# pw1316/MonteCarloPathTracer

Hardware: AMD Instinct MI355X
Metric: Mray/s + achieved HBM GB/s, Cornell Box 1024spp at 1/2/4/8 MI355X (higher is better)
Workload: dtype f32; 1 GPU; cornell_1024x1024_1024spp; scene=scene01, width=1024, height=1024, spp=1024, max_depth=7, spp_chunk=32, parallelism=pixel-tiles x1, pipeline=wavefront, wf_sort=False, kd_build=reference, kd_nodes=4395, kernel_variant=4

## Files before the change

include/mcpt.h:

```cpp
#ifndef MCPT_H
#define MCPT_H

#include <stddef.h>
#include <stdint.h>

#ifdef __cplusplus
extern "C" {
#endif

#define MCPT_ABI_VERSION 9

enum {
    MCPT_OK = 0,
    MCPT_E_INVALID = -1,
    MCPT_E_IO = -2,
    MCPT_E_PARSE = -3,
    MCPT_E_DEVICE = -4,
    MCPT_E_NOMEM = -5,
    MCPT_E_UNSUPPORTED = -6
};

typedef struct mcpt_model mcpt_model;
typedef struct mcpt_scene mcpt_scene;

// ... 84 lines not shown

typedef struct {
    int32_t pipeline;
    int32_t variant;
    int32_t wf_streams;
    uint32_t wf_batch;
    int32_t wf_refill;
    int32_t wf_group_shift;
    int32_t ready_thresh;
    int32_t tail_units;
    uint64_t work_paths;
    uint64_t workspace_bytes;
    uint64_t wf_queue_bytes;
    uint64_t device_free_bytes;
    int32_t devices;
    int32_t peer_access;
    uint32_t wf_batch_default;
} mcpt_plan_info;

typedef struct {
    const char* kd_cache_dir;
    int32_t host_only;
    int32_t layout;
    int32_t kd_build;
} mcpt_scene_options;

enum {
    MCPT_LAYOUT_AUTO = 0,
    MCPT_LAYOUT_GLOBAL = 1
};
enum {
    MCPT_KD_BUILD_REFERENCE = 0,
    MCPT_KD_BUILD_SAH = 1
};

int mcpt_abi_version(void);
const char* mcpt_last_error(void);
int mcpt_init(const int32_t* devices, int32_t n_devices);
int mcpt_device_count(int32_t* out);
void mcpt_render_params_default(mcpt_render_params* p);
void mcpt_render_params_quinengine(mcpt_render_params* p);

typedef struct {
    const float* vertices;        int64_t n_vertices;
    const float* normals;         int64_t n_normals;
    const int32_t* triangles;     int64_t n_triangles;
    const double* materials;      int64_t n_materials;
    const char* const* group_names;
    const int64_t* group_offsets;
    const int32_t* group_tris;    int64_t n_groups;
} mcpt_model_desc;
int mcpt_model_create(const mcpt_model_desc* d, mcpt_model** out);
int mcpt_model_read_obj(const char* path, mcpt_model** out);
int mcpt_model_read_obj_ex(const char* path, int32_t flavor, mcpt_model** out);
enum {
    MCPT_OBJ_CVMCTRACER = 0,
    MCPT_OBJ_TINYOBJ = 1
};
void mcpt_model_free(mcpt_model* m);
int mcpt_model_get_info(const mcpt_model* m, mcpt_model_info* out);
int mcpt_model_copy_vertices(const mcpt_model* m, float* out);
int mcpt_model_copy_normals(const mcpt_model* m, float* out);
int mcpt_model_copy_triangles(const mcpt_model* m, int32_t* out);
int mcpt_model_copy_materials(const mcpt_model* m, double* out);
int mcpt_model_group(const mcpt_model* m, int64_t g, char* name_buf, int64_t name_cap,
                     int64_t* n, int32_t* tris);

int mcpt_scene_create(const mcpt_model* m, mcpt_scene** out);
int mcpt_scene_create_host(const mcpt_model* m, mcpt_scene** out);
int mcpt_scene_create_cached(const mcpt_model* m, const char* kd_cache_dir, int32_t host_only,
                             mcpt_scene** out, int32_t* cache_hit);
int mcpt_scene_create_ex(const mcpt_model* m, const mcpt_scene_options* options, mcpt_scene** out,
                         int32_t* cache_hit);
void mcpt_scene_destroy(mcpt_scene* s);
int mcpt_scene_get_info(const mcpt_scene* s, mcpt_scene_info* out);
int mcpt_scene_terminal_cull_boxes(const mcpt_scene* s);
int mcpt_scene_miss_cull_boxes(const mcpt_scene* s, float* boxes);
int mcpt_scene_direct_lists(const mcpt_scene* s, int32_t* tri_box, uint32_t* box_tris, uint32_t* lists,
                            int32_t* list_kd);
uint64_t mcpt_scene_direct_rays(const mcpt_scene* s);
uint64_t mcpt_scene_extend_rays(const mcpt_scene* s);
uint64_t mcpt_scene_clipped_rays(const mcpt_scene* s);
uint64_t mcpt_scene_primary_shaded(const mcpt_scene* s);
uint64_t mcpt_scene_primary_shade_lds(const mcpt_scene* s);
int mcpt_scene_primary_tile_classes(mcpt_scene* s, uint32_t out[4]);
int mcpt_scene_copy_kd(const mcpt_scene* s, uint32_t* nodes, uint32_t* leaf_ids,
                       int32_t* kd_tris, float* geoms);

int mcpt_render(mcpt_scene* s, const mcpt_render_params* p, float* fb_rgb, mcpt_render_stats* stats);
int mcpt_render_device(mcpt_scene* s, const mcpt_render_params* p, float* d_fb_rgba, void* hip_stream);
int mcpt_render_stats_read(mcpt_scene* s, mcpt_render_stats* out);
int mcpt_render_unit_counters(mcpt_scene* s, const mcpt_render_params* p, float* fb_rgb,
                              uint32_t* unit_counters);
int64_t mcpt_shard_pixel_count(const mcpt_render_params* p);
int mcpt_shard_pixels(const mcpt_render_params* p, int32_t* xy);
int mcpt_intersect(mcpt_scene* s, int64_t n, const float* o, const float* d, float t_max,
                   int32_t* tri_out, float* hit_out, mcpt_render_stats* stats);
int mcpt_scene_reserve(mcpt_scene* s, const mcpt_render_params* p);
int mcpt_plan_query(mcpt_scene* s, const mcpt_render_params* p, mcpt_plan_info* out);

int mcpt_render_aov(mcpt_scene* s, const mcpt_render_params* p, float* albedo_cov, float* normal_depth);
int mcpt_render_aov_device(mcpt_scene* s, const mcpt_render_params* p, float* d_albedo_cov, float* d_normal_depth,
                           void* hip_stream);

typedef struct {
    int32_t width, height;
    int32_t iterations;
    int32_t normal_power_log2;
    float sigma_z;
    float albedo_floor;
    int32_t gamma_space;
} mcpt_denoise_params;
void mcpt_denoise_params_default(mcpt_denoise_params* p);
int mcpt_denoise(const mcpt_denoise_params* p, const float* color_rgb, const float* albedo_cov,
                 const float* normal_depth, float* out_rgb);
int mcpt_denoise_device(const mcpt_denoise_params* p, const float* d_color_rgba, const float* d_albedo_cov,
                        const float* d_normal_depth, float* d_out_rgba, float* d_scratch_rgba, void* hip_stream);

int mcpt_render_var(mcpt_scene* s, const mcpt_render_params* p, float* fb_rgb, float* var_rgba,
                    mcpt_render_stats* stats);
int mcpt_render_var_device(mcpt_scene* s, const mcpt_render_params* p, float* d_fb_rgba, float* d_var_rgba,
                           void* hip_stream);

typedef struct {
    mcpt_denoise_params base;
    float sigma_l;
} mcpt_denoise_var_params;
void mcpt_denoise_var_params_default(mcpt_denoise_var_params* p);
int mcpt_denoise_var(const mcpt_denoise_var_params* p, const float* color_rgb, const float* var_rgba,
                     const float* albedo_cov, const float* normal_depth, float* out_rgb);
int mcpt_denoise_var_device(const mcpt_denoise_var_params* p, const float* d_color_rgba, const float* d_var_rgba,
                            const float* d_albedo_cov, const float* d_normal_depth, float* d_out_rgba,
                            float* d_scratch_rgba, void* hip_stream);

typedef struct {
    int32_t max_passes;
    int32_t min_passes;
    float   threshold;
    float   lum_floor;
    int32_t dilate;
    int32_t force_list;
} mcpt_adaptive_params;
void mcpt_adaptive_params_default(mcpt_adaptive_params*);
int mcpt_render_adaptive(mcpt_scene*, const mcpt_render_params*, const mcpt_adaptive_params*,
                         float* fb_rgb, float* var_rgba, uint32_t* pass_count, mcpt_render_stats* stats);
int mcpt_render_adaptive_device(mcpt_scene*, const mcpt_render_params*, const mcpt_adaptive_params*,
                                float* d_fb_rgba, float* d_var_rgba, uint32_t* d_pass_count, void* hip_stream);
int mcpt_render_adaptive_ex(mcpt_scene*, const mcpt_render_params*, const mcpt_adaptive_params*,
                            float* fb_rgb, float* var_rgba, uint32_t* pass_count, mcpt_render_stats* stats);
int mcpt_render_adaptive_ex_device(mcpt_scene*, const mcpt_render_params*, const mcpt_adaptive_params*,
                                   float* d_fb_rgba, float* d_var_rgba, uint32_t* d_pass_count, void* hip_stream);

enum { MCPT_TRACE_CLOSEST = 0, MCPT_TRACE_ANY = 1 };
typedef struct {
    int32_t kind;
    float   t_max;
    int32_t lean;
    int32_t workgroups;
    int32_t refill;
} mcpt_trace_params;
void mcpt_trace_params_default(mcpt_trace_params*);

int mcpt_trace_device(mcpt_scene*, const mcpt_trace_params* p, int64_t n, const float* d_o, const float* d_d,
                      const float* d_t_max, int32_t* d_tri, float* d_hit, void* hip_stream);
int mcpt_occluded_device(mcpt_scene*, const mcpt_trace_params* p, int64_t n, const float* d_o, const float* d_d,
                         const float* d_t_max, uint8_t* d_occluded, void* hip_stream);
// ... 31 lines not shown
```

montecarlopathtracer_amd/_build.py:

```python
from __future__ import annotations

import os
import subprocess
import sys
from concurrent.futures import ThreadPoolExecutor

HERE = os.path.dirname(os.path.abspath(__file__))
ROOT = os.path.dirname(HERE)
CSRC = os.path.join(HERE, "csrc")
LIBDIR = os.path.join(HERE, "lib")
LIB = os.path.join(LIBDIR, os.environ.get("MCPT_LIB_NAME", "libmcpt.so"))
SOURCES = ["host_model.cpp", "kd_cache.cpp", "capi.cpp", "scene_image.cpp", "plan.cpp", "render_host.cpp", "queries.cpp",
           "render.hip", "wavefront.hip", "wavefront_primary.hip", "wavefront_primary_shade.hip",
           "aov.hip", "denoise.hip", "variance.hip", "denoise_var.hip", "adaptive.hip", "rayquery.hip"]
_WF_FLAGS = ["-mllvm", "-amdgpu-set-wave-priority=1", "-mllvm", "-two-entry-phi-node-folding-threshold=8",
             "-mllvm", "-unroll-threshold=2000"]
SOURCE_FLAGS = {"wavefront_primary.hip": ["-mllvm", "-structurizecfg-skip-uniform-regions=1"] + _WF_FLAGS,
                "wavefront_primary_shade.hip": _WF_FLAGS,
                "wavefront.hip": _WF_FLAGS,
                "rayquery.hip": _WF_FLAGS,
                "render.hip": ["-mllvm", "-enable-gvn-hoist", "-mllvm", "-unroll-threshold=2000"]}
SOURCE_SCHED = {"wavefront_primary_shade.hip": "iterative-minreg"}
HEADERS = ["capi_internal.hpp", "staging.hpp", "host_model.hpp", "mcpt_device.hpp", "render_launch.hpp", "wf_route.hpp", "trace_device.hpp", "half_box.hpp",
           "aov_device.hpp", "aov_launch.hpp", "variance_launch.hpp", "adaptive_launch.hpp", "partial_sum.hpp", "rayquery_launch.hpp",
           "wf_device.hpp", "wf_primary_body.hpp", "wf_primary_walk.hpp", "wf_primary_pairs.hpp", "wf_primary_shade_body.hpp", "wf_shade_item.hpp"]
ARCH = os.environ.get("MCPT_OFFLOAD_ARCH", "gfx950")

COMMON = ["-O3", "-std=c++17", "-fPIC", "-ffp-contract=off", "-fno-fast-math", "-fno-slp-vectorize", "-Wall",
          "-I" + os.path.join(ROOT, "include")] + os.environ.get("MCPT_EXTRA_FLAGS", "").split()


def _hipcc() -> str:
    for c in (os.environ.get("HIPCC"), "/opt/rocm/bin/hipcc", "hipcc"):
        if c and (os.path.sep not in c or os.path.exists(c)):
            return c
    raise RuntimeError("hipcc not found")


def _stale() -> bool:
    if not os.path.exists(LIB):
        return True
    t = os.path.getmtime(LIB)
    deps = [os.path.join(CSRC, f) for f in SOURCES + HEADERS] + [os.path.join(ROOT, "include", "mcpt.h"),
                                                                 os.path.abspath(__file__)]
    return any(os.path.getmtime(d) > t for d in deps)


def build(force: bool = False, verbose: bool = False) -> str:
    if not force and not _stale():
        return LIB
    os.makedirs(os.path.join(LIBDIR, "obj"), exist_ok=True)
    hipcc = _hipcc()

    def compile_one(src):
        obj = os.path.join(LIBDIR, "obj", os.path.basename(LIB) + "." + src + ".o")
        sched = SOURCE_SCHED.get(src) or os.environ.get("MCPT_SCHED", "max-ilp")
        lang = (["-x", "hip", f"--offload-arch={ARCH}", "-mllvm", f"-amdgpu-sched-strategy={sched}"]
                if src.endswith(".hip")
                else ["-x", "c++", "-D__HIP_PLATFORM_AMD__", "-I/opt/rocm/include"])
        cmd = [hipcc] + lang + COMMON + SOURCE_FLAGS.get(src, []) + ["-c", os.path.join(CSRC, src), "-o", obj]
        if verbose:
            print(" ".join(cmd), file=sys.stderr)
        r = subprocess.run(cmd, capture_output=True, text=True)
        if r.returncode != 0:
            raise RuntimeError(f"compile failed: {src}\n{r.stdout}\n{r.stderr}")
        return obj

    with ThreadPoolExecutor(max_workers=len(SOURCES)) as ex:
        objs = list(ex.map(compile_one, SOURCES))
    tmp = LIB + f".{os.getpid()}.tmp"
    cmd = [hipcc, f"--offload-arch={ARCH}", "-shared", "-fPIC", "-o", tmp] + objs
    r = subprocess.run(cmd, capture_output=True, text=True)
    if r.returncode != 0:
        raise RuntimeError(f"link failed\n{r.stdout}\n{r.stderr}")
    os.replace(tmp, LIB)
    return LIB


if __name__ == "__main__":
    print(build(force="--force" in sys.argv, verbose=True))
```

montecarlopathtracer_amd/_capi.py:

```python
from __future__ import annotations

import ctypes as C
import os

try:
    import torch
except Exception:
    torch = None

_HERE = os.path.dirname(os.path.abspath(__file__))
LIB_PATH = os.environ.get("MCPT_LIB_PATH") or os.path.join(_HERE, "lib", "libmcpt.so")

MCPT_OK = 0
ABI_VERSION = 9
MODE_CVMCTRACER = 0
MODE_QUINENGINE = 1
PIPELINE_MEGAKERNEL = 0
PIPELINE_WAVEFRONT = 1
GATHER_PEER = 0
GATHER_RCCL = 1
ERRORS = {-1: "INVALID", -2: "IO", -3: "PARSE", -4: "DEVICE", -5: "NOMEM", -6: "UNSUPPORTED"}


class McptError(RuntimeError):
# ... 57 lines not shown


class DenoiseParamsC(C.Structure):
    _fields_ = [("width", C.c_int32), ("height", C.c_int32), ("iterations", C.c_int32),
                ("normal_power_log2", C.c_int32), ("sigma_z", C.c_float), ("albedo_floor", C.c_float),
                ("gamma_space", C.c_int32)]


class DenoiseVarParamsC(C.Structure):
    _fields_ = [("base", DenoiseParamsC), ("sigma_l", C.c_float)]


class AdaptiveParamsC(C.Structure):
    _fields_ = [("max_passes", C.c_int32), ("min_passes", C.c_int32), ("threshold", C.c_float),
                ("lum_floor", C.c_float), ("dilate", C.c_int32), ("force_list", C.c_int32)]


class TraceParamsC(C.Structure):
    _fields_ = [("kind", C.c_int32), ("t_max", C.c_float), ("lean", C.c_int32), ("workgroups", C.c_int32),
                ("refill", C.c_int32)]


class RadianceParamsC(C.Structure):
    _fields_ = [("spp", C.c_uint32), ("spp_offset", C.c_uint32), ("spp_chunk", C.c_uint32),
                ("max_depth", C.c_int32), ("illum", C.c_float), ("fresnel_kd", C.c_int32), ("seed", C.c_uint64),
                ("prev_count", C.c_uint32), ("lean", C.c_int32), ("workgroups", C.c_int32),
                ("ready_thresh", C.c_int32)]


TRACE_CLOSEST = 0
TRACE_ANY = 1
OBJ_CVMCTRACER = 0
OBJ_TINYOBJ = 1
LAYOUT_AUTO = 0
LAYOUT_GLOBAL = 1
KD_BUILD_REFERENCE = 0
KD_BUILD_SAH = 1


class ModelDesc(C.Structure):
    _fields_ = [
        ("vertices", C.POINTER(C.c_float)), ("n_vertices", C.c_int64),
        ("normals", C.POINTER(C.c_float)), ("n_normals", C.c_int64),
        ("triangles", C.POINTER(C.c_int32)), ("n_triangles", C.c_int64),
        ("materials", C.POINTER(C.c_double)), ("n_materials", C.c_int64),
        ("group_names", C.POINTER(C.c_char_p)), ("group_offsets", C.POINTER(C.c_int64)),
        ("group_tris", C.POINTER(C.c_int32)), ("n_groups", C.c_int64),
    ]


_vp = C.c_void_p
_SIGS = {
    "mcpt_abi_version": (C.c_int, []),
    "mcpt_last_error": (C.c_char_p, []),
    "mcpt_init": (C.c_int, [C.POINTER(C.c_int32), C.c_int32]),
    "mcpt_device_count": (C.c_int, [C.POINTER(C.c_int32)]),
    "mcpt_render_params_default": (None, [C.POINTER(RenderParamsC)]),
    "mcpt_render_params_quinengine": (None, [C.POINTER(RenderParamsC)]),
    "mcpt_model_create": (C.c_int, [C.POINTER(ModelDesc), C.POINTER(_vp)]),
    "mcpt_model_read_obj": (C.c_int, [C.c_char_p, C.POINTER(_vp)]),
    "mcpt_model_read_obj_ex": (C.c_int, [C.c_char_p, C.c_int32, C.POINTER(_vp)]),
    "mcpt_model_free": (None, [_vp]),
    "mcpt_model_get_info": (C.c_int, [_vp, C.POINTER(ModelInfo)]),
    "mcpt_model_copy_vertices": (C.c_int, [_vp, C.POINTER(C.c_float)]),
    "mcpt_model_copy_normals": (C.c_int, [_vp, C.POINTER(C.c_float)]),
    "mcpt_model_copy_triangles": (C.c_int, [_vp, C.POINTER(C.c_int32)]),
    "mcpt_model_copy_materials": (C.c_int, [_vp, C.POINTER(C.c_double)]),
    "mcpt_model_group": (C.c_int, [_vp, C.c_int64, C.c_char_p, C.c_int64, C.POINTER(C.c_int64), C.POINTER(C.c_int32)]),
    "mcpt_scene_create": (C.c_int, [_vp, C.POINTER(_vp)]),
    "mcpt_scene_create_host": (C.c_int, [_vp, C.POINTER(_vp)]),
    "mcpt_scene_create_cached": (C.c_int, [_vp, C.c_char_p, C.c_int32, C.POINTER(_vp), C.POINTER(C.c_int32)]),
    "mcpt_scene_create_ex": (C.c_int, [_vp, C.POINTER(SceneOptions), C.POINTER(_vp), C.POINTER(C.c_int32)]),
    "mcpt_scene_destroy": (None, [_vp]),
    "mcpt_scene_get_info": (C.c_int, [_vp, C.POINTER(SceneInfo)]),
    "mcpt_scene_terminal_cull_boxes": (C.c_int, [_vp]),
    "mcpt_scene_miss_cull_boxes": (C.c_int, [_vp, C.POINTER(C.c_float)]),
    "mcpt_scene_primary_tile_classes": (C.c_int, [_vp, C.POINTER(C.c_uint32)]),
    "mcpt_scene_direct_lists": (C.c_int, [_vp, C.POINTER(C.c_int32), C.POINTER(C.c_uint32), C.POINTER(C.c_uint32),
                                           C.POINTER(C.c_int32)]),
    "mcpt_scene_direct_rays": (C.c_uint64, [_vp]),
    "mcpt_scene_extend_rays": (C.c_uint64, [_vp]),
    "mcpt_scene_clipped_rays": (C.c_uint64, [_vp]),
    "mcpt_scene_primary_shaded": (C.c_uint64, [_vp]),
    "mcpt_scene_primary_shade_lds": (C.c_uint64, [_vp]),
    "mcpt_scene_copy_kd": (C.c_int, [_vp, C.POINTER(C.c_uint32), C.POINTER(C.c_uint32), C.POINTER(C.c_int32),
                                     C.POINTER(C.c_float)]),
    "mcpt_render": (C.c_int, [_vp, C.POINTER(RenderParamsC), C.POINTER(C.c_float), C.POINTER(RenderStats)]),
    "mcpt_render_device": (C.c_int, [_vp, C.POINTER(RenderParamsC), _vp, _vp]),
    "mcpt_render_unit_counters": (C.c_int, [_vp, C.POINTER(RenderParamsC), C.POINTER(C.c_float),
                                            C.POINTER(C.c_uint32)]),
    "mcpt_render_stats_read": (C.c_int, [_vp, C.POINTER(RenderStats)]),
    "mcpt_intersect": (C.c_int, [_vp, C.c_int64, C.POINTER(C.c_float), C.POINTER(C.c_float), C.c_float,
                                 C.POINTER(C.c_int32), C.POINTER(C.c_float), C.POINTER(RenderStats)]),
    "mcpt_shard_pixel_count": (C.c_int64, [C.POINTER(RenderParamsC)]),
    "mcpt_shard_pixels": (C.c_int, [C.POINTER(RenderParamsC), C.POINTER(C.c_int32)]),
    "mcpt_scene_reserve": (C.c_int, [_vp, C.POINTER(RenderParamsC)]),
    "mcpt_plan_query": (C.c_int, [_vp, C.POINTER(RenderParamsC), C.POINTER(PlanInfo)]),
    "mcpt_render_aov": (C.c_int, [_vp, C.POINTER(RenderParamsC), C.POINTER(C.c_float), C.POINTER(C.c_float)]),
    "mcpt_render_aov_device": (C.c_int, [_vp, C.POINTER(RenderParamsC), _vp, _vp, _vp]),
    "mcpt_denoise_params_default": (None, [C.POINTER(DenoiseParamsC)]),
    "mcpt_denoise": (C.c_int, [C.POINTER(DenoiseParamsC), C.POINTER(C.c_float), C.POINTER(C.c_float),
                               C.POINTER(C.c_float), C.POINTER(C.c_float)]),
    "mcpt_denoise_device": (C.c_int, [C.POINTER(DenoiseParamsC), _vp, _vp, _vp, _vp, _vp, _vp]),
    "mcpt_render_var": (C.c_int, [_vp, C.POINTER(RenderParamsC), C.POINTER(C.c_float), C.POINTER(C.c_float),
                                  C.POINTER(RenderStats)]),
    "mcpt_render_var_device": (C.c_int, [_vp, C.POINTER(RenderParamsC), _vp, _vp, _vp]),
    "mcpt_denoise_var_params_default": (None, [C.POINTER(DenoiseVarParamsC)]),
    "mcpt_denoise_var": (C.c_int, [C.POINTER(DenoiseVarParamsC), C.POINTER(C.c_float), C.POINTER(C.c_float),
                                   C.POINTER(C.c_float), C.POINTER(C.c_float), C.POINTER(C.c_float)]),
    "mcpt_denoise_var_device": (C.c_int, [C.POINTER(DenoiseVarParamsC), _vp, _vp, _vp, _vp, _vp, _vp, _vp]),
    "mcpt_adaptive_params_default": (None, [C.POINTER(AdaptiveParamsC)]),
    "mcpt_render_adaptive": (C.c_int, [_vp, C.POINTER(RenderParamsC), C.POINTER(AdaptiveParamsC),
                                       C.POINTER(C.c_float), C.POINTER(C.c_float), C.POINTER(C.c_uint32),
                                       C.POINTER(RenderStats)]),
    "mcpt_render_adaptive_device": (C.c_int, [_vp, C.POINTER(RenderParamsC), C.POINTER(AdaptiveParamsC), _vp, _vp,
                                              _vp, _vp]),
    "mcpt_render_adaptive_ex": (C.c_int, [_vp, C.POINTER(RenderParamsC), C.POINTER(AdaptiveParamsC),
                                          C.POINTER(C.c_float), C.POINTER(C.c_float), C.POINTER(C.c_uint32),
                                          C.POINTER(RenderStats)]),
    "mcpt_render_adaptive_ex_device": (C.c_int, [_vp, C.POINTER(RenderParamsC), C.POINTER(AdaptiveParamsC), _vp,
                                                 _vp, _vp, _vp]),
    "mcpt_trace_params_default": (None, [C.POINTER(TraceParamsC)]),
    "mcpt_trace_device": (C.c_int, [_vp, C.POINTER(TraceParamsC), C.c_int64, _vp, _vp, _vp, _vp, _vp, _vp]),
    "mcpt_occluded_device": (C.c_int, [_vp, C.POINTER(TraceParamsC), C.c_int64, _vp, _vp, _vp, _vp, _vp]),
    "mcpt_occluded": (C.c_int, [_vp, C.POINTER(TraceParamsC), C.c_int64, C.POINTER(C.c_float), C.POINTER(C.c_float),
                                C.POINTER(C.c_float), C.POINTER(C.c_uint8), C.POINTER(RenderStats)]),
    "mcpt_trace_stats_read": (C.c_int, [_vp, C.POINTER(RenderStats)]),
    "mcpt_scene_reserve_rays": (C.c_int, [_vp]),
    "mcpt_radiance_params_default": (None, [C.POINTER(RadianceParamsC)]),
    "mcpt_radiance_device": (C.c_int, [_vp, C.POINTER(RadianceParamsC), C.c_int64, _vp, _vp, _vp, _vp, _vp]),
    "mcpt_radiance": (C.c_int, [_vp, C.POINTER(RadianceParamsC), C.c_int64, C.POINTER(C.c_float),
                                C.POINTER(C.c_float), C.POINTER(C.c_uint32), C.POINTER(C.c_float),
                                C.POINTER(RenderStats)]),
    "mcpt_scene_reserve_radiance": (C.c_int, [_vp, C.POINTER(RadianceParamsC), C.c_int64]),
}

_lib = None


def lib():
    global _lib
    if _lib is None:
        if not os.path.exists(LIB_PATH):
            raise ImportError(f"{LIB_PATH} not found: build it with `python -c 'import __graft_entry__ as g; "
                              f"g.build()'` or `python -m montecarlopathtracer_amd._build`")
        L = C.CDLL(LIB_PATH)
        for name, (res, args) in _SIGS.items():
            f = getattr(L, name)
            f.restype = res
            f.argtypes = args
        if L.mcpt_abi_version() != ABI_VERSION:
            raise ImportError("libmcpt.so ABI version mismatch")
        _lib = L
    return _lib


def check(rc: int) -> int:
    if rc < 0:
        raise McptError(rc, lib().mcpt_last_error().decode(errors="replace"))
    return rc


def declared_symbols():
    return list(_SIGS)
```

montecarlopathtracer_amd/csrc/capi_internal.hpp:

```cpp
#pragma once
#include <hip/hip_runtime.h>
#include <rccl/rccl.h>

#include <cstdint>
#include <cstring>
#include <memory>
#include <string>
#include <vector>

#include "../../include/mcpt.h"
#include "host_model.hpp"
#include "render_launch.hpp"
#include "staging.hpp"
#include "wf_route.hpp"

struct mcpt_model {
    mcpt::ObjModel m;
};

namespace mcpt::host {

int fail(int code, const std::string& msg);
extern thread_local std::vector<int> g_devices;
extern thread_local bool g_peer_ok;
// ... 5 lines not shown
            throw mcpt::Error{e_ == hipErrorOutOfMemory ? MCPT_E_NOMEM : MCPT_E_DEVICE,   \
                              std::string(#expr) + ": " + hipGetErrorString(e_)};       \
    } while (0)

template <typename F>
int guarded(F&& f) {
    try {
        return f();
    } catch (const mcpt::Error& e) {
        return fail(e.code, e.msg);
    } catch (const std::bad_alloc&) {
        return fail(MCPT_E_NOMEM, "out of host memory");
    } catch (const std::exception& e) {
        return fail(MCPT_E_INVALID, e.what());
    }
}

struct DevBuf {
    void* p = nullptr;
    size_t bytes = 0;
};

struct TempDev {
    void* p = nullptr;
    TempDev() = default;
    explicit TempDev(size_t bytes) { alloc(bytes); }
    TempDev(const TempDev&) = delete;
    TempDev& operator=(const TempDev&) = delete;
    ~TempDev() {
        if (p) (void)hipFree(p);
    }
    void alloc(size_t bytes) { HIP_TRY(hipMalloc(&p, bytes ? bytes : 16)); }
    void* release() {
        void* q = p;
        p = nullptr;
        return q;
    }
};

struct Workspace {
    DevBuf partial;
    DevBuf small;
    DevBuf spill;
    DevBuf fb;
    DevBuf wf;
    DevBuf tail;
};

struct Timing {
    hipEvent_t e[3];
};

struct DeviceGuard {
    int prev = -1;
    DeviceGuard() { (void)hipGetDevice(&prev); }
    ~DeviceGuard() {
        if (prev >= 0) (void)hipSetDevice(prev);
    }
};

}

struct mcpt_scene {
    mcpt::HostScene hs;
    bool on_device = false;
    int device = -1;
    int cus = 0;
    std::vector<unsigned char> image;
    std::vector<uint32_t> tri_order;
    mcpt::GpuScene gpu{};
    uint32_t n_cull_boxes = 0;
    uint32_t cull_box[mcpt::kMaxCullBoxes][3] = {};
    float cull_gain = 0.0f;
    uint32_t n_miss_boxes = 0;
    float miss_box[mcpt::kMaxMissBoxes][6] = {};
    std::vector<int32_t> tri_box;
    uint32_t box_tris[mcpt::kMaxMissBoxes] = {};
    uint32_t direct_counts = 0;
    uint32_t direct_list[mcpt::kMaxMissBoxes * 16] = {};
    uint64_t direct_rays = 0;
    uint64_t extend_rays = 0;
    uint64_t clipped_rays = 0;
    uint64_t primary_shaded = 0;
    mcpt::host::DevBuf d_image, d_normals;
    mcpt::host::Workspace ws;
    std::vector<mcpt::host::Timing> pending, free_timing;
    mcpt::host::Timing capture_timing{};
    bool has_capture_timing = false;
    int last_variant = 0;
    uint64_t renders = 0;
    size_t wf_reserved = 0;
    bool reserved = false;
    std::vector<void*> retired;
    std::vector<std::unique_ptr<mcpt_scene>> replicas;
    hipStream_t stream = nullptr;
    hipEvent_t done = nullptr;
    hipEvent_t start = nullptr;
    mcpt::host::DevBuf gather;
    hipStream_t wf_stream[mcpt::kMaxWfStreams] = {};
    hipEvent_t wf_fork = nullptr, wf_join[mcpt::kMaxWfStreams] = {};
    bool peer_access = true;
    std::vector<ncclComm_t> comms;
    mcpt::host::DevBuf gather_send;
    mcpt::host::DevBuf ad_list, ad_flags, ad_blocks;
    uint32_t* ad_host_n = nullptr;
    mcpt::host::DevBuf rq_order, rq_stats;
    mcpt::host::DevBuf rad_partial, rad_tail, rad_small;

    std::vector<mcpt::host::DevBuf*> buffers() {
        return {&d_image, &d_normals, &ws.partial, &ws.small, &ws.spill, &ws.fb, &ws.wf, &ws.tail, &gather, &gather_send,
                &ad_list, &ad_flags, &ad_blocks, &rq_order, &rq_stats, &rad_partial, &rad_tail, &rad_small};
    }
    ~mcpt_scene();
};

namespace mcpt::host {

struct Plan {
    mcpt::KernelParams kp;
    size_t out_pixels;
    bool capturing = false;
    int pipeline;
    int wf_streams;
    uint32_t wf_capacity;
    bool wf_batch_explicit;
    int32_t wf_sort;
    int32_t wf_refill;
    mcpt::WfRoute route;
    int64_t tail_per_lane;
    int64_t tail_exact;
    uint64_t wf_mem_limit;
    uint64_t work;
    int sets() const { return pipeline == MCPT_PIPELINE_WAVEFRONT ? wf_streams : 1; }
};

struct Prepared {
    Plan pl;
    mcpt::WfParams wf[mcpt::kMaxWfStreams];
};

inline bool ranges_overlap(const void* a, size_t na, const void* b, size_t nb) {
    const uintptr_t x = reinterpret_cast<uintptr_t>(a), y = reinterpret_cast<uintptr_t>(b);
    return x < y + nb && y < x + na;
}

void ensure_buf(DevBuf& b, size_t need);
void grow_ws(mcpt_scene& s, DevBuf& b, size_t need, bool capturing);
void set_device(const mcpt_scene& s);
bool stream_capturing(hipStream_t st);
uint32_t tea16(uint32_t v0, uint32_t v1);
int ready_thresh_for(const mcpt_scene& s, int32_t asked);
size_t launched_lanes(const mcpt_scene& s);
mcpt::WfFacts scene_facts(const mcpt_scene& s);
constexpr size_t kSpillEntries = 32;
constexpr int64_t kTailPerLane = 4;
size_t spill_bytes(const mcpt_scene& s, int sets);
void grow_spill(mcpt_scene& s, int sets, bool capturing);
uint64_t tail_split(uint64_t lanes, int64_t per_lane, int64_t exact, uint32_t total_units, uint32_t chunk);
uint64_t tail_units_for(const mcpt_scene& s, const Plan& pl);
Plan make_plan(const mcpt_scene& s, const mcpt_render_params* p);
uint32_t wf_batch_capacity(const mcpt_scene& s, const mcpt_render_params* p, uint64_t work, uint32_t chunk, int nstr);
void prepare_wavefront_list(mcpt_scene& s, Plan& pl, const Plan& pass0, uint32_t n, const mcpt_render_params* p,
                            mcpt::WfParams* out);
void fit_wavefront(const mcpt_scene& s, Plan& pl);
void prepare_workspace(mcpt_scene& s, Plan& pl, bool tail_split = false, int spill_sets = 1);
uint32_t* tile_classes(const mcpt_scene& s);
// ... 8 lines not shown
```

montecarlopathtracer_amd/csrc/host_model.cpp:

```cpp
#include "host_model.hpp"

#include <algorithm>
#include <array>
#include <cmath>
#include <cctype>
#include <cfloat>
#include <cstdio>
#include <cstdlib>
#include <cstring>
#include <deque>
#include <fstream>
#include <map>
#include <numeric>
#include <sstream>

#include "../../include/mcpt.h"

namespace mcpt {
namespace {

struct Cursor {
    const char* p;
    const char* end;
    bool fail = false;
// ... 501 lines not shown
    if (!nt || max_boxes < 1) return 0;
    for (float v : hs.kd_verts)
        if (!std::isfinite(v)) return 0;
    std::vector<CBox> tb(nt);
    CBox all{{INFINITY, INFINITY, INFINITY}, {-INFINITY, -INFINITY, -INFINITY}};
    for (size_t k = 0; k < nt; ++k) {
        const float* v = &hs.kd_verts[9 * k];
        CBox b{{v[0], v[1], v[2]}, {v[0], v[1], v[2]}};
        for (int j = 1; j < 3; ++j) b.add(CBox{{v[3 * j], v[3 * j + 1], v[3 * j + 2]}, {v[3 * j], v[3 * j + 1], v[3 * j + 2]}});
        tb[k] = b;
        all.add(b);
    }
    std::vector<CBox> bx;
    if (nt <= kMissCullExact) {
        bx = tb;
    } else {
        for (int with_planes = 1; with_planes >= 0; --with_planes) {
            std::map<std::pair<int, uint32_t>, CBox> buckets;
            for (const CBox& b : tb) {
                std::pair<int, uint32_t> key{3, 0u};
                for (int a = 0; a < 3 && with_planes; ++a)
                    if (b.lo[a] == b.hi[a] && key.first == 3) {
                        const float c = b.lo[a] + 0.0f;
                        uint32_t bits;
                        std::memcpy(&bits, &c, 4);
                        key = {a, bits};
                    }
                if (key.first == 3) {
                    for (int a = 0; a < 3; ++a) {
                        const double ext = double(all.hi[a]) - all.lo[a];
                        const double c = (double(b.lo[a]) + b.hi[a]) * 0.5 - all.lo[a];
                        const int cell = ext > 0.0 ? std::min(7, std::max(0, int(c / ext * 8.0))) : 0;
                        key.second = key.second * 8u + uint32_t(cell);
                    }
                }
                auto it = buckets.find(key);
                if (it == buckets.end()) buckets.emplace(key, b);
                else it->second.add(b);
            }
            bx.clear();
            for (const auto& kv : buckets) bx.push_back(kv.second);
            if (bx.size() <= kMissCullExact) break;
        }
    }
    cluster_boxes(bx, bx.size());
    bool face[3][2] = {};
    for (const CBox& b : bx) {
        for (int a = 0; a < 3; ++a) {
            if (b.lo[a] != b.hi[a]) continue;
            bool covers = true;
            for (int c = 0; c < 3; ++c)
                if (c != a) covers = covers && b.lo[c] <= all.lo[c] && b.hi[c] >= all.hi[c];
            if (covers && b.lo[a] == all.lo[a]) face[a][0] = true;
            if (covers && b.lo[a] == all.hi[a]) face[a][1] = true;
        }
    }
    if (face[0][0] && face[0][1] && face[1][0] && face[1][1] && face[2][0] && face[2][1]) return 0;
    cluster_boxes(bx, static_cast<size_t>(max_boxes));
    for (const CBox& b : bx) {
        bool spans = true;
        for (int a = 0; a < 3; ++a) spans = spans && b.lo[a] <= all.lo[a] && b.hi[a] >= all.hi[a];
        if (spans) return 0;
    }
    for (size_t k = 0; k < bx.size(); ++k)
        for (int a = 0; a < 3; ++a) {
            boxes[k][a] = bx[k].lo[a];
            boxes[k][3 + a] = bx[k].hi[a];
        }
    return static_cast<int>(bx.size());
}

void direct_list_assign(const HostScene& hs, const float (*boxes)[6], int n_boxes, std::vector<int32_t>& tri_box) {
    const size_t nt = hs.kd_verts.size() / 9;
    tri_box.assign(nt, -1);
    for (size_t k = 0; k < nt; ++k) {
        const float* v = &hs.kd_verts[9 * k];
        for (int b = 0; b < n_boxes && tri_box[k] < 0; ++b) {
            bool in = true;
            for (int j = 0; j < 3; ++j)
                for (int a = 0; a < 3; ++a) in = in && v[3 * j + a] >= boxes[b][a] && v[3 * j + a] <= boxes[b][3 + a];
            if (in) tri_box[k] = b;
        }
    }
}

namespace {

inline float smin(float a, float b) { return (b < a) ? b : a; }
inline float smax(float a, float b) { return (a < b) ? b : a; }

struct Box {
    float mn[3], mx[3];
    static Box empty() {
        Box b;
        for (int i = 0; i < 3; ++i) { b.mn[i] = FLT_MAX; b.mx[i] = -FLT_MAX; }
        return b;
    }
    void add_pt(const float* p) {
        for (int i = 0; i < 3; ++i) { mn[i] = smin(mn[i], p[i]); mx[i] = smax(mx[i], p[i]); }
    }
    void add(const Box& r) { add_pt(r.mn); add_pt(r.mx); }
    void clip(const Box& r) {
        for (int i = 0; i < 3; ++i) { mn[i] = smax(mn[i], r.mn[i]); mx[i] = smin(mx[i], r.mx[i]); }
    }
    float half_area() const {
        float s0 = mx[0] - mn[0], s1 = mx[1] - mn[1], s2 = mx[2] - mn[2];
        return s0 * s1 + s1 * s2 + s2 * s0;
    }
};

struct BNode {
    Box box;
    Box region;
    std::vector<uint32_t> ids;
    uint32_t axis = 0;
    float split = 0.0f;
    int32_t left = -1, right = -1;
    int depth = 0;
};

template <typename FL, typename FR>
inline void classify(const Box& tb, int a, float v, FL&& to_left, FR&& to_right) {
    if (tb.mn[a] == tb.mx[a] && tb.mn[a] == v) {
        to_left();
    } else {
        if (tb.mn[a] < v) to_left();
        if (tb.mx[a] > v) to_right();
    }
}

#ifndef MCPT_SAH_CT
#define MCPT_SAH_CT 1.0f
#define MCPT_SAH_CI 1.5f
#endif
constexpr float kSahCt = MCPT_SAH_CT, kSahCi = MCPT_SAH_CI;
struct SahScratch {
    std::vector<float> mins, maxs, plan, cand;
};
bool sah_split(const std::vector<Box>& tbox, const std::vector<uint32_t>& ids, const Box& R, SahScratch& w,
               int& ax, float& val) {
    const float sz[3] = {R.mx[0] - R.mn[0], R.mx[1] - R.mn[1], R.mx[2] - R.mn[2]};
    const float A0 = sz[0] * sz[1] + sz[1] * sz[2] + sz[2] * sz[0];
    if (!(A0 > 0.0f)) return false;
    const size_t n = ids.size();
    float best = kSahCi * static_cast<float>(n);
    bool found = false;
    for (int a = 0; a < 3; ++a) {
        w.mins.clear(); w.maxs.clear(); w.plan.clear(); w.cand.clear();
        for (uint32_t id : ids) {
            const float lo = tbox[id].mn[a], hi = tbox[id].mx[a];
            w.mins.push_back(lo);
            w.maxs.push_back(hi);
            if (lo == hi) w.plan.push_back(lo);
            if (R.mn[a] < lo && lo < R.mx[a]) w.cand.push_back(lo + 0.0f);
            if (R.mn[a] < hi && hi < R.mx[a]) w.cand.push_back(hi + 0.0f);
        }
        std::sort(w.mins.begin(), w.mins.end());
        std::sort(w.maxs.begin(), w.maxs.end());
        std::sort(w.plan.begin(), w.plan.end());
        std::sort(w.cand.begin(), w.cand.end());
        size_t im = 0, ix = 0, ip = 0;
        for (size_t q = 0; q < w.cand.size(); ++q) {
            if (q > 0 && !(w.cand[q - 1] < w.cand[q])) continue;
            const float v = w.cand[q];
            while (im < n && w.mins[im] < v) ++im;
            while (ix < n && !(v < w.maxs[ix])) ++ix;
// ... 161 lines not shown
```

montecarlopathtracer_amd/csrc/host_model.hpp:

```cpp
#pragma once

#include <cstdint>
#include <map>
#include <string>
#include <vector>

namespace mcpt {

struct Vec3 {
    float x = 0, y = 0, z = 0;
};

struct ObjTriangle {
    int32_t v[3] = {0, 0, 0};
    int32_t t[3] = {0, 0, 0};
    int32_t n[3] = {0, 0, 0};
    int32_t material = 0;
};

struct ObjMaterial {
    std::string name;
    Vec3 Ka, Kd, Ks;
    double Ns = 1.0, Tr = 0.0, Ni = 1.0;
};

struct ObjModel {
    std::string path;
    std::vector<Vec3> vertices;
    int64_t n_texcoords = 0;
    std::vector<Vec3> normals;
    std::vector<ObjTriangle> triangles;
    std::vector<ObjMaterial> materials;
    std::map<std::string, std::vector<int32_t>> groups;
};

void read_obj(const std::string& path, ObjModel& out, int flavor = 0);
void read_obj_cv(const std::string& path, ObjModel& out);

struct Geometry {
    Vec3 Ka, Kd, Ks;
    float Ns, Tr, Ni;
    uint32_t start, count;
};

struct KdNode {
    uint32_t left = 0xFFFFFFFFu, right = 0xFFFFFFFFu;
    float bmin[3], bmax[3];
    uint32_t axis = 0;
    float split = 0.0f;
    uint32_t leaf_begin = 0, leaf_count = 0;
};

struct HostScene {
    std::vector<Geometry> geoms;
    std::vector<int32_t> kd_tris;
    std::vector<uint32_t> kd_geom;
    std::vector<uint32_t> kd_prio;
    std::vector<float> kd_verts;
    std::vector<float> kd_normals;
    std::vector<KdNode> nodes;
    std::vector<uint32_t> leaf_ids;
    int kd_depth = 0;
    int kd_build = 0;
};

void build_host_scene(const ObjModel& m, HostScene& out, const char* kd_cache_dir = nullptr,
                      int* cache_hit = nullptr, int kd_build = 0);
int terminal_cull_boxes(const HostScene& hs, float (*boxes)[6], int max_boxes);
int miss_cull_boxes(const HostScene& hs, float (*boxes)[6], int max_boxes);
void direct_list_assign(const HostScene& hs, const float (*boxes)[6], int n_boxes, std::vector<int32_t>& tri_box);
bool kd_cache_load(const std::string& dir, const std::vector<float>& tri_verts, std::vector<KdNode>& nodes,
                   std::vector<uint32_t>& leaf_ids, int& depth, int kd_build = 0);
bool kd_cache_store(const std::string& dir, const std::vector<float>& tri_verts, const std::vector<KdNode>& nodes,
                    const std::vector<uint32_t>& leaf_ids, int depth, int kd_build = 0);
void build_kdtree(const std::vector<float>& tri_verts, std::vector<KdNode>& nodes,
                  std::vector<uint32_t>& leaf_ids, int& depth, int kd_build = 0);

struct Error {
    int code;
    std::string msg;
};

}
```

montecarlopathtracer_amd/csrc/plan.cpp:

```cpp
#include <algorithm>
#include <cfloat>
#include <cmath>
#include <cstdio>

#include "capi_internal.hpp"

using namespace mcpt::host;

namespace {

struct Vf {
    float x, y, z;
};
Vf normal_of(Vf v) {
    float len = std::sqrt(v.x * v.x + v.y * v.y + v.z * v.z);
    float d = std::fmax(len, FLT_MIN);
    return Vf{v.x / d, v.y / d, v.z / d};
}
Vf cross_of(Vf a, Vf b) { return Vf{a.y * b.z - a.z * b.y, a.z * b.x - a.x * b.z, a.x * b.y - a.y * b.x}; }

int clamp_i(int v, int lo, int hi) { return v < lo ? lo : (v > hi ? hi : v); }

int wavefront_streams(const mcpt::WfRoute& r, uint64_t work, const mcpt_render_params* p) {
    const int n = p->wf_streams > 0 ? p->wf_streams
// ... 51 lines not shown
        w.radiance = reinterpret_cast<float4*>(b); b += l.f4;
        w.tile_cand = l.tiles ? reinterpret_cast<uint32_t*>(b) : nullptr; b += l.tiles;
        w.tile_classes = tile_classes(s);
        w.cnt = reinterpret_cast<mcpt::WfCounters*>(b);
        w.capacity = pl.wf_capacity;
        w.slot_stride = static_cast<uint32_t>(l.cap_slots);
        w.refill_thresh = clamp_i(pl.wf_refill, 1, 64);
        w.sort = pl.wf_sort;
        w.nseg = r.nseg;
        w.group_shift = r.group_shift;
        w.xcd_deal = r.xcd_deal;
        w.shade_cull = r.shade_cull ? 1u : 0u;
        w.n_cull_boxes = r.n_cull_boxes;
        std::memcpy(w.cull_box, s.cull_box, sizeof w.cull_box);
        w.n_miss_boxes = r.n_miss_boxes;
        std::memcpy(w.miss_box, s.miss_box, sizeof w.miss_box);
        w.direct_counts = r.direct_counts;
        std::memcpy(w.direct_list, s.direct_list, sizeof w.direct_list);
    }
}

void ensure_wf_streams(mcpt_scene& s, int n) {
    if (n > 1 && !s.wf_fork) HIP_TRY(hipEventCreateWithFlags(&s.wf_fork, hipEventDisableTiming));
    for (int i = 1; i < n; i++) {
        if (!s.wf_stream[i]) HIP_TRY(hipStreamCreateWithFlags(&s.wf_stream[i], hipStreamNonBlocking));
        if (!s.wf_join[i]) HIP_TRY(hipEventCreateWithFlags(&s.wf_join[i], hipEventDisableTiming));
    }
}

}

namespace mcpt::host {

void ensure_buf(DevBuf& b, size_t need) {
    if (b.bytes >= need && b.p) return;
    if (b.p) HIP_TRY(hipFree(b.p));
    b.p = nullptr;
    b.bytes = 0;
    HIP_TRY(hipMalloc(&b.p, need ? need : 16));
    b.bytes = need;
}

void grow_ws(mcpt_scene& s, DevBuf& b, size_t need, bool capturing) {
    if (b.bytes >= need && b.p) return;
    if (capturing)
        throw mcpt::Error{MCPT_E_NOMEM, "render needs more workspace than the scene holds while its stream is "
                                        "capturing a graph: call mcpt_scene_reserve with these params first"};
    if (b.p && s.reserved) {
        s.retired.push_back(b.p);
        b.p = nullptr;
        b.bytes = 0;
    }
    ensure_buf(b, need);
}

void set_device(const mcpt_scene& s) {
    int cur = -1;
    HIP_TRY(hipGetDevice(&cur));
    if (cur != s.device) HIP_TRY(hipSetDevice(s.device));
}

bool stream_capturing(hipStream_t st) {
    if (!st) return false;
    hipStreamCaptureStatus cs = hipStreamCaptureStatusNone;
    HIP_TRY(hipStreamIsCapturing(st, &cs));
    return cs != hipStreamCaptureStatusNone;
}

uint32_t tea16(uint32_t v0, uint32_t v1) {
    uint32_t sum = 0;
    for (int n = 0; n < 16; n++) {
        sum += 0x9e3779b9u;
        v0 += ((v1 << 4) + 0xa341316cu) ^ (v1 + sum) ^ ((v1 >> 5) + 0xc8013ea4u);
        v1 += ((v0 << 4) + 0xad90777du) ^ (v0 + sum) ^ ((v0 >> 5) + 0x7e95761eu);
    }
    return v0;
}

int ready_thresh_for(const mcpt_scene& s, int32_t asked) { return asked > 0 ? asked : (mcpt::scene_in_lds(s.gpu) ? 32 : 40); }

size_t launched_lanes(const mcpt_scene& s) { return static_cast<size_t>(mcpt::total_lanes_for(s.gpu, s.cus)); }

mcpt::WfFacts scene_facts(const mcpt_scene& s) {
    return mcpt::WfFacts{&s.gpu, s.n_miss_boxes, s.direct_counts, s.n_cull_boxes, s.cus};
}

size_t spill_bytes(const mcpt_scene& s, int sets) { return size_t(sets) * kSpillEntries * launched_lanes(s) * 16; }
void grow_spill(mcpt_scene& s, int sets, bool capturing) { grow_ws(s, s.ws.spill, spill_bytes(s, sets), capturing); }

Plan make_plan(const mcpt_scene& s, const mcpt_render_params* p) {
    if (!p) throw mcpt::Error{MCPT_E_INVALID, "params is NULL"};
    if (p->width <= 0 || p->height <= 0) throw mcpt::Error{MCPT_E_INVALID, "width/height must be positive"};
    if (p->spp == 0) throw mcpt::Error{MCPT_E_INVALID, "spp must be > 0"};
    if (p->max_depth < 0 || p->max_depth > mcpt::kMaxDepthParam) throw mcpt::Error{MCPT_E_INVALID, "max_depth out of range"};
    if (p->wf_streams < 0 || p->wf_streams > mcpt::kMaxWfStreams)
        throw mcpt::Error{MCPT_E_INVALID, "wf_streams must be 0 (automatic) or 1..4"};
    if (p->wf_refill < 0 || p->wf_refill > 64 || p->ready_thresh < 0 || p->ready_thresh > 64)
        throw mcpt::Error{MCPT_E_INVALID, "wf_refill / ready_thresh must be 0 (automatic) or 1..64"};
    if (p->wf_group_shift != 0 && (p->wf_group_shift < 6 || p->wf_group_shift > 14))
        throw mcpt::Error{MCPT_E_INVALID, "wf_group_shift must be 0 (automatic) or 6..14"};
    if (p->tail_units < 0) throw mcpt::Error{MCPT_E_INVALID, "tail_units must be >= 0"};
    if (p->gather != MCPT_GATHER_PEER && p->gather != MCPT_GATHER_RCCL)
        throw mcpt::Error{MCPT_E_INVALID, "unknown gather"};
    const int T = p->tile > 0 ? p->tile : 8;
    if (T > 256) throw mcpt::Error{MCPT_E_INVALID, "tile too large"};
    const int sc = p->shard_count > 1 ? p->shard_count : 1;
    const int si = sc > 1 ? p->shard_index : 0;
    if (si < 0 || si >= sc) throw mcpt::Error{MCPT_E_INVALID, "shard_index out of range"};
    const uint64_t tiles_x = (uint64_t(p->width) + T - 1) / T, tiles_y = (uint64_t(p->height) + T - 1) / T;
    const uint64_t ntiles = tiles_x * tiles_y;
    const uint64_t owned = uint64_t(si) < ntiles ? (ntiles - uint64_t(si) + uint64_t(sc) - 1) / uint64_t(sc) : 0;
    const uint64_t npix = owned * uint64_t(T) * uint64_t(T);
    const uint32_t chunk = p->spp_chunk ? (p->spp_chunk < p->spp ? p->spp_chunk : p->spp) : p->spp;
    const uint64_t nchunks = (uint64_t(p->spp) + chunk - 1) / chunk;
    if (npix * nchunks >= 0xFFFFFFFFull) throw mcpt::Error{MCPT_E_UNSUPPORTED, "too many work units for one call"};

    Plan pl;
    mcpt::KernelParams& k = pl.kp;
    std::memset(&k, 0, sizeof k);
    k.scene = s.gpu;
    k.width = p->width; k.height = p->height;
    k.tile = T; k.tiles_x = static_cast<int32_t>(tiles_x);
    k.shard_count = sc; k.shard_index = si;
    k.packed = (p->packed || sc > 1) ? 1 : 0;
    k.npix_local = static_cast<uint32_t>(npix);
    k.spp = p->spp; k.spp_offset = p->spp_offset; k.chunk = chunk;
    k.nchunks = static_cast<uint32_t>(nchunks);
    k.total_units = static_cast<uint32_t>(npix * nchunks);
    k.div_npix = mcpt::FastDiv::make(std::max<uint32_t>(k.npix_local, 1));
    k.div_tt = mcpt::FastDiv::make(static_cast<uint32_t>(T * T));
    k.div_tiles_x = mcpt::FastDiv::make(static_cast<uint32_t>(tiles_x));
    k.div_tile = mcpt::FastDiv::make(static_cast<uint32_t>(T));
    k.div_chunk = mcpt::FastDiv::make(chunk);
    k.tail_units = k.total_units;
    k.total_items = k.total_units;
    k.max_depth = p->max_depth;
    k.lean = p->lean ? 1 : 0;
    k.illum = p->illum;
    const float a = p->fov_deg * 3.14159265359f / 360;
    k.tan_half_fov = static_cast<float>(std::tan(static_cast<double>(a)));
    k.h_over_w = 1.0 * static_cast<double>(static_cast<uint32_t>(p->height)) / static_cast<double>(static_cast<uint32_t>(p->width));
    k.inv_w_pow2 = (p->width > 0 && (p->width & (p->width - 1)) == 0) ? 1.0 / static_cast<double>(p->width) : 0.0;
    k.fresnel_kd = p->fresnel_kd ? 1 : 0;
    k.prev_count = p->prev_count;
    Vf d = normal_of(Vf{p->dir[0], p->dir[1], p->dir[2]});
    Vf r = normal_of(cross_of(d, Vf{p->up[0], p->up[1], p->up[2]}));
    Vf u = normal_of(cross_of(r, d));
    for (int i = 0; i < 3; ++i) k.eye[i] = p->eye[i];
    k.fwd[0] = d.x; k.fwd[1] = d.y; k.fwd[2] = d.z;
    k.up[0] = u.x; k.up[1] = u.y; k.up[2] = u.z;
    k.right[0] = r.x; k.right[1] = r.y; k.right[2] = r.z;
    if (p->mode != MCPT_MODE_CVMCTRACER && p->mode != MCPT_MODE_QUINENGINE)
        throw mcpt::Error{MCPT_E_INVALID, "unknown mode"};
    k.mode = p->mode;
    k.best_init = FLT_MAX;
    if (p->mode == MCPT_MODE_QUINENGINE) {
        k.key = static_cast<uint32_t>(p->seed);
        k.best_init = 10000.0f;
        const float a = p->fov_deg * 3.14159265359f / 360;
        const float ys = static_cast<float>(1.0 / std::tan(static_cast<double>(a)));
        k.proj22 = ys;
        k.proj11 = ys / (static_cast<float>(p->width) / static_cast<float>(p->height));
    } else {
        k.key = tea16(static_cast<uint32_t>(p->seed), static_cast<uint32_t>(p->seed >> 32));
    }
    k.ready_thresh = ready_thresh_for(s, p->ready_thresh);
    pl.out_pixels = k.packed ? size_t(npix) : size_t(p->width) * size_t(p->height);
// ... 227 lines not shown
```

montecarlopathtracer_amd/csrc/render_host.cpp:

```cpp
#include <dlfcn.h>

#include <algorithm>
#include <cmath>

#include "adaptive_launch.hpp"
#include "aov_launch.hpp"
#include "capi_internal.hpp"
#include "variance_launch.hpp"

using namespace mcpt::host;

namespace {

struct Rccl {
    decltype(&ncclCommInitAll) comm_init_all = nullptr;
    decltype(&ncclCommDestroy) comm_destroy = nullptr;
    decltype(&ncclGather) gather = nullptr;
    decltype(&ncclGroupStart) group_start = nullptr;
    decltype(&ncclGroupEnd) group_end = nullptr;
    decltype(&ncclGetErrorString) error_string = nullptr;
    std::string load_error;
};
const Rccl& rccl() {
    static const Rccl r = [] {
        Rccl x;
        void* h = dlopen("librccl.so.1", RTLD_NOW | RTLD_LOCAL);
        if (!h) h = dlopen("/opt/rocm/lib/librccl.so.1", RTLD_NOW | RTLD_LOCAL);
        if (!h) {
            const char* e = dlerror();
            x.load_error = std::string("cannot load librccl: ") + (e ? e : "?");
            return x;
        }
        x.comm_init_all = reinterpret_cast<decltype(&ncclCommInitAll)>(dlsym(h, "ncclCommInitAll"));
        x.comm_destroy = reinterpret_cast<decltype(&ncclCommDestroy)>(dlsym(h, "ncclCommDestroy"));
        x.gather = reinterpret_cast<decltype(&ncclGather)>(dlsym(h, "ncclGather"));
        x.group_start = reinterpret_cast<decltype(&ncclGroupStart)>(dlsym(h, "ncclGroupStart"));
        x.group_end = reinterpret_cast<decltype(&ncclGroupEnd)>(dlsym(h, "ncclGroupEnd"));
        x.error_string = reinterpret_cast<decltype(&ncclGetErrorString)>(dlsym(h, "ncclGetErrorString"));
        if (!x.comm_init_all || !x.comm_destroy || !x.gather || !x.group_start || !x.group_end || !x.error_string)
            x.load_error = "librccl lacks ncclCommInitAll / ncclGather / ncclGroupStart / ncclGroupEnd";
        return x;
    }();
    return r;
}

#define NCCL_TRY(expr)                                                                                  \
    do {                                                                                                \
        ncclResult_t r_ = (expr);                                                                       \
        if (r_ != ncclSuccess)                                                                          \
            throw mcpt::Error{MCPT_E_DEVICE, std::string(#expr) + ": " + rccl().error_string(r_)};   \
    } while (0)

void render_multi(mcpt_scene& s, const mcpt_render_params* p, float* d_fb, hipStream_t st);

void ensure_capture_timing(mcpt_scene& s) {
    if (s.has_capture_timing) return;
    for (auto& ev : s.capture_timing.e) HIP_TRY(hipEventCreate(&ev));
    s.has_capture_timing = true;
}

Timing acquire_timing(mcpt_scene& s, bool capturing) {
    Timing t;
    if (capturing) {
        ensure_capture_timing(s);
        t = s.capture_timing;
    } else if (!s.free_timing.empty()) {
        t = s.free_timing.back();
        s.free_timing.pop_back();
    } else {
        for (auto& ev : t.e) HIP_TRY(hipEventCreate(&ev));
    }
    return t;
}

mcpt::WfStreams wf_streams_on(const mcpt_scene& s, int n, hipStream_t st) {
    mcpt::WfStreams wst{};
    wst.n = n;
    wst.st[0] = st;
    wst.fork = s.wf_fork;
    for (int i = 1; i < wst.n; i++) {
        wst.st[i] = s.wf_stream[i];
        wst.join[i] = s.wf_join[i];
    }
    return wst;
}

void render_async(mcpt_scene& s, const mcpt_render_params* p, float* d_fb, hipStream_t st,
                  uint32_t* d_unit_counters = nullptr, bool raw_mean = false, float* d_var = nullptr,
                  Plan* fitted = nullptr) {
    if (!s.on_device) throw mcpt::Error{MCPT_E_INVALID, "scene was created host-only"};
    if (!d_fb) throw mcpt::Error{MCPT_E_INVALID, "framebuffer is NULL"};
    if (multi_device(s, p, d_unit_counters)) {
        render_multi(s, p, d_fb, st);
        return;
    }
    set_device(s);
    Prepared R;
    prepare_render(s, p, stream_capturing(st), d_unit_counters != nullptr, R);
    Plan& pl = R.pl;
    pl.kp.raw_mean = raw_mean ? 1 : 0;
    pl.kp.unit_counters = d_unit_counters;
    if (fitted) *fitted = pl;
    HIP_TRY(hipMemsetAsync(tile_classes(s), 0, 16, st));
    const Timing t = acquire_timing(s, pl.capturing);
    if (pl.pipeline == MCPT_PIPELINE_WAVEFRONT) {
        HIP_TRY(mcpt::launch_wavefront(pl.kp, pl.route, R.wf, wf_streams_on(s, pl.sets(), st), t.e[0], t.e[1], t.e[2],
                                       reinterpret_cast<float4*>(d_fb), &s.last_variant));
    } else {
        HIP_TRY(mcpt::launch_render(pl.kp, s.cus, st, t.e[0], t.e[1], t.e[2], reinterpret_cast<float4*>(d_fb),
                                    &s.last_variant));
    }
    if (d_var) HIP_TRY(mcpt::launch_variance(pl.kp, reinterpret_cast<float4*>(d_var), st));
    if (pl.capturing) return;
    s.pending.push_back(t);
    s.renders++;
}

void read_stats(mcpt_scene& s, mcpt_render_stats* out) {
    set_device(s);
    mcpt_render_stats r;
    std::memset(&r, 0, sizeof r);
    double kms = 0, rms = 0;
    for (auto& t : s.pending) {
        HIP_TRY(hipEventSynchronize(t.e[2]));
        float a = 0, b = 0;
        HIP_TRY(hipEventElapsedTime(&a, t.e[0], t.e[1]));
        HIP_TRY(hipEventElapsedTime(&b, t.e[1], t.e[2]));
        kms += a;
        rms += b;
        s.free_timing.push_back(t);
    }
    s.pending.clear();
    s.direct_rays = 0;
    s.extend_rays = 0;
    s.clipped_rays = 0;
    s.primary_shaded = 0;
    if (s.ws.small.p) {
        unsigned long long st[mcpt::kStatSlots];
        char* const block = static_cast<char*>(s.ws.small.p) + 64;
        HIP_TRY(hipMemcpy(st, block, sizeof st, hipMemcpyDeviceToHost));
        HIP_TRY(hipMemset(block, 0, sizeof st));
        HIP_TRY(hipStreamSynchronize(nullptr));
        if (st[8] | st[9] | st[10] | st[11])
            std::fprintf(stderr, "mcpt phase cycles (sum over waves): units %llu trav %llu shade %llu burst_iters %llu "
                         "scatter %llu\n", st[8], st[9], st[10], st[11], st[12]);
#ifdef MCPT_PHASE_TIMING
        {
            unsigned long long lu[6], lw[6];
            mcpt::read_lane_use(lu);
            mcpt::read_lane_use_wf(lw);
            for (int i = 0; i < 6; i++) lu[i] += lw[i];
            std::fprintf(stderr, "mcpt lane use: descent %.3f (%llu wave-iters) triangle %.3f (%llu) burst %.3f (%llu)\n",
                         lu[0] ? double(lu[1]) / (64.0 * lu[0]) : 0.0, lu[0], lu[2] ? double(lu[3]) / (64.0 * lu[2]) : 0.0,
                         lu[2], lu[4] ? double(lu[5]) / (64.0 * lu[4]) : 0.0, lu[4]);
        }
#endif
        r.rays = st[0]; r.paths = st[1]; r.inner_visits = st[2]; r.leaf_visits = st[3];
        r.leaf_refs = st[4]; r.tri_tests = st[5]; r.shades = st[6]; r.stack_spills = st[7];
        s.direct_rays = st[mcpt::kStatDirect];
        s.extend_rays = st[mcpt::kStatExtend];
        s.clipped_rays = st[mcpt::kStatClipped];
        s.primary_shaded = st[mcpt::kStatPrimaryShaded];
    }
    r.renders = s.renders;
    r.devices = 1;
    s.renders = 0;
    r.kernel_ms = kms;
    r.reduce_ms = rms;
    r.variant = s.last_variant;
    if (out) *out = r;
}

void ensure_comms(mcpt_scene& s) {
    if (!s.comms.empty()) return;
    const Rccl& R = rccl();
    if (!R.load_error.empty()) throw mcpt::Error{MCPT_E_UNSUPPORTED, R.load_error};
    std::vector<int> devs{s.device};
    for (auto& rep : s.replicas) devs.push_back(rep->device);
    std::vector<ncclComm_t> comms(devs.size(), nullptr);
    NCCL_TRY(R.comm_init_all(comms.data(), static_cast<int>(devs.size()), devs.data()));
    s.comms = comms;
}

uint64_t multi_slot(const Plan& full, const mcpt_render_params* p, int n) {
    const int T = full.kp.tile;
    const uint64_t ntiles = uint64_t(full.kp.tiles_x) * ((uint64_t(p->height) + T - 1) / T);
    return (ntiles + n - 1) / n * uint64_t(T) * uint64_t(T);
}

void render_multi(mcpt_scene& s, const mcpt_render_params* p, float* d_fb, hipStream_t st) {
    DeviceGuard guard;
    set_device(s);
    const Plan full = make_plan(s, p);
    const bool use_rccl = p->gather == MCPT_GATHER_RCCL;
    const int n = 1 + static_cast<int>(s.replicas.size());
    const int T = full.kp.tile;
    const uint64_t slot = multi_slot(full, p, n);
    if (slot * n >= (uint64_t(1) << 32)) throw mcpt::Error{MCPT_E_UNSUPPORTED, "image too large"};
    const bool cap = stream_capturing(st);
    grow_ws(s, s.gather, size_t(n) * slot * 16, cap);
    if (use_rccl) {
        ensure_comms(s);
        grow_ws(s, s.gather_send, size_t(slot) * 16, cap);
    }
    if (!s.start) HIP_TRY(hipEventCreateWithFlags(&s.start, hipEventDisableTiming));
    HIP_TRY(hipEventRecord(s.start, st));
    for (int r = 1; r < n; ++r) {
        mcpt_scene& R = *s.replicas[size_t(r - 1)];
        set_device(R);
        const mcpt_render_params pr = shard_params(*p, n, r);
        const size_t bytes = size_t(mcpt_shard_pixel_count(&pr)) * 16;
        grow_ws(R, R.ws.fb, use_rccl ? size_t(slot) * 16 : bytes, cap);
        HIP_TRY(hipStreamWaitEvent(R.stream, s.start, 0));
        render_async(R, &pr, static_cast<float*>(R.ws.fb.p), R.stream, nullptr, true);
        if (use_rccl) continue;
        char* dst = static_cast<char*>(s.gather.p) + size_t(r) * slot * 16;
        if (!bytes) {
        } else if (R.device == s.device && !p->force_peer_copy)
            HIP_TRY(hipMemcpyAsync(dst, R.ws.fb.p, bytes, hipMemcpyDeviceToDevice, R.stream));
        else
            HIP_TRY(hipMemcpyPeerAsync(dst, s.device, R.ws.fb.p, R.device, bytes, R.stream));
        HIP_TRY(hipEventRecord(R.done, R.stream));
    }
    set_device(s);
    const mcpt_render_params p0 = shard_params(*p, n, 0);
    render_async(s, &p0, static_cast<float*>(use_rccl ? s.gather_send.p : s.gather.p), st, nullptr, true);
    if (use_rccl) {
        const Rccl& R = rccl();
        const size_t count = size_t(slot) * 4;
        NCCL_TRY(R.group_start());
        try {
            for (int r = 0; r < n; ++r) {
                const void* send = r ? s.replicas[size_t(r - 1)]->ws.fb.p : s.gather_send.p;
                hipStream_t rs = r ? s.replicas[size_t(r - 1)]->stream : st;
                NCCL_TRY(R.gather(send, r ? nullptr : s.gather.p, count, ncclFloat32, 0, s.comms[size_t(r)], rs));
            }
        } catch (...) {
            (void)R.group_end();
            throw;
        }
        NCCL_TRY(R.group_end());
        for (auto& rep : s.replicas) {
            set_device(*rep);
            HIP_TRY(hipEventRecord(rep->done, rep->stream));
        }
        set_device(s);
    }
    for (auto& R : s.replicas) HIP_TRY(hipStreamWaitEvent(st, R->done, 0));
    mcpt::GatherParams g{};
    g.src = static_cast<const float4*>(s.gather.p);
    g.fb = reinterpret_cast<float4*>(d_fb);
    g.slot = static_cast<uint32_t>(slot);
    g.width = p->width; g.height = p->height; g.tile = T; g.tiles_x = full.kp.tiles_x; g.nshards = n;
    g.prev_count = p->prev_count;
    g.mode = p->mode;
    HIP_TRY(mcpt::launch_gather(g, st));
}

void read_stats_all(mcpt_scene& s, mcpt_render_stats* out) {
    mcpt_render_stats r;
    read_stats(s, &r);
    for (auto& R : s.replicas) {
        mcpt_render_stats q;
        read_stats(*R, &q);
        r.rays += q.rays; r.paths += q.paths; r.inner_visits += q.inner_visits; r.leaf_visits += q.leaf_visits;
        r.leaf_refs += q.leaf_refs; r.tri_tests += q.tri_tests; r.shades += q.shades;
        r.stack_spills += q.stack_spills;
        s.direct_rays += R->direct_rays;
        s.extend_rays += R->extend_rays;
        s.clipped_rays += R->clipped_rays;
        s.primary_shaded += R->primary_shaded;
        r.kernel_ms = std::max(r.kernel_ms, q.kernel_ms);
        r.reduce_ms = std::max(r.reduce_ms, q.reduce_ms);
    }
    r.devices = 1 + static_cast<int32_t>(s.replicas.size());
    set_device(s);
    if (out) *out = r;
}

void check_aov(const mcpt_scene& s, const mcpt_render_params* p, const float* ac, const float* nd) {
    if (ac == nd) throw mcpt::Error{MCPT_E_INVALID, "albedo_cov and normal_depth are the same buffer"};
    if (p->width <= 0 || p->height <= 0) throw mcpt::Error{MCPT_E_INVALID, "width/height must be positive"};
    if (p->spp == 0) throw mcpt::Error{MCPT_E_INVALID, "spp must be > 0"};
    if (!s.on_device) throw mcpt::Error{MCPT_E_INVALID, "scene was created host-only"};
    if (p->shard_count > 1 || p->packed)
        throw mcpt::Error{MCPT_E_UNSUPPORTED, "feature buffers are not sharded: shard_count <= 1, packed = 0"};
}

void aov_async(mcpt_scene& s, const mcpt_render_params* p, float* d_ac, float* d_nd, hipStream_t st) {
    if (!p) throw mcpt::Error{MCPT_E_INVALID, "params is NULL"};
    if (!d_ac || !d_nd) throw mcpt::Error{MCPT_E_INVALID, "NULL feature buffer"};
    check_aov(s, p, d_ac, d_nd);
    set_device(s);
    mcpt_render_params q = *p;
    q.spp_chunk = 0;
    q.tile = 8;
    q.shard_count = 1; q.shard_index = 0;
    q.pipeline = MCPT_PIPELINE_MEGAKERNEL;
    q.max_depth = 0;
    Plan pl = make_plan(s, &q);
    pl.capturing = stream_capturing(st);
    grow_spill(s, 1, pl.capturing);
    pl.kp.spill = static_cast<uint4*>(s.ws.spill.p);
    pl.kp.total_lanes = static_cast<uint32_t>(launched_lanes(s));
    HIP_TRY(mcpt::launch_aov(pl.kp, reinterpret_cast<float4*>(d_ac), reinterpret_cast<float4*>(d_nd), st));
}

void check_var_params(const mcpt_scene& s, const mcpt_render_params* p) {
    if (!p) throw mcpt::Error{MCPT_E_INVALID, "params is NULL"};
    if (p->width <= 0 || p->height <= 0) throw mcpt::Error{MCPT_E_INVALID, "width/height must be positive"};
    if (p->spp == 0) throw mcpt::Error{MCPT_E_INVALID, "spp must be > 0"};
    if (p->spp_chunk == 0 || p->spp_chunk >= p->spp)
        throw mcpt::Error{MCPT_E_INVALID, "the variance needs at least two chunks: set spp_chunk to 1 .. spp - 1 "
                                          "(spp_chunk = 0 is one chunk)"};
    if (p->shard_count > 1 || p->packed)
        throw mcpt::Error{MCPT_E_UNSUPPORTED, "the variance is not sharded: shard_count <= 1, packed = 0"};
    if (!s.replicas.empty() || p->gather == MCPT_GATHER_RCCL)
        throw mcpt::Error{MCPT_E_UNSUPPORTED, "the variance needs a one-device scene and the peer gather"};
}
void check_var_render(const mcpt_scene& s, const mcpt_render_params* p) {
    check_var_params(s, p);
    if (!s.on_device) throw mcpt::Error{MCPT_E_INVALID, "scene was created host-only"};
}

struct Adaptive {
    int32_t max_passes, min_passes, radius;
    float threshold, lum_floor;
    bool force_list;
};
Adaptive adaptive_resolve(const mcpt_adaptive_params* p) {
    mcpt_adaptive_params z;
    std::memset(&z, 0, sizeof z);
    if (!p) p = &z;
    if (p->max_passes < 0 || p->max_passes > 4096)
        throw mcpt::Error{MCPT_E_INVALID, "max_passes must be 0 (default 8) or 1..4096"};
    Adaptive a;
    a.max_passes = p->max_passes ? p->max_passes : 8;
    if (p->min_passes < 0 || p->min_passes > a.max_passes)
        throw mcpt::Error{MCPT_E_INVALID, "min_passes must be 0 (default 1) or 1..max_passes"};
    a.min_passes = p->min_passes ? p->min_passes : 1;
    if (!(p->threshold >= 0.0f) || !std::isfinite(p->threshold))
        throw mcpt::Error{MCPT_E_INVALID, "threshold must be finite and >= 0 (0 = default 0.2)"};
    a.threshold = p->threshold != 0.0f ? p->threshold : 0.2f;
    if (!(p->lum_floor >= 0.0f) || !std::isfinite(p->lum_floor))
        throw mcpt::Error{MCPT_E_INVALID, "lum_floor must be finite and >= 0 (0 = default 0.01)"};
    a.lum_floor = p->lum_floor != 0.0f ? p->lum_floor : 0.01f;
    if (p->dilate > 4) throw mcpt::Error{MCPT_E_INVALID, "dilate must be at most 4 (0 = default 1, < 0 = none)"};
    a.radius = p->dilate == 0 ? 1 : (p->dilate < 0 ? 0 : p->dilate);
    if (p->force_list != 0 && p->force_list != 1) throw mcpt::Error{MCPT_E_INVALID, "force_list must be 0 or 1"};
    a.force_list = p->force_list == 1;
    return a;
}

void check_adaptive_render(const mcpt_scene& s, const mcpt_render_params* p, const Adaptive& a, hipStream_t st,
                           bool any_pipeline) {
    check_var_params(s, p);
    (void)make_plan(s, p);
    if (p->prev_count != 0)
        throw mcpt::Error{MCPT_E_INVALID, "prev_count must be 0: an adaptive render starts its own running mean"};
    if (uint64_t(p->spp_offset) + uint64_t(a.max_passes) * uint64_t(p->spp) > (uint64_t(1) << 32))
        throw mcpt::Error{MCPT_E_INVALID, "spp_offset + max_passes * spp passes 2^32 sample indices"};
    if (!any_pipeline && p->pipeline != MCPT_PIPELINE_MEGAKERNEL)
        throw mcpt::Error{MCPT_E_UNSUPPORTED, "pipeline: adaptive sampling runs on the megakernel only"};
    if (p->mode != MCPT_MODE_CVMCTRACER)
        throw mcpt::Error{MCPT_E_UNSUPPORTED, "mode: adaptive sampling selects in linear radiance, CVMCTracer mode only"};
    if (!s.on_device) throw mcpt::Error{MCPT_E_INVALID, "scene was created host-only"};
    if (stream_capturing(st))
        throw mcpt::Error{MCPT_E_UNSUPPORTED, "hip_stream is capturing a graph: the host reads the pixel list's "
                                              "length each pass"};
}

void adaptive_async(mcpt_scene& s, const mcpt_render_params* p, const Adaptive& a, float* d_fb, float* d_var,
                    uint32_t* d_count, hipStream_t st) {
    set_device(s);
    const Plan full = make_plan(s, p);
    const size_t npx = size_t(p->width) * size_t(p->height);
    const uint32_t npix = full.kp.npix_local, nb = mcpt::adaptive_blocks(npix);
    mcpt::AdaptiveWs aw{};
    if (a.max_passes > 1) {
        const size_t counts = (size_t(nb) + 1 + 1) / 2 * 8;
        grow_ws(s, s.ad_list, size_t(npix) * 4, false);
        grow_ws(s, s.ad_flags, npx * 4, false);
        grow_ws(s, s.ad_blocks, counts + size_t(nb) * (mcpt::kAdaptiveBlock / 64) * 8, false);
        if (!s.ad_host_n) HIP_TRY(hipHostMalloc(reinterpret_cast<void**>(&s.ad_host_n), 64, hipHostMallocDefault));
        aw.list = static_cast<uint32_t*>(s.ad_list.p);
        aw.flags = static_cast<uint32_t*>(s.ad_flags.p);
        aw.blocks = static_cast<uint32_t*>(s.ad_blocks.p);
        aw.masks = reinterpret_cast<unsigned long long*>(static_cast<char*>(s.ad_blocks.p) + counts);
    }
    float4* fb = reinterpret_cast<float4*>(d_fb);
    float4* var = reinterpret_cast<float4*>(d_var);
    const bool wavefront = p->pipeline == MCPT_PIPELINE_WAVEFRONT;
    Plan pass0;
    render_async(s, p, d_fb, st, nullptr, false, d_var, &pass0);
    HIP_TRY(mcpt::launch_adaptive_fill(d_count, npx, 1u, st));
    for (int32_t j = 1; j < a.max_passes; ++j) {
        mcpt_render_params pj = *p;
        pj.spp_offset = p->spp_offset + uint32_t(j) * p->spp;
        pj.prev_count = uint32_t(j);
        const bool all = j < a.min_passes;
        if (all && !a.force_list) {
            render_async(s, &pj, d_fb, st, nullptr, false, d_var);
            HIP_TRY(mcpt::launch_adaptive_fill(d_count, npx, uint32_t(j) + 1u, st));
            continue;
        }
        mcpt::AdaptiveSelect sel;
        sel.threshold = a.threshold;
        sel.lum_floor = a.lum_floor;
        sel.radius = a.radius;
        sel.pass = uint32_t(j);
        sel.all = all ? 1 : 0;
        HIP_TRY(mcpt::launch_adaptive_select(full.kp, sel, aw, fb, var, d_count, st));
        HIP_TRY(hipMemcpyAsync(s.ad_host_n, aw.blocks + nb, 4, hipMemcpyDeviceToHost, st));
        HIP_TRY(hipStreamSynchronize(st));
        const uint32_t n = *s.ad_host_n;
        if (!n) break;
        if (n > npix) throw mcpt::Error{MCPT_E_DEVICE, "adaptive pixel list longer than the frame"};
        Prepared R;
        R.pl = make_plan(s, &pj);
        mcpt::KernelParams& k = R.pl.kp;
        Timing t;
        if (wavefront) {
            prepare_wavefront_list(s, R.pl, pass0, n, &pj, R.wf);
            k.pixel_list = aw.list;
            HIP_TRY(hipMemsetAsync(tile_classes(s), 0, 16, st));
            t = acquire_timing(s, false);
            HIP_TRY(mcpt::launch_wavefront(k, R.pl.route, R.wf, wf_streams_on(s, R.pl.sets(), st), t.e[0], t.e[1],
                                           nullptr, nullptr, &s.last_variant));
        } else {
            k.npix_local = n;
            k.total_units = n * k.nchunks;
            k.div_npix = mcpt::FastDiv::make(n);
            prepare_workspace(s, R.pl, true);
            k.pixel_list = aw.list;
            t = acquire_timing(s, false);
            HIP_TRY(mcpt::launch_render_list(k, s.cus, st, t.e[0], t.e[1], &s.last_variant));
        }
        HIP_TRY(mcpt::launch_adaptive_merge(k, fb, var, d_count, st));
        HIP_TRY(hipEventRecord(t.e[2], st));
        s.pending.push_back(t);
        s.renders++;
    }
}

int render_sync(mcpt_scene* s, const mcpt_render_params* p, float* fb_rgb, mcpt_render_stats* stats,
                uint32_t* unit_counters, float* var_rgba = nullptr) {
    return guarded([&]() -> int {
        if (!s || !fb_rgb) return fail(MCPT_E_INVALID, "NULL argument");
        if (var_rgba) check_var_render(*s, p);
        if (!s->on_device) return fail(MCPT_E_INVALID, "scene was created host-only");
        set_device(*s);
        Plan pl = make_plan(*s, p);
        const size_t npx = pl.out_pixels;
        const auto c = carve({npx * 16, var_rgba ? npx * 16 : size_t(0)});
        ensure_buf(s->ws.fb, c.total);
        float* d_fb = c.at<float>(s->ws.fb.p, 0);
        float* d_var = var_rgba ? c.at<float>(s->ws.fb.p, 1) : nullptr;
        if (var_rgba && p->prev_count > 0) HIP_TRY(hipMemcpy(d_var, var_rgba, npx * 16, hipMemcpyHostToDevice));
        std::vector<float> rgba(npx * 4, 0.0f);
        if (p->prev_count > 0) {
            rgb_to_rgba(fb_rgb, npx, rgba.data());
            HIP_TRY(hipMemcpy(d_fb, rgba.data(), npx * 16, hipMemcpyHostToDevice));
        } else {
            HIP_TRY(hipMemset(d_fb, 0, npx * 16));
        }
        read_stats_all(*s, nullptr);
        TempDev uc;
        const size_t uc_bytes = size_t(pl.kp.total_units) * 16;
        if (unit_counters) {
            uc.alloc(uc_bytes);
            HIP_TRY(hipMemset(uc.p, 0, uc_bytes ? uc_bytes : 16));
        }
        render_async(*s, p, d_fb, nullptr, static_cast<uint32_t*>(uc.p), false, d_var);
        HIP_TRY(hipStreamSynchronize(nullptr));
        if (var_rgba) HIP_TRY(hipMemcpy(var_rgba, d_var, npx * 16, hipMemcpyDeviceToHost));
        if (unit_counters) HIP_TRY(hipMemcpy(unit_counters, uc.p, uc_bytes, hipMemcpyDeviceToHost));
        HIP_TRY(hipMemcpy(rgba.data(), d_fb, npx * 16, hipMemcpyDeviceToHost));
        rgba_to_rgb(rgba.data(), npx, fb_rgb);
        read_stats_all(*s, stats);
        return MCPT_OK;
    });
}

}

namespace mcpt::host {

void destroy_comms(mcpt_scene& s) {
    if (s.comms.empty()) return;
    for (auto& R : s.replicas) {
        (void)hipSetDevice(R->device);
        (void)hipDeviceSynchronize();
    }
    for (ncclComm_t c : s.comms) (void)rccl().comm_destroy(c);
    (void)hipSetDevice(s.device);
}

}

extern "C" {

int mcpt_render_device(mcpt_scene* s, const mcpt_render_params* p, float* d_fb_rgba, void* hip_stream) {
    return guarded([&]() -> int {
        if (!s) return fail(MCPT_E_INVALID, "NULL scene");
        render_async(*s, p, d_fb_rgba, static_cast<hipStream_t>(hip_stream));
        return MCPT_OK;
    });
}

// ... 181 lines not shown
```

montecarlopathtracer_amd/csrc/render_launch.hpp:

```cpp
#pragma once

#include <hip/hip_runtime.h>
#include <stdint.h>

namespace mcpt {

constexpr int kLdsBlock = 1024;
constexpr int kGlobalBlock = 256;
constexpr int kGlobalBlocksPerCu = 4;
#ifndef MCPT_WF_GLOBAL_SEGS
#define MCPT_WF_GLOBAL_SEGS 4
#endif
constexpr int kWfGlobalSegsPerCu = MCPT_WF_GLOBAL_SEGS;
constexpr size_t kMaxLds = 160 * 1024;
constexpr int kMaxCullBoxes = 8;
#ifndef MCPT_PRIMARY_LIST_K
#define MCPT_PRIMARY_LIST_K 4
#endif
constexpr uint32_t kListK = MCPT_PRIMARY_LIST_K;
constexpr uint32_t kListRecWords = (kListK + 2u + 3u) & ~3u;
constexpr uint32_t kListMaxTris = 4096;
constexpr int kMaxMissBoxes = 8;
#ifndef MCPT_DIRECT_K
#define MCPT_DIRECT_K 2
#endif
constexpr uint32_t kDirectK = MCPT_DIRECT_K;
static_assert(kDirectK >= 1 && kDirectK <= 15, "a box's count is carried in 4 bits");
constexpr uint32_t kDirectTableWords = kMaxMissBoxes * kDirectK;
constexpr size_t kDirectLdsBytes = (size_t(kDirectTableWords) * 4 + 16 + 15) & ~size_t(15);
constexpr int kStatDirect = 13;
constexpr size_t kDirectShadeLds = size_t(kDirectTableWords) * (48 + 4);
static_assert(kDirectTableWords * 3 <= 256, "the shade's smallest workgroup copies one record part per thread");
constexpr int kStatExtend = 14;
constexpr uint32_t kDirectShift = 24, kDepthMask = (1u << kDirectShift) - 1u;
constexpr int kMaxDepthParam = 1000;
static_assert(3u * kMaxDepthParam + 1u < kDepthMask, "a ray's depth must fit under its selector");
static_assert(kMaxMissBoxes <= 8, "the clip walk's selector is one byte of box bits");
constexpr int kStatClipped = 15;
constexpr int kStatPrimaryShaded = 16;
constexpr int kStatSlots = 17;

struct GpuGeom {
    float Ka[3], Kd[3], Ks[3];
    float Ns, Tr, Ni;
    uint32_t Ns_u;
    uint32_t pad[3];
};
static_assert(sizeof(GpuGeom) == 64, "GpuGeom layout");

struct GpuScene {
    const unsigned char* image;
    const float4* normals;
    uint32_t image_bytes;
    uint32_t off_tris, off_nodes, off_leafs, off_geoms;
    uint32_t node_boxes;
    uint32_t n_tris, n_nodes, n_leafs, n_geoms;
    float root_min[3], root_max[3];
    uint32_t root_w[2];
};

struct FastDiv {
    uint32_t m, s1, s2, d;
    static FastDiv make(uint32_t d) {
        uint32_t l = 0;
        while (l < 32 && (uint64_t(1) << l) < d) l++;
        FastDiv f;
        f.m = static_cast<uint32_t>(((uint64_t(1) << 32) * ((uint64_t(1) << l) - d)) / d + 1);
        f.s1 = l < 1 ? l : 1;
        f.s2 = l > 0 ? l - 1 : 0;
        f.d = d;
        return f;
    }
    __host__ __device__ __forceinline__ uint32_t div(uint32_t n) const {
        const uint32_t t = static_cast<uint32_t>((uint64_t(m) * n) >> 32);
        return (t + ((n - t) >> s1)) >> s2;
    }
};

struct KernelParams {
    GpuScene scene;
    int32_t width, height;
    int32_t tile, tiles_x, shard_count, shard_index, packed;
    uint32_t npix_local;
    uint32_t spp, spp_offset, chunk, nchunks, total_units;
    int32_t max_depth;
    float illum, tan_half_fov;
    int32_t fresnel_kd;
    uint32_t prev_count;
    int32_t mode;
    float proj11, proj22;
    float best_init;
    float eye[3], fwd[3], up[3], right[3];
    uint32_t key;
    float4* partial;
    uint32_t* counter;
    unsigned long long* stats;
    uint4* spill;
    uint32_t total_lanes;
    uint32_t* unit_counters;
    int32_t ready_thresh;
    int32_t lean;
    FastDiv div_npix, div_tt, div_tiles_x, div_tile;
    uint32_t tail_units, total_items;
    FastDiv div_chunk;
    float4* tail_buf;
    double h_over_w, inv_w_pow2;
    int32_t raw_mean;
    const uint32_t* pixel_list;
};

struct RayInputs {
    const float* o;
    const float* d;
    const uint32_t* stream;
};
constexpr uint32_t kRadMinUnits = 64;

struct GatherParams {
    const float4* src;
    float4* fb;
    uint32_t slot;
    int32_t width, height, tile, tiles_x, nshards;
    uint32_t prev_count;
    int32_t mode;
};

constexpr int kQueryBlock = 256;
struct QueryParams {
    GpuScene scene;
    const float* o;
    const float* d;
    int32_t* slot;
    float* hit;
    uint4* spill;
    unsigned long long* stats;
    uint32_t n;
    float best_init;
};

struct WfCounters {
    uint32_t queued;
    uint32_t hits;
    uint32_t resolved;
    uint32_t pad[5];
};
struct WfParams {
    float4* q[2];
    float4* radiance;
    WfCounters* cnt;
    uint32_t capacity;
    uint32_t slot_stride;
    uint32_t v0, nb, s_begin, ns, chunk_index;
    uint32_t nsc;
    uint32_t nseg, seg;
    uint32_t group_shift;
    int32_t bounce;
    int32_t refill_thresh;
    int32_t sort;
    uint32_t xcd_deal;
    uint32_t n_cull_boxes;
    uint32_t cull_box[kMaxCullBoxes][3];
    uint32_t* tile_cand;
    uint32_t* tile_classes;
    uint32_t n_miss_boxes;
    float miss_box[kMaxMissBoxes][6];
    uint32_t direct_counts;
    uint32_t direct_list[kDirectTableWords];
    uint32_t shade_cull;
};

inline size_t lds_bytes_in_lds(uint32_t image_bytes, int S) { return (size_t)image_bytes + (size_t)S * kLdsBlock * 16; }
constexpr size_t kLdsCounterBytes = 32;
inline size_t lds_bytes_counted_in_lds(uint32_t image_bytes, int S) {
    return lds_bytes_in_lds(image_bytes, S) + kLdsCounterBytes;
}
constexpr size_t lds_bytes_global(int S, bool counted) {
    return (size_t)S * kGlobalBlock * 16 + (counted ? kLdsCounterBytes : 0);
}
inline bool scene_in_lds(const GpuScene& sc) { return !sc.node_boxes; }
struct MegakernelVariant {
    int variant;
    bool in_lds;
    int S;
};
MegakernelVariant megakernel_variant(const GpuScene& sc);
int total_lanes_for(const GpuScene& sc, int cus);
#ifdef __HIP__
template <typename K>
hipError_t set_dyn_lds(K kernel, size_t lds_bytes) {
    return hipFuncSetAttribute(reinterpret_cast<const void*>(kernel), hipFuncAttributeMaxDynamicSharedMemorySize,
                               (int)lds_bytes);
}
template <typename K, typename... Args>
hipError_t launch_dyn_lds(K kernel, dim3 grid, dim3 block, size_t lds_bytes, hipStream_t st, const Args&... args) {
    const hipError_t e = set_dyn_lds(kernel, lds_bytes);
    if (e != hipSuccess) return e;
    hipLaunchKernelGGL(kernel, grid, block, lds_bytes, st, args...);
    return hipGetLastError();
}
#endif
hipError_t launch_render(const KernelParams& kp, int cus, hipStream_t st, hipEvent_t ev0, hipEvent_t ev1,
                         hipEvent_t ev2, float4* fb, int* variant_out);
hipError_t launch_render_list(const KernelParams& kp, int cus, hipStream_t st, hipEvent_t ev0, hipEvent_t ev1,
                              int* variant_out);
hipError_t launch_reduce(const KernelParams& kp, float4* fb, hipStream_t st);
hipError_t prepare_radiance(const GpuScene& sc);
uint32_t radiance_grid(const GpuScene& sc, uint64_t items, int cus, int max_workgroups);
hipError_t launch_radiance(const KernelParams& kp, const RayInputs& ri, int cus, int max_workgroups, float4* out,
                           hipStream_t st);
hipError_t launch_gather(const GatherParams& g, hipStream_t st);
hipError_t launch_query(const QueryParams& q, hipStream_t st);
#ifdef MCPT_PHASE_TIMING
void read_lane_use(unsigned long long out[6]);
void read_lane_use_wf(unsigned long long out[6]);
#endif
constexpr int kMaxWfStreams = 4;
struct WfStreams {
    int n;
    hipStream_t st[kMaxWfStreams];
    hipEvent_t fork, join[kMaxWfStreams];
};
struct WfRoute;
hipError_t launch_wavefront(const KernelParams& kp, const WfRoute& route, const WfParams* wf, const WfStreams& ws,
                            hipEvent_t ev0, hipEvent_t ev1, hipEvent_t ev2, float4* fb, int* variant_out);

}
```

montecarlopathtracer_amd/csrc/scene_image.cpp:

```cpp
#include <algorithm>
#include <cmath>
#include <cstdio>

#include "capi_internal.hpp"
#include "half_box.hpp"

using namespace mcpt::host;

mcpt_scene::~mcpt_scene() {
    if (!on_device) return;
    int prev = -1;
    (void)hipGetDevice(&prev);
    (void)hipSetDevice(device);
    (void)hipDeviceSynchronize();
    destroy_comms(*this);
    for (DevBuf* b : buffers())
        if (b->p) (void)hipFree(b->p);
    if (ad_host_n) (void)hipHostFree(ad_host_n);
    for (void* p : retired) (void)hipFree(p);
    for (auto& t : pending) for (auto ev : t.e) (void)hipEventDestroy(ev);
    for (auto& t : free_timing) for (auto ev : t.e) (void)hipEventDestroy(ev);
    if (has_capture_timing) for (auto ev : capture_timing.e) (void)hipEventDestroy(ev);
    for (hipEvent_t ev : {done, start, wf_fork})
        if (ev) (void)hipEventDestroy(ev);
// ... 128 lines not shown
        for (uint32_t i : ord.leaf_order) {
            leaf_begin_new[i] = at;
            for (uint32_t r = 0; r < hs.nodes[i].leaf_count; ++r)
                refs[at++] = 3u * ord.tri_new[hs.leaf_ids[hs.nodes[i].leaf_begin + r]];
        }
    }
    for (uint32_t i = 0; i < nn; ++i) {
        const mcpt::KdNode& n = hs.nodes[i];
        uint32_t w[2];
        if (n.axis) {
            const uint32_t dl = ord.node_new[n.left];
            w[0] = ((n.axis - 1u) << 30) | (boxes ? 3u * ((dl - 1u) / 2u) : dl);
            std::memcpy(&w[1], &n.split, 4);
        } else {
            w[0] = (3u << 30) | leaf_begin_new[i];
            w[1] = n.leaf_count;
        }
        const uint32_t dv = ord.node_new[i];
        if (i == 0) {
            s.gpu.root_w[0] = w[0];
            s.gpu.root_w[1] = w[1];
            if (boxes) continue;
        }
        if (!boxes) {
            std::memcpy(img + off_nodes + size_t(dv + 1) * 8, w, 8);
            continue;
        }
        const size_t m = (dv - 1) / 2, side = (dv - 1) % 2;
        unsigned char* rec = img + off_nodes + m * 48;
        std::memcpy(rec + side * 8, w, 8);
        uint16_t hb[6];
        for (int a = 0; a < 3; ++a) {
            hb[a] = mcpt::f32_to_f16_dir(n.bmin[a], -1);
            hb[3 + a] = mcpt::f32_to_f16_dir(n.bmax[a], +1);
        }
        std::memcpy(rec + 16 + side * 12, hb, 12);
    }
    for (uint32_t g = 0; g < ng; ++g) {
        const mcpt::Geometry& ge = hs.geoms[g];
        mcpt::GpuGeom gg{};
        gg.Ka[0] = ge.Ka.x; gg.Ka[1] = ge.Ka.y; gg.Ka[2] = ge.Ka.z;
        gg.Kd[0] = ge.Kd.x; gg.Kd[1] = ge.Kd.y; gg.Kd[2] = ge.Kd.z;
        gg.Ks[0] = ge.Ks.x; gg.Ks[1] = ge.Ks.y; gg.Ks[2] = ge.Ks.z;
        gg.Ns = ge.Ns; gg.Tr = ge.Tr; gg.Ni = ge.Ni;
        gg.Ns_u = ge.Ns > 0.0f ? (ge.Ns < 4294967040.0f ? static_cast<uint32_t>(ge.Ns) : 0xFFFFFF00u) : 0u;
        std::memcpy(img + off_geoms + size_t(g) * 64, &gg, 64);
    }
    mcpt::GpuScene& gs = s.gpu;
    gs.image_bytes = static_cast<uint32_t>(total);
    gs.off_tris = static_cast<uint32_t>(off_tris);
    gs.off_nodes = static_cast<uint32_t>(off_nodes);
    gs.off_leafs = static_cast<uint32_t>(off_leafs);
    gs.off_geoms = static_cast<uint32_t>(off_geoms);
    gs.node_boxes = boxes ? 1u : 0u;
    gs.n_tris = nt; gs.n_nodes = nn; gs.n_leafs = nl; gs.n_geoms = ng;
    if (nn) {
        for (int a = 0; a < 3; ++a) { gs.root_min[a] = hs.nodes[0].bmin[a]; gs.root_max[a] = hs.nodes[0].bmax[a]; }
    }
    float eb[mcpt::kMaxCullBoxes][6];
    s.n_cull_boxes = static_cast<uint32_t>(mcpt::terminal_cull_boxes(hs, eb, mcpt::kMaxCullBoxes));
    for (uint32_t b = 0; b < s.n_cull_boxes; ++b) {
        uint16_t hb[6];
        for (int a = 0; a < 3; ++a) {
            hb[a] = mcpt::f32_to_f16_dir(eb[b][a], -1);
            hb[3 + a] = mcpt::f32_to_f16_dir(eb[b][3 + a], +1);
        }
        std::memcpy(s.cull_box[b], hb, 12);
    }
    s.n_miss_boxes = static_cast<uint32_t>(mcpt::miss_cull_boxes(hs, s.miss_box, mcpt::kMaxMissBoxes));
    mcpt::direct_list_assign(hs, s.miss_box, static_cast<int>(s.n_miss_boxes), s.tri_box);
    s.direct_counts = 0;
    std::memset(s.direct_list, 0, sizeof s.direct_list);
    std::memset(s.box_tris, 0, sizeof s.box_tris);
    for (uint32_t slot = 0; slot < nt && s.n_miss_boxes; ++slot) {
        const int32_t b = s.tri_box[s.tri_order[slot]];
        if (b < 0) throw mcpt::Error{MCPT_E_INVALID, "a triangle outside every occluder box"};
        if (s.box_tris[b] < mcpt::kDirectK) s.direct_list[size_t(b) * mcpt::kDirectK + s.box_tris[b]] = 3u * slot;
        s.box_tris[b]++;
    }
    for (uint32_t b = 0; b < s.n_miss_boxes; ++b) {
        if (s.box_tris[b] >= 1 && s.box_tris[b] <= mcpt::kDirectK) s.direct_counts |= s.box_tris[b] << (4u * b);
        else std::memset(&s.direct_list[size_t(b) * mcpt::kDirectK], 0, 4 * mcpt::kDirectK);
    }
    s.cull_gain = 0.0f;
    for (const mcpt::Geometry& ge : hs.geoms)
        for (float k : {ge.Kd.x, ge.Kd.y, ge.Kd.z, ge.Ks.x, ge.Ks.y, ge.Ks.z})
            if (std::fabs(k) > s.cull_gain) s.cull_gain = std::fabs(k);
}

void upload(mcpt_scene& s, int device, const std::vector<unsigned char>& image, const std::vector<float>& nrm) {
    HIP_TRY(hipSetDevice(device));
    s.device = device;
    HIP_TRY(hipDeviceGetAttribute(&s.cus, hipDeviceAttributeMultiprocessorCount, s.device));
    s.on_device = true;
    HIP_TRY(hipMalloc(&s.d_image.p, image.size()));
    HIP_TRY(hipMemcpy(s.d_image.p, image.data(), image.size(), hipMemcpyHostToDevice));
    HIP_TRY(hipMalloc(&s.d_normals.p, nrm.size() * 4));
    HIP_TRY(hipMemcpy(s.d_normals.p, nrm.data(), nrm.size() * 4, hipMemcpyHostToDevice));
    s.gpu.image = static_cast<const unsigned char*>(s.d_image.p);
    s.gpu.normals = static_cast<const float4*>(s.d_normals.p);
}

int scene_create_impl(const mcpt_model* m, mcpt_scene** out, bool device, const char* kd_cache_dir = nullptr,
                      int32_t* cache_hit = nullptr, int32_t layout = MCPT_LAYOUT_AUTO,
                      int32_t kd_build = MCPT_KD_BUILD_REFERENCE) {
    return guarded([&]() -> int {
        if (!m || !out) return fail(MCPT_E_INVALID, "NULL argument");
        if (kd_build != MCPT_KD_BUILD_REFERENCE && kd_build != MCPT_KD_BUILD_SAH)
            return fail(MCPT_E_INVALID, "unknown kd_build");
        auto s = std::make_unique<mcpt_scene>();
        int hit = 0;
        mcpt::build_host_scene(m->m, s->hs, kd_cache_dir, &hit, kd_build);
        if (cache_hit) *cache_hit = hit;
        if (s->hs.kd_tris.empty()) return fail(MCPT_E_INVALID, "scene has no triangles");
        if (layout != MCPT_LAYOUT_AUTO && layout != MCPT_LAYOUT_GLOBAL) return fail(MCPT_E_INVALID, "unknown layout");
        build_image(*s, layout == MCPT_LAYOUT_GLOBAL);
        if (device) {
            const size_t nt = s->hs.kd_tris.size();
            std::vector<float> nrm(nt * 12, 0.0f);
            for (size_t k = 0; k < nt; ++k)
                for (int j = 0; j < 3; ++j)
                    for (int c = 0; c < 3; ++c)
                        nrm[12 * k + 4 * j + c] = s->hs.kd_normals[9 * size_t(s->tri_order[k]) + 3 * j + c];
            int cur = 0;
            HIP_TRY(hipGetDevice(&cur));
            const std::vector<int> devs = g_devices.empty() ? std::vector<int>{cur} : g_devices;
            upload(*s, devs[0], s->image, nrm);
            for (size_t i = 1; i < devs.size(); ++i) {
                auto R = std::make_unique<mcpt_scene>();
                R->gpu = s->gpu;
                R->n_cull_boxes = s->n_cull_boxes;
                std::memcpy(R->cull_box, s->cull_box, sizeof s->cull_box);
                R->cull_gain = s->cull_gain;
                R->n_miss_boxes = s->n_miss_boxes;
                std::memcpy(R->miss_box, s->miss_box, sizeof s->miss_box);
                R->direct_counts = s->direct_counts;
                std::memcpy(R->direct_list, s->direct_list, sizeof s->direct_list);
                upload(*R, devs[i], s->image, nrm);
                HIP_TRY(hipStreamCreateWithFlags(&R->stream, hipStreamNonBlocking));
                HIP_TRY(hipEventCreateWithFlags(&R->done, hipEventDisableTiming));
                s->replicas.push_back(std::move(R));
            }
            HIP_TRY(hipSetDevice(devs[0]));
            s->peer_access = g_peer_ok;
        }
        *out = s.release();
        return MCPT_OK;
    });
}

}

extern "C" {

int mcpt_model_create(const mcpt_model_desc* d, mcpt_model** out) {
    return guarded([&]() -> int {
        if (!d || !out) return fail(MCPT_E_INVALID, "NULL argument");
        if (d->n_vertices < 1 || d->n_normals < 1 || d->n_triangles < 1 || d->n_materials < 1 || d->n_groups < 0)
            return fail(MCPT_E_INVALID, "arrays must include the dummy element 0");
        if (!d->vertices || !d->normals || !d->triangles || !d->materials ||
            (d->n_groups > 0 && (!d->group_names || !d->group_offsets || !d->group_tris)))
            return fail(MCPT_E_INVALID, "NULL array");
        auto m = std::make_unique<mcpt_model>();
        mcpt::ObjModel& o = m->m;
        o.path = "<memory>";
        o.vertices.resize(size_t(d->n_vertices));
        for (int64_t i = 0; i < d->n_vertices; ++i)
            o.vertices[size_t(i)] = mcpt::Vec3{d->vertices[3 * i], d->vertices[3 * i + 1], d->vertices[3 * i + 2]};
        o.normals.resize(size_t(d->n_normals));
        for (int64_t i = 0; i < d->n_normals; ++i)
            o.normals[size_t(i)] = mcpt::Vec3{d->normals[3 * i], d->normals[3 * i + 1], d->normals[3 * i + 2]};
        o.n_texcoords = 1;
        o.triangles.resize(size_t(d->n_triangles));
        for (int64_t i = 0; i < d->n_triangles; ++i) {
            const int32_t* t = d->triangles + 10 * i;
            auto& dst = o.triangles[size_t(i)];
            for (int j = 0; j < 3; ++j) { dst.v[j] = t[j]; dst.t[j] = t[3 + j]; dst.n[j] = t[6 + j]; }
            dst.material = t[9];
            if (i > 0 && (t[9] < 0 || t[9] >= d->n_materials)) return fail(MCPT_E_INVALID, "material index out of range");
        }
        o.materials.resize(size_t(d->n_materials));
        for (int64_t i = 0; i < d->n_materials; ++i) {
            const double* q = d->materials + 12 * i;
            auto& mt = o.materials[size_t(i)];
            mt.Ka = mcpt::Vec3{float(q[0]), float(q[1]), float(q[2])};
            mt.Kd = mcpt::Vec3{float(q[3]), float(q[4]), float(q[5])};
            mt.Ks = mcpt::Vec3{float(q[6]), float(q[7]), float(q[8])};
            mt.Ns = q[9]; mt.Tr = q[10]; mt.Ni = q[11];
        }
        for (int64_t g = 0; g < d->n_groups; ++g) {
            const int64_t b = d->group_offsets[g], e = d->group_offsets[g + 1];
            if (b < 0 || e < b) return fail(MCPT_E_INVALID, "bad group offsets");
            auto& dst = o.groups[d->group_names[g] ? d->group_names[g] : ""];
            for (int64_t k = b; k < e; ++k) {
                if (d->group_tris[k] < 1 || d->group_tris[k] >= d->n_triangles)
                    return fail(MCPT_E_INVALID, "group triangle index out of range");
                dst.push_back(d->group_tris[k]);
            }
        }
        *out = m.release();
        return MCPT_OK;
    });
}

int mcpt_model_read_obj(const char* path, mcpt_model** out) {
    return guarded([&]() -> int {
        if (!path || !out) return fail(MCPT_E_INVALID, "path/out is NULL");
        auto m = std::make_unique<mcpt_model>();
        mcpt::read_obj(path, m->m);
        *out = m.release();
        return MCPT_OK;
    });
}

int mcpt_model_read_obj_ex(const char* path, int32_t flavor, mcpt_model** out) {
    return guarded([&]() -> int {
        if (!path || !out) return fail(MCPT_E_INVALID, "path/out is NULL");
        if (flavor != MCPT_OBJ_CVMCTRACER && flavor != MCPT_OBJ_TINYOBJ) return fail(MCPT_E_INVALID, "unknown flavor");
        auto m = std::make_unique<mcpt_model>();
        mcpt::read_obj(path, m->m, flavor);
// ... 55 lines not shown
int mcpt_model_group(const mcpt_model* m, int64_t g, char* name_buf, int64_t name_cap, int64_t* n, int32_t* tris) {
    if (!m || g < 0 || g >= static_cast<int64_t>(m->m.groups.size())) return fail(MCPT_E_INVALID, "bad group index");
    auto it = m->m.groups.begin();
    std::advance(it, g);
    if (name_buf && name_cap > 0) std::snprintf(name_buf, static_cast<size_t>(name_cap), "%s", it->first.c_str());
    if (n) *n = static_cast<int64_t>(it->second.size());
    if (tris && !it->second.empty()) std::memcpy(tris, it->second.data(), it->second.size() * sizeof(int32_t));
    return MCPT_OK;
}

int mcpt_scene_create(const mcpt_model* m, mcpt_scene** out) { return scene_create_impl(m, out, true); }
int mcpt_scene_create_host(const mcpt_model* m, mcpt_scene** out) { return scene_create_impl(m, out, false); }
int mcpt_scene_create_cached(const mcpt_model* m, const char* kd_cache_dir, int32_t host_only, mcpt_scene** out,
                             int32_t* cache_hit) {
    return scene_create_impl(m, out, host_only == 0, kd_cache_dir, cache_hit);
}
int mcpt_scene_create_ex(const mcpt_model* m, const mcpt_scene_options* o, mcpt_scene** out, int32_t* cache_hit) {
    const mcpt_scene_options d{nullptr, 0, MCPT_LAYOUT_AUTO, MCPT_KD_BUILD_REFERENCE};
    if (!o) o = &d;
    const char* dir = o->kd_cache_dir && o->kd_cache_dir[0] ? o->kd_cache_dir : nullptr;
    return scene_create_impl(m, out, o->host_only == 0, dir, cache_hit, o->layout, o->kd_build);
}

void mcpt_scene_destroy(mcpt_scene* s) { delete s; }

int mcpt_scene_get_info(const mcpt_scene* s, mcpt_scene_info* out) {
    if (!s || !out) return fail(MCPT_E_INVALID, "NULL argument");
    out->n_geometries = static_cast<int64_t>(s->hs.geoms.size());
    out->n_triangles = static_cast<int64_t>(s->hs.kd_tris.size());
    out->n_nodes = static_cast<int64_t>(s->hs.nodes.size());
    out->n_leaf_refs = static_cast<int64_t>(s->hs.leaf_ids.size());
    out->kd_depth = s->hs.kd_depth;
    out->lds_bytes = s->gpu.node_boxes ? 0 : s->gpu.image_bytes;
    out->node_boxes = s->gpu.node_boxes;
    out->device = s->device;
    out->n_devices = s->on_device ? 1 + static_cast<int64_t>(s->replicas.size()) : 0;
    out->kd_build = s->hs.kd_build;
    return MCPT_OK;
}

int mcpt_scene_primary_tile_classes(mcpt_scene* s, uint32_t out[4]) {
    if (!s || !out) return MCPT_E_INVALID;
    return guarded([&] {
        out[0] = out[1] = out[2] = 0;
        out[3] = mcpt::kListK;
        if (!s->on_device || !s->ws.small.p) return MCPT_OK;
        set_device(*s);
        HIP_TRY(hipDeviceSynchronize());
        HIP_TRY(hipMemcpy(out, tile_classes(*s), 12, hipMemcpyDeviceToHost));
        return MCPT_OK;
    });
}

int mcpt_scene_terminal_cull_boxes(const mcpt_scene* s) {
    return s ? static_cast<int>(s->n_cull_boxes) : 0;
}

int mcpt_scene_miss_cull_boxes(const mcpt_scene* s, float* boxes) {
    if (!s) return 0;
    if (boxes) std::memcpy(boxes, s->miss_box, sizeof(float) * 6 * s->n_miss_boxes);
    return static_cast<int>(s->n_miss_boxes);
}

int mcpt_scene_direct_lists(const mcpt_scene* s, int32_t* tri_box, uint32_t* box_tris, uint32_t* lists,
                            int32_t* list_kd) {
    if (!s) return 0;
    if (list_kd)
        for (uint32_t b = 0; b < mcpt::kMaxMissBoxes; ++b)
            for (uint32_t j = 0; j < mcpt::kDirectK; ++j) {
                const bool have = j < ((s->direct_counts >> (4u * b)) & 15u);
                list_kd[b * mcpt::kDirectK + j] =
                    have ? static_cast<int32_t>(s->tri_order[s->direct_list[b * mcpt::kDirectK + j] / 3u]) : -1;
            }
    if (tri_box && !s->tri_box.empty()) std::memcpy(tri_box, s->tri_box.data(), 4 * s->tri_box.size());
    if (box_tris) std::memcpy(box_tris, s->box_tris, 4 * mcpt::kMaxMissBoxes);
    if (lists) std::memcpy(lists, s->direct_list, 4 * mcpt::kDirectTableWords);
    return static_cast<int>(mcpt::kDirectK);
}

uint64_t mcpt_scene_direct_rays(const mcpt_scene* s) { return s ? s->direct_rays : 0; }
uint64_t mcpt_scene_extend_rays(const mcpt_scene* s) { return s ? s->extend_rays : 0; }
uint64_t mcpt_scene_clipped_rays(const mcpt_scene* s) { return s ? s->clipped_rays : 0; }
uint64_t mcpt_scene_primary_shaded(const mcpt_scene* s) { return s ? s->primary_shaded : 0; }
uint64_t mcpt_scene_primary_shade_lds(const mcpt_scene* s) {
    if (!s) return 0;
    mcpt::WfFacts f = scene_facts(*s);
    f.lean = true;
    return mcpt::wf_route(f).primary_shade_lds;
}

int mcpt_scene_copy_kd(const mcpt_scene* s, uint32_t* nodes, uint32_t* leaf_ids, int32_t* kd_tris, float* geoms) {
    if (!s) return fail(MCPT_E_INVALID, "NULL scene");
    const auto& hs = s->hs;
    if (nodes)
        for (size_t i = 0; i < hs.nodes.size(); ++i) {
            const auto& n = hs.nodes[i];
            uint32_t* o = nodes + 12 * i;
            o[0] = n.left; o[1] = n.right; o[2] = n.axis;
            std::memcpy(&o[3], &n.split, 4);
            std::memcpy(&o[4], n.bmin, 12);
            std::memcpy(&o[7], n.bmax, 12);
            o[10] = n.leaf_begin; o[11] = n.leaf_count;
        }
    if (leaf_ids && !hs.leaf_ids.empty()) std::memcpy(leaf_ids, hs.leaf_ids.data(), hs.leaf_ids.size() * 4);
    if (kd_tris) std::memcpy(kd_tris, hs.kd_tris.data(), hs.kd_tris.size() * 4);
    if (geoms)
        for (size_t g = 0; g < hs.geoms.size(); ++g) {
            const auto& e = hs.geoms[g];
            float* o = geoms + 14 * g;
            o[0] = e.Ka.x; o[1] = e.Ka.y; o[2] = e.Ka.z; o[3] = e.Kd.x; o[4] = e.Kd.y; o[5] = e.Kd.z;
            o[6] = e.Ks.x; o[7] = e.Ks.y; o[8] = e.Ks.z; o[9] = e.Ns; o[10] = e.Tr; o[11] = e.Ni;
            o[12] = static_cast<float>(e.start); o[13] = static_cast<float>(e.count);
        }
    return MCPT_OK;
}

}
```

montecarlopathtracer_amd/csrc/trace_device.hpp:

```cpp
#pragma once

#include <hip/hip_runtime.h>
#include <stdint.h>

#include "mcpt_device.hpp"
#include "render_launch.hpp"

namespace mcpt {
namespace trace {

using namespace dev;

struct Counters {
    uint32_t rays, paths, inner, leaf, refs, tests, shades, spills;
};

#ifdef MCPT_PHASE_TIMING
struct LaneUse {
    unsigned long long desc_w, desc_l, tri_w, tri_l, burst_w, burst_l;
};
static __device__ LaneUse g_lane_use;
__device__ __forceinline__ void lane_use(unsigned long long& w, unsigned long long& l) {
    const uint64_t ex = __builtin_amdgcn_read_exec();
    if ((threadIdx.x & 63u) == (uint32_t)(__ffsll((unsigned long long)ex) - 1)) {
// ... 152 lines not shown
template <bool EARLY_PRIO = false>
__device__ __forceinline__ void test_tri_pair(RayState& r, const float4 A0, const float4 A1, const float4 A2,
                                              uint32_t ka, const float4 B0, const float4 B1, const float4 B2,
                                              uint32_t kb, bool two) {
    TriDets qa, qb;
    const bool oka = tri_prefilter(r, A0, A1, A2, qa);
    const bool okb = tri_prefilter(r, B0, B1, B2, qb) & two;
    uint32_t prio = 0;
    if constexpr (EARLY_PRIO) prio = oka ? __float_as_uint(A0.w) : __float_as_uint(B0.w);
    if (oka | okb) {
        TriDets q;
        q.detA = oka ? qa.detA : qb.detA;
        q.qb = oka ? qa.qb : qb.qb;
        q.qg = oka ? qa.qg : qb.qg;
        q.qt = oka ? qa.qt : qb.qt;
        if constexpr (!EARLY_PRIO) prio = oka ? __float_as_uint(A0.w) : __float_as_uint(B0.w);
        tri_accept(r, q, prio, oka ? ka : kb);
    }
    if (oka & okb) tri_accept(r, qb, __float_as_uint(B0.w), kb);
}
__device__ __forceinline__ void test_tri(RayState& r, const float4* __restrict__ tris, uint32_t k) {
    test_tri_v(r, tris[k], tris[k + 1], tris[k + 2], k);
}

typedef float f32x4 __attribute__((ext_vector_type(4)));
typedef __attribute__((address_space(3))) f32x4 lds_f32x4;
template <bool IN_LDS>
__device__ __forceinline__ float4 ld_tri(const float4* __restrict__ p) {
    if constexpr (IN_LDS) {
        const f32x4 v = *(const volatile lds_f32x4*)p;
        return make_float4(v.x, v.y, v.z, v.w);
    } else {
        return *p;
    }
}

#ifdef MCPT_PHASE_MARKERS
#define MCPT_MARK(n) asm volatile("s_nop 15\n\ts_nop " #n ::: "memory")
#else
#define MCPT_MARK(n) do {} while (0)
#endif
#ifdef MCPT_PHASE_TIMING
#define MCPT_LU_PARAM , LaneUse& lu
#define MCPT_LU_ARG , lu
#else
#define MCPT_LU_PARAM
#define MCPT_LU_ARG
#endif
#ifndef MCPT_DESCENT_CAP
#define MCPT_DESCENT_CAP 4
#endif
#ifndef MCPT_DESCENT_CAP_GLOBAL
#define MCPT_DESCENT_CAP_GLOBAL 5
#endif
__device__ __forceinline__ float h2f(uint32_t bits16) {
    return (float)__builtin_bit_cast(_Float16, (unsigned short)bits16);
}
__device__ __forceinline__ bool slab_hit(const RayState& r, float lx, float ly, float lz, float hx, float hy,
                                         float hz) {
    const bool nx = __float_as_uint(r.d.x) >> 31, ny = __float_as_uint(r.d.y) >> 31, nz = __float_as_uint(r.d.z) >> 31;
    const float tx0 = ((nx ? hx : lx) - r.o.x) * r.ix, tx1 = ((nx ? lx : hx) - r.o.x) * r.ix;
    const float ty0 = ((ny ? hy : ly) - r.o.y) * r.iy, ty1 = ((ny ? ly : hy) - r.o.y) * r.iy;
    const float tz0 = ((nz ? hz : lz) - r.o.z) * r.iz, tz1 = ((nz ? lz : hz) - r.o.z) * r.iz;
    const float lo = max_qnan(max3_qnan(0.0f, tx0, ty0), tz0);
    const float hi = min_qnan(min3_qnan(r.best, tx1, ty1), tz1);
    return !(lo * kEpsLo > hi * kEpsHi);
}
__device__ __forceinline__ bool box_hit(const RayState& r, uint32_t b0, uint32_t b1, uint32_t b2) {
    const float lx = h2f(b0 & 0xFFFFu), hx = h2f(b1 >> 16);
    const float ly = h2f(b0 >> 16), hy = h2f(b2 & 0xFFFFu);
    const float lz = h2f(b1 & 0xFFFFu), hz = h2f(b2 >> 16);
    return slab_hit(r, lx, ly, lz, hx, hy, hz);
}

__device__ __forceinline__ void box_interval(V3 o, V3 d, V3 inv, float best_init, const float (&b)[6], float& lo,
                                             float& hi) {
    const bool nx = __float_as_uint(d.x) >> 31, ny = __float_as_uint(d.y) >> 31, nz = __float_as_uint(d.z) >> 31;
    const float ax = (b[0] - o.x) * inv.x, bx = (b[3] - o.x) * inv.x;
    const float ay = (b[1] - o.y) * inv.y, by = (b[4] - o.y) * inv.y;
    const float az = (b[2] - o.z) * inv.z, bz = (b[5] - o.z) * inv.z;
    lo = max_qnan(max3_qnan(0.0f, nx ? bx : ax, ny ? by : ay), nz ? bz : az);
    hi = min_qnan(min3_qnan(best_init, nx ? ax : bx, ny ? ay : by), nz ? az : bz);
}
__device__ __forceinline__ uint32_t scene_box_hits(V3 o, V3 d, V3 inv, float best_init,
                                                   const float (&boxes)[kMaxMissBoxes][6], uint32_t n) {
    uint32_t acc = 0;
#pragma unroll 1
    for (uint32_t i = 0; i < n; i++) {
        float lo, hi;
        box_interval(o, d, inv, best_init, boxes[i], lo, hi);
        acc |= !(lo * kEpsLo > hi * kEpsHi) ? 1u << i : 0u;
    }
    return acc;
}

__device__ __forceinline__ bool emitter_reachable(V3 o, V3 d, V3 inv, float best_init,
                                                  const uint32_t (&boxes)[kMaxCullBoxes][3], uint32_t n) {
    RayState r;
    r.o = o;
    r.d = d;
    r.ix = inv.x;
    r.iy = inv.y;
    r.iz = inv.z;
    r.best = best_init;
    bool hit = false;
#pragma unroll 1
    for (uint32_t i = 0; i < n; i++) hit |= box_hit(r, boxes[i][0], boxes[i][1], boxes[i][2]);
    return hit;
}

__device__ __forceinline__ uint4 settle4(uint4 v) {
    asm volatile("v_mov_b32 %0, %0\n\tv_mov_b32 %1, %1\n\tv_mov_b32 %2, %2\n\tv_mov_b32 %3, %3"
                 : "+v"(v.x), "+v"(v.y), "+v"(v.z), "+v"(v.w));
    return v;
}
template <int S, bool LAZY>
__device__ __forceinline__ bool pop_entry(RayState& r, uint4* st, int stride, uint4* __restrict__ spill,
                                          uint32_t spill_stride, const uint4* top = nullptr) {
    const int32_t U = stride * 16;
    if (r.sp == 0) return false;
    r.sp -= U;
    uint4 e;
    if constexpr (LAZY) {
        if (r.sp < r.lo) {
            e = settle4(spill[((uint32_t)r.sp / (uint32_t)U) * spill_stride]);
            r.lo = r.sp;
        } else {
            if (top) e = *top;
            else e = ld4(slot_of<S>(st, stride, r.sp));
        }
    } else {
        lds_uint4* slot = slot_of<S>(st, stride, r.sp);
        if (top) e = *top;
        else e = ld4(slot);
        if (r.sp >= S * U) st4(slot, spill[((uint32_t)r.sp / (uint32_t)U - S) * spill_stride]);
    }
    r.nw0 = e.x;
    r.nw1 = e.y;
    r.tmin = __uint_as_float(e.z);
    r.tmax = __uint_as_float(e.w);
    return !(r.best <= r.tmin * kEpsLo);
}

constexpr uint32_t kLeftMask = 0x3FFFFFFFu;

template <int S, bool BOXES = false, bool COUNT = true>
__device__ __forceinline__ int descend_steps(RayState& r, const uint2* __restrict__ nodes1, uint4* st, int stride,
                                             uint4* __restrict__ spill, uint32_t spill_stride, Counters& c,
                                             const uint4* __restrict__ pairs, int cap MCPT_LU_PARAM) {
    const int32_t U = stride * 16;
    uint32_t& w0 = r.nw0;
    uint32_t& w1 = r.nw1;
    int steps = 0;
    while ((w0 >> 30) != 3u) {
        if (steps == cap) return 0;
        steps++;
        MCPT_MARK(1);
        if constexpr (COUNT) c.inner++;
        MCPT_LANE_USE(desc_w, desc_l, lu);
        const uint32_t left = w0 & kLeftMask;
        uint4 pr, bx0, bx1;
        if constexpr (BOXES) {
            const uint4* rec = pairs + left;
            pr = rec[0];
            bx0 = rec[1];
            bx1 = rec[2];
// ... 364 lines not shown
```

montecarlopathtracer_amd/csrc/wavefront.hip:

```cpp
#include <hip/hip_runtime.h>

#include <cstdlib>

#include "wf_device.hpp"

namespace mcpt {
namespace {

constexpr int kGenBlock = 256;
constexpr int kClassTerminate = 0;

__global__ void __launch_bounds__(kGenBlock) wf_generate(const KernelParams kp, const WfParams wf) {
    const uint32_t n = wf.nb * wf.ns;
    const uint32_t gs = wf.group_shift, gm = (1u << gs) - 1u;
    const V3 eye = v3(kp.eye[0], kp.eye[1], kp.eye[2]);
    Counters c = {0, 0, 0, 0, 0, 0, 0, 0};
    for (uint32_t pid = blockIdx.x * kGenBlock + threadIdx.x; pid < n; pid += gridDim.x * kGenBlock) {
        const uint32_t s_local = pid / wf.nb;
        const uint32_t v = wf.v0 + (pid - s_local * wf.nb);
        const uint32_t grp = pid >> gs, blk = grp / wf.nseg;
        const uint32_t g = seg_of(grp - blk * wf.nseg, blk, wf.nseg, wf.xcd_deal);
        const uint32_t slot = g * wf.seg + (blk << gs) + (pid & gm);
        if (grp < wf.nseg && (pid & gm) == 0u) wf.cnt[g].queued = seg_queue0_len(wf, g);
        int px, py;
        V3 d = v3(0, 0, 0);
        uint32_t depth = kNoRay;
        V3 o = eye;
        if (unit_pixel(kp, v, px, py)) {
            uint32_t sd;
            const uint32_t pix = (uint32_t)py * (uint32_t)kp.width + (uint32_t)px;
            if (kp.mode == kModeQE)
                primary_ray_qe(kp, pix, px, py, wf.s_begin + s_local, sd, o, d);
            else
                primary_ray(kp, pix, px, py, wf.s_begin + s_local, sd, d);
            if (!implicit0(kp, wf))
                stq(&wf.q[0][qf(slot, kQPS, wf.slot_stride)], make_float4(1.0f, 1.0f, 1.0f, __uint_as_float(sd)));
            c.paths++;
            c.rays++;
            depth = 0;
        }
        if (!(MCPT_WF_IMPLICIT0 >= 2 && implicit0(kp, wf))) stq(&wf.q[0][qf(slot, kQO, wf.slot_stride)], pack(o, pid));
        stq(&wf.q[0][qf(slot, kQD, wf.slot_stride)], pack(d, depth));
    }
    flush_counters(c, kp.stats);
}

__global__ void __launch_bounds__(kGenBlock) wf_generate_list(const KernelParams kp, const WfParams wf) {
    const uint32_t n = wf.nb * wf.ns;
    const uint32_t gs = wf.group_shift, gm = (1u << gs) - 1u;
    const V3 eye = v3(kp.eye[0], kp.eye[1], kp.eye[2]);
    Counters c = {0, 0, 0, 0, 0, 0, 0, 0};
    for (uint32_t pid = blockIdx.x * kGenBlock + threadIdx.x; pid < n; pid += gridDim.x * kGenBlock) {
        const uint32_t s_local = pid / wf.nb;
        const uint32_t v = kp.pixel_list[wf.v0 + (pid - s_local * wf.nb)];
        const uint32_t grp = pid >> gs, blk = grp / wf.nseg;
        const uint32_t g = seg_of(grp - blk * wf.nseg, blk, wf.nseg, wf.xcd_deal);
        const uint32_t slot = g * wf.seg + (blk << gs) + (pid & gm);
        if (grp < wf.nseg && (pid & gm) == 0u) wf.cnt[g].queued = seg_queue0_len(wf, g);
        int px, py;
        V3 d = v3(0, 0, 0);
        uint32_t depth = kNoRay, sd = 0;
        if (unit_pixel(kp, v, px, py)) {
            primary_ray(kp, (uint32_t)py * (uint32_t)kp.width + (uint32_t)px, px, py, wf.s_begin + s_local, sd, d);
            c.paths++;
            c.rays++;
            depth = 0;
        }
        stq(&wf.q[0][qf(slot, kQO, wf.slot_stride)], pack(eye, pid));
        stq(&wf.q[0][qf(slot, kQD, wf.slot_stride)], pack(d, depth));
        stq(&wf.q[0][qf(slot, kQPS, wf.slot_stride)], make_float4(1.0f, 1.0f, 1.0f, __uint_as_float(sd)));
    }
    flush_counters(c, kp.stats);
}

template <int LAY, int S, int BLOCK, bool COUNT>
__global__ void __launch_bounds__(BLOCK, (LAY == kLayGlobal && !COUNT && MCPT_WF_GLOBAL_WAVES)
                                             ? MCPT_WF_GLOBAL_WAVES
                                             : (LAY == kLayLds && !COUNT && MCPT_WF_LDS_WPE
                                                    ? MCPT_WF_LDS_WPE : 1))
wf_extend(const KernelParams kp, const WfParams wf) {
    constexpr bool IN_LDS = LAY != kLayGlobal;
    extern __shared__ __attribute__((aligned(16))) unsigned char smem[];
    const uint32_t g = blockIdx.x;
    WfCounters* cn = wf.cnt + (size_t)wf.bounce * wf.nseg + g;
    const uint32_t count = g < wf.nseg ? cn->queued : 0u;
    if (count == 0) {
        if (g < wf.nseg && threadIdx.x == 0) cn->hits = 0;
        return;
    }
    const int tid = (int)threadIdx.x;
    const GpuScene& sc = kp.scene;
    unsigned char* const lds_image = smem + (size_t)S * BLOCK * 16;
    uint32_t* const lslot = reinterpret_cast<uint32_t*>(lds_image + (IN_LDS ? sc.image_bytes : 0u));
    if (tid == 0) *lslot = 0;
    const SceneView sv = open_scene<IN_LDS, BLOCK>(lds_image, sc, tid);
    constexpr bool CLIP = LAY == kLayLds && !COUNT;
    uint32_t dtab = 0, dcnt = 0;
    if constexpr (CLIP) {
        asm volatile("s_mov_b32 %0, %1" : "=s"(dcnt) : "s"(wf.direct_counts));
        asm volatile("s_mov_b32 %0, %1" : "=s"(dtab) : "s"((sc.image_bytes + (uint32_t)kLdsCounterBytes - sc.off_leafs) / 4u));
        if (dcnt && tid < (int)(kDirectLdsBytes / 4))
            (lslot + kLdsCounterBytes / 4)[tid] = tid < (int)kDirectTableWords ? wf.direct_list[tid] : 0u;
    }
    uint32_t unl = 0, nclip = 0, csel = 0;
    if constexpr (CLIP) asm volatile("s_mov_b32 %0, %1" : "=s"(unl) : "s"(unlisted_boxes(wf.direct_counts)));
    __syncthreads();
    uint4* st = reinterpret_cast<uint4*>(smem) + tid;
    uint4* spill = kp.spill + (blockIdx.x * BLOCK + (uint32_t)tid);
    const uint32_t spill_stride = kp.total_lanes;
    const size_t seg0 = (size_t)g * wf.seg;
    float4* qb = wf.q[wf.bounce & 1];
    const uint32_t qs = wf.slot_stride;

    Counters c = {0, 0, 0, 0, 0, 0, 0, 0};
#ifdef MCPT_PHASE_TIMING
    LaneUse lu = {0, 0, 0, 0, 0, 0};
#endif
    SlotCursor cur_chunk = {0, kChunk};
    RayState r;
    r.htri = -1;
    int mode = kDead;
    constexpr bool PF = LAY != kLayGlobal || MCPT_WF_GLOBAL_PREFETCH;
    uint32_t slot = cur_chunk.take(true, lslot), depth = 0;
    uint32_t nslot = PF ? cur_chunk.take(true, lslot) : 0u;
    float4 no4 = make_float4(0, 0, 0, 0), nd4 = make_float4(0, 0, 0, 0);
    auto start = [&](float4 o4, float4 d4) {
        r.o = v3(opaque(o4.x), opaque(o4.y), opaque(o4.z));
        r.d = v3(opaque(d4.x), opaque(d4.y), opaque(d4.z));
        depth = __float_as_uint(d4.w);
        const bool live = begin_ray(r, sc, kp.best_init);
        if constexpr (CLIP) {
            csel = depth == kNoRay ? 0u : depth >> kDirectShift;
            const uint32_t um = csel & unl;
            const V3 inv = v3(r.ix, r.iy, r.iz);
            float clo = kFltMax, chi = 0.0f;
#pragma unroll 1
            for (uint32_t i = 0; i < wf.n_miss_boxes; i++) {
                const bool mine = ((um >> i) & 1u) != 0u;
                if (((unl >> i) & 1u) != 0u && __ballot(mine)) {
                    float lo, hi;
                    box_interval(r.o, r.d, inv, kp.best_init, wf.miss_box[i], lo, hi);
                    clo = mine ? min_qnan(clo, lo) : clo;
                    chi = mine ? max_qnan(chi, hi) : chi;
                }
            }
            const bool sel = csel != 0u;
            const float t0 = max_qnan(r.tmin, clo * kEpsLo);
            const float t1 = min_qnan(r.tmax, (chi * kEpsHi) * kEpsHi);
            const bool walk = !(t0 > t1);
            const uint32_t lm = csel & ~unl;
            const bool hasl = lm != 0u;
            const uint32_t lb = (uint32_t)(__ffs((int)lm) - 1) & 7u;
            const uint32_t lp = dtab + lb * kDirectK;
            r.lpos = hasl ? lp : 0u;
            r.lend = hasl ? lp + ((dcnt >> (4u * lb)) & 15u) : 0u;
            r.tmin = sel ? t0 : r.tmin;
            r.tmax = sel ? t1 : r.tmax;
            if (hasl & walk) {
                st4(slot_of<S>(st, BLOCK, 0), make_uint4(r.nw0, r.nw1, __float_as_uint(t0), __float_as_uint(t1)));
                r.sp = BLOCK * 16;
            }
            mode = (depth != kNoRay && live && (!sel | hasl | walk)) ? kTrav : kReady;
            return;
        }
        mode = (depth != kNoRay && live) ? kTrav : kReady;
    };
#ifdef MCPT_PHASE_TIMING
    unsigned long long tm_setup = 0, tm_trav = 0, tm_hand = 0, tm_iters = 0, tm_hands = 0,
                       tm_t0 = __builtin_amdgcn_s_memtime();
#define WF_STAMP(acc) do { unsigned long long t1_ = __builtin_amdgcn_s_memtime(); acc += t1_ - tm_t0; tm_t0 = t1_; } while (0)
#else
#define WF_STAMP(acc) do {} while (0)
#endif
    int refill;
    asm volatile("s_mov_b32 %0, %1" : "=s"(refill) : "s"(wf.refill_thresh));
    const bool eye0 = MCPT_WF_IMPLICIT0 >= 2 && wf.bounce == 0 && eye_origins0(kp);
    const float4 eye4 = make_float4(kp.eye[0], kp.eye[1], kp.eye[2], 0.0f);
    auto ld_o = [&](uint32_t sl) { return eye0 ? eye4 : ldq(&qb[qf(seg0 + sl, kQO, qs)]); };
    if (slot < count) start(ld_o(slot), ldq(&qb[qf(seg0 + slot, kQD, qs)]));
    if constexpr (CLIP) nclip += (uint32_t)__popcll(__ballot(slot < count && csel != 0u));
    if (PF && nslot < count) { no4 = ld_o(nslot); nd4 = ldq(&qb[qf(seg0 + nslot, kQD, qs)]); }
    WF_STAMP(tm_setup);
    for (;;) {
        __builtin_amdgcn_s_setprio(MCPT_WF_EXT_PRIO);
        for (;;) {
#ifdef MCPT_PHASE_TIMING
            tm_iters++;
            {
                const uint64_t tv = __ballot(mode == kTrav);
                if ((threadIdx.x & 63u) == 0) { lu.burst_w += 1; lu.burst_l += (unsigned long long)__popcll(tv); }
            }
#endif
            MCPT_MARK(5);
            if (mode == kTrav) {
                if (trav_iter<S, !IN_LDS, COUNT, LAY == kLayLds, IN_LDS ? kWfLdsCap : MCPT_WF_DESCENT_CAP_GLOBAL>(
                        r, sv.tris, sv.nodes, sv.leafs, st, BLOCK, spill, spill_stride, c MCPT_LU_ARG, sv.pairs))
                    mode = kReady;
            }
            MCPT_MARK(6);
            const uint64_t trv = __ballot(mode == kTrav);
            const uint64_t rdy = __ballot(mode == kReady);
            if (!trv || (int)__popcll(rdy) >= refill) break;
        }
        WF_STAMP(tm_trav);
#ifdef MCPT_PHASE_TIMING
        tm_hands++;
#endif
        MCPT_MARK(7);
        __builtin_amdgcn_s_setprio(MCPT_WF_EXT_PRIO + 1);
        if constexpr (PF) {
            no4 = make_float4(opaque(no4.x), opaque(no4.y), opaque(no4.z), opaque(no4.w));
            nd4 = make_float4(opaque(nd4.x), opaque(nd4.y), opaque(nd4.z), opaque(nd4.w));
        }
        const bool fin = mode == kReady;
        const uint32_t ns0 = PF ? 0u : cur_chunk.take(fin, lslot);
        const uint32_t fslot = slot;
        csel = 0u;
        if (fin) {
            const int32_t hid = r.htri;
            if constexpr (PF) {
                slot = nslot;
                start(no4, nd4);
            } else {
                slot = ns0;
                float4 o4 = make_float4(0, 0, 0, 0), d4 = make_float4(0, 0, 0, __uint_as_float(kNoRay));
                if (slot < count) { o4 = ld_o(slot); d4 = ldq(&qb[qf(seg0 + slot, kQD, qs)]); }
                start(o4, d4);
            }
            if (slot >= count) mode = kDead;
            reinterpret_cast<int32_t*>(qb + qf(0, kQHIT, qs))[seg0 + fslot] = hid;
        }
        if constexpr (CLIP) nclip += (uint32_t)__popcll(__ballot(fin && mode != kDead && csel != 0u));
        if constexpr (PF) {
            const bool want = fin && mode != kDead;
            const uint32_t ns = cur_chunk.take(want, lslot);
            if (want) {
                nslot = ns;
                if (nslot < count) { no4 = ld_o(nslot); nd4 = ldq(&qb[qf(seg0 + nslot, kQD, qs)]); }
            }
        }
        WF_STAMP(tm_hand);
        MCPT_MARK(8);
        if (!__ballot(mode != kDead)) break;
    }
#ifdef MCPT_PHASE_TIMING
    if ((threadIdx.x & 63u) == 0) {
        atomicAdd(kp.stats + 8, tm_setup);
        atomicAdd(kp.stats + 9, tm_trav);
        atomicAdd(kp.stats + 10, tm_hand);
        atomicAdd(kp.stats + 11, tm_iters);
        atomicAdd(kp.stats + 12, tm_hands);
    }
    {
        unsigned long long* gl = reinterpret_cast<unsigned long long*>(&g_lane_use);
        const unsigned long long v[6] = {lu.desc_w, lu.desc_l, lu.tri_w, lu.tri_l, lu.burst_w, lu.burst_l};
        for (int i = 0; i < 6; i++) {
            unsigned long long x = v[i];
            for (int off = 32; off > 0; off >>= 1) x += __shfl_xor(x, off);
            if ((threadIdx.x & 63u) == 0) atomicAdd(gl + i, x);
        }
    }
#endif
    flush_counters(c, kp.stats);
    if (tid == 0 && wf.bounce > 0) atomicAdd(kp.stats + kStatExtend, (unsigned long long)count);
    if constexpr (CLIP)
        if ((tid & 63) == 0 && nclip) atomicAdd(kp.stats + kStatClipped, (unsigned long long)nclip);
    if (tid == 0) cn->hits = count;
}

template <int BLOCK, bool GEO_LDS, bool SORTB>
__global__ void __launch_bounds__(BLOCK, 6)
wf_shade_slots(const KernelParams kp, const WfParams wf) {
    const uint32_t g = blockIdx.x;
    if (g >= wf.nseg) return;
    __shared__ uint32_t lnext;
    __shared__ uint32_t lcls[SORTB ? 8 : 1];
    __shared__ uint16_t lperm[SORTB ? BLOCK : 1];
    if (SORTB && threadIdx.x < 8) lcls[threadIdx.x] = 0;
    extern __shared__ __attribute__((aligned(16))) GpuGeom lgeo[];
    const WfCounters* cn = wf.cnt + (size_t)wf.bounce * wf.nseg + g;
    WfCounters* nx = wf.cnt + (size_t)(wf.bounce + 1) * wf.nseg + g;
    __shared__ uint32_t ltail;
    const uint32_t head = cn->hits;
    const uint32_t total = head + cn->resolved;
    const uint32_t tail0 = wf.seg - total;
    if (threadIdx.x == 0) ltail = 0;
    __shared__ uint32_t ltake;
    if (threadIdx.x == 0) ltake = 0;
    auto slot_at = [&](uint32_t i) { return i < head ? i : tail0 + i; };
    const GpuScene& sc = kp.scene;
    if (threadIdx.x == 0) lnext = 0;
    if constexpr (GEO_LDS) {
        const uint4* src = reinterpret_cast<const uint4*>(sc.image + sc.off_geoms);
        uint4* dst = reinterpret_cast<uint4*>(lgeo);
        for (uint32_t i = threadIdx.x; i < sc.n_geoms * 4u; i += BLOCK) dst[i] = src[i];
    }
    __shared__ __attribute__((aligned(16))) float4 ldrec[kDirectTableWords * 3];
    __shared__ uint32_t ldk[kDirectTableWords];
    if (wf.direct_counts && threadIdx.x < kDirectTableWords * 3u) {
        const uint32_t e = threadIdx.x / 3u;
        uint32_t k = 0;
#pragma unroll
        for (uint32_t b = 0; b < kDirectTableWords; b++) k = e == b ? wf.direct_list[b] : k;
        ldrec[threadIdx.x] = open_scene<false, BLOCK>(nullptr, sc, 0).tris[k + (threadIdx.x - 3u * e)];
        if (threadIdx.x == 3u * e) ldk[e] = k;
    }
    const uint32_t unlisted = unlisted_boxes(wf.direct_counts);
    __syncthreads();
    const SceneView sv = open_scene<false, BLOCK>(nullptr, sc, 0);
    const float4* tris = sv.tris;
    const GpuGeom* geoms = GEO_LDS ? lgeo : sv.geoms;
    const size_t seg0 = (size_t)g * wf.seg;
    const float4* qb = wf.q[wf.bounce & 1];
    float4* qb2 = wf.q[(wf.bounce + 1) & 1];
    const uint32_t qs = wf.slot_stride;
    const bool qe = kp.mode == kModeQE;
    const bool imp = wf.bounce == 0 && implicit0(kp, wf);
    const int lane = (int)(threadIdx.x & 63u);
    Counters c = {0, 0, 0, 0, 0, 0, 0, 0};
    uint32_t ndirect = 0;
    uint32_t par = 0;
    const int32_t tdepth = (qe ? 3 : 1) * kp.max_depth;
    bool carry = false;
    uint32_t nchain = 0;
    bool drained = false;
    int32_t rhit = -1;
    uint32_t pid = 0, depth = kNoRay, sd = 0;
    V3 o = v3(0, 0, 0), d = v3(0, 0, 0), color = v3(0, 0, 0);
    for (uint32_t base = 0;; base += BLOCK) {
        uint32_t i = total;
        if constexpr (SORTB) {
            if (base >= total) break;
            i = base + threadIdx.x;
        } else {
            const uint64_t fr = ~__ballot(carry);
            if (!drained && fr) {
                const int leader = __ffsll((unsigned long long)fr) - 1;
                const uint32_t nf = (uint32_t)__popcll(fr);
                uint32_t b0 = 0;
                if (lane == leader) b0 = atomicAdd(&ltake, nf);
                b0 = lane_bcast(b0, leader);
                drained = b0 + nf >= total;
                if (!carry && b0 < total) i = b0 + (uint32_t)__popcll(fr & ((1ull << lane) - 1ull));
            }
            if (!__ballot(carry || i < total)) break;
        }
        if constexpr (SORTB) {
            uint32_t k = 4u;
            if (i < total) {
                const size_t js = seg0 + slot_at(i);
// ... 167 lines not shown
    const double m0 = 1e-3 * ext;
    const float4* tris = open_scene<false, kCandBlock>(nullptr, sc, 0).tris;
    uint32_t* rec = wf.tile_cand + (size_t)tile * kListRecWords;
    uint32_t n = 0;
    for (uint32_t i0 = 0; i0 < sc.n_tris; i0 += 64u) {
        const uint32_t i = i0 + lane;
        bool keep = false;
        if (i < sc.n_tris) {
            const float4 A0 = tris[3u * i], A1 = tris[3u * i + 1u], A2 = tris[3u * i + 2u];
            uint32_t out = 0x1Fu;
            for (int k = 0; k < 3; k++) {
                double p[3] = {(double)A0.x, (double)A0.y, (double)A0.z};
                if (k == 1) { p[0] -= (double)A1.x; p[1] -= (double)A1.y; p[2] -= (double)A1.z; }
                if (k == 2) { p[0] -= (double)A2.x; p[1] -= (double)A2.y; p[2] -= (double)A2.z; }
                for (int a = 0; a < 3; a++) p[a] -= (double)kp.eye[a];
                const double m = m0 + sqrt(p[0] * p[0] + p[1] * p[1] + p[2] * p[2]) * (1.0 / 65536.0);
                for (int q = 0; q < 5; q++)
                    if (!(pn[q][0] * p[0] + pn[q][1] * p[1] + pn[q][2] * p[2] < -m)) out &= ~(1u << q);
            }
            keep = out == 0u;
        }
        const uint64_t mk = __ballot(keep);
        if (keep) {
            const uint32_t pos = n + (uint32_t)__popcll(mk & ((1ull << lane) - 1ull));
            if (pos < kListK) rec[1u + pos] = 3u * i;
        }
        n += (uint32_t)__popcll(mk);
    }
    if (lane == 0) {
        rec[0] = n;
        atomicAdd(&wf.tile_classes[n == 0u ? 0 : (n <= kListK ? 1 : 2)], 1u);
    }
}

__global__ void __launch_bounds__(256) wf_accumulate(const KernelParams kp, const WfParams wf) {
    const uint32_t u = blockIdx.x * 256u + threadIdx.x;
    if (u >= wf.nb) return;
    const uint32_t j = blockIdx.y;
    V3 part = v3(0, 0, 0);
    for (uint32_t s = j * wf.nsc; s < (j + 1u) * wf.nsc; s++)
        part = vadd(part, xyz(wf.radiance[(size_t)s * wf.nb + u]));
    kp.partial[(size_t)(wf.chunk_index + j) * kp.npix_local + wf.v0 + u] = make_float4(part.x, part.y, part.z, 0.0f);
}

template <int BLOCK>
auto shade_kernel(bool geo_lds, bool sortb) {
    return sortb ? (geo_lds ? wf_shade_slots<BLOCK, true, true> : wf_shade_slots<BLOCK, false, true>)
                 : (geo_lds ? wf_shade_slots<BLOCK, true, false> : wf_shade_slots<BLOCK, false, false>);
}

template <int LAY, int S, int BLOCK>
hipError_t launch_extend(const KernelParams& kp, const WfParams& wf, int grid, size_t lds, hipStream_t st) {
    auto kern = kp.lean ? wf_extend<LAY, S, BLOCK, false> : wf_extend<LAY, S, BLOCK, true>;
    return launch_dyn_lds(kern, dim3(grid), dim3(BLOCK), lds, st, kp, wf);
}

}

#ifdef MCPT_PHASE_TIMING
void read_lane_use_wf(unsigned long long out[6]) {
    LaneUse z = {0, 0, 0, 0, 0, 0};
    (void)hipMemcpyFromSymbol(out, HIP_SYMBOL(g_lane_use), sizeof z);
    (void)hipMemcpyToSymbol(HIP_SYMBOL(g_lane_use), &z, sizeof z);
}
#endif

namespace {

struct WfBatch {
    const WfRoute& route;
    KernelParams kp;
    WfParams wf;
    hipStream_t st;
    bool lists;
};

hipError_t launch_generate(const WfBatch& b) {
    const uint32_t n = b.wf.nb * b.wf.ns, gen_grid = (n + kGenBlock - 1) / kGenBlock, cap = 16u * (uint32_t)b.route.cus;
    hipLaunchKernelGGL(b.kp.pixel_list ? wf_generate_list : wf_generate, dim3(gen_grid < cap ? gen_grid : cap),
                       dim3(kGenBlock), 0, b.st, b.kp, b.wf);
    return hipGetLastError();
}

enum class Extend { kPrimaryShade, kPrimaryLists, kPacket, kLds, kGlobal };
Extend extend_form(const WfRoute& r, int bounce, bool lists) {
    if (bounce == 0 && lists) return r.primary_shade ? Extend::kPrimaryShade : Extend::kPrimaryLists;
    if (bounce == 0 && r.packet) return Extend::kPacket;
    return r.in_lds ? Extend::kLds : Extend::kGlobal;
}
hipError_t launch_bounce(const WfBatch& b, bool* shaded) {
    const WfRoute& r = b.route;
    const WfParams& wf = b.wf;
    const Extend form = extend_form(r, wf.bounce, b.lists);
    *shaded = form == Extend::kPrimaryShade;
    switch (form) {
        case Extend::kPrimaryShade: return launch_wavefront_primary_shade(b.kp, wf, (int)r.nseg, r.primary_shade_lds, b.st);
        case Extend::kPrimaryLists: return launch_wavefront_primary_lists(b.kp, wf, (int)r.nseg, r.packet_lds, b.st);
        case Extend::kPacket: return launch_wavefront_primary(b.kp, wf, (int)r.nseg, r.packet_lds, b.st);
        case Extend::kLds: return launch_extend<kLayLds, 4, kLdsBlock>(b.kp, wf, (int)r.nseg, r.extend_lds, b.st);
        default: return launch_extend<kLayGlobal, MCPT_WF_GLOBAL_S, kGlobalBlock>(b.kp, wf, (int)r.nseg, r.extend_lds, b.st);
    }
}

hipError_t launch_shade(const WfBatch& b, int streams) {
    const WfRoute& r = b.route;
    const bool geo = r.geo_lds != 0, sortb = b.wf.sort != 0;
    const int block = wf_shade_block(r, streams);
    auto kern = block == 1024 ? shade_kernel<1024>(geo, sortb)
                : block == MCPT_WF_SHADE_LDS_BLOCK ? shade_kernel<MCPT_WF_SHADE_LDS_BLOCK>(geo, sortb)
                                                   : shade_kernel<256>(geo, sortb);
    hipLaunchKernelGGL(kern, dim3(r.nseg), dim3(block), r.geo_lds, b.st, b.kp, b.wf);
    return hipGetLastError();
}

hipError_t launch_batch(WfBatch& b, int streams, uint32_t ncb) {
    const WfRoute& r = b.route;
    hipError_t e = hipMemsetAsync(b.wf.cnt, 0, sizeof(WfCounters) * (size_t)r.nseg * (size_t)(r.queries + 1), b.st);
    if (e == hipSuccess && r.generate) e = launch_generate(b);
    for (int bounce = 0; bounce < r.queries && e == hipSuccess; bounce++) {
        bool shaded = false;
        b.wf.bounce = bounce;
        e = launch_bounce(b, &shaded);
        if (e == hipSuccess && !shaded) e = launch_shade(b, streams);
        if (e == hipSuccess && bounce + 1 == r.cull_bounce) {
            b.wf.bounce = bounce + 1;
            hipLaunchKernelGGL(wf_cull_terminal, dim3(r.nseg), dim3(kCullBlock), 0, b.st, b.kp, b.wf);
            e = hipGetLastError();
        }
    }
    if (e != hipSuccess) return e;
    hipLaunchKernelGGL(wf_accumulate, dim3((b.wf.nb + 255u) / 256u, ncb), dim3(256), 0, b.st, b.kp, b.wf);
    return hipGetLastError();
}

}

hipError_t launch_wavefront(const KernelParams& kp_in, const WfRoute& route, const WfParams* wf_in, const WfStreams& ws,
                            hipEvent_t ev0, hipEvent_t ev1, hipEvent_t ev2, float4* fb, int* variant_out) {
    KernelParams kp = kp_in;
    kp.total_lanes = (uint32_t)total_lanes_for(kp.scene, route.cus);
    const int ns = ws.n < 1 ? 1 : (ws.n > kMaxWfStreams ? kMaxWfStreams : ws.n);
    const hipStream_t st = ws.st[0];
    hipError_t e = hipSuccess;
    if (ev0 && (e = hipEventRecord(ev0, st)) != hipSuccess) return e;
    if (!kp.npix_local) {
        if (ev1 && (e = hipEventRecord(ev1, st)) != hipSuccess) return e;
        if (ev2 && (e = hipEventRecord(ev2, st)) != hipSuccess) return e;
        if (variant_out) *variant_out = route.variant;
        return hipSuccess;
    }
    const bool lists = route.can_list && any_whole_tile_batch(kp, wf_in[0].capacity, route.whole);
    if (lists) {
        const uint32_t tiles = kp.npix_local >> 6;
        hipLaunchKernelGGL(wf_tile_candidates, dim3((tiles + kCandBlock / 64 - 1) / (kCandBlock / 64)),
                           dim3(kCandBlock), 0, st, kp, wf_in[0]);
        if ((e = hipGetLastError()) != hipSuccess) return e;
    }
    if (ns > 1) {
        if ((e = hipEventRecord(ws.fork, st)) != hipSuccess) return e;
        for (int i = 1; i < ns; i++)
            if ((e = hipStreamWaitEvent(ws.st[i], ws.fork, 0)) != hipSuccess) return e;
    }
    uint32_t batch = 0;
    wf_for_each_batch(kp, wf_in[0].capacity, route.whole, [&](const WfSpan& span, uint32_t chunk0, uint32_t v0) {
        const int h = (int)(batch++ % (uint32_t)ns);
        WfBatch b{route, kp, wf_batch_params(wf_in[h], route, kp, span, chunk0, v0), ws.st[h], false};
        b.kp.spill = kp.spill + (size_t)h * 32 * kp.total_lanes;
        b.lists = lists && whole_tiles(b.wf.v0, b.wf.nb);
        if (b.lists) b.wf.tile_cand = wf_in[0].tile_cand;
        e = launch_batch(b, ns, span.ncb);
        return e == hipSuccess;
    });
    for (int i = 1; i < ns; i++) {
        hipError_t j = hipEventRecord(ws.join[i], ws.st[i]);
        if (j == hipSuccess) j = hipStreamWaitEvent(st, ws.join[i], 0);
        if (e == hipSuccess) e = j;
    }
    if (e != hipSuccess) return e;
    if (ev1 && (e = hipEventRecord(ev1, st)) != hipSuccess) return e;
    if (fb) e = launch_reduce(kp, fb, st);
    if (e == hipSuccess && ev2) e = hipEventRecord(ev2, st);
    if (variant_out) *variant_out = route.variant;
// ... 5 lines not shown
```

montecarlopathtracer_amd/csrc/wf_device.hpp:

```cpp
#pragma once

#include <hip/hip_runtime.h>

#include <cstdint>

#include "mcpt_device.hpp"
#include "render_launch.hpp"
#include "trace_device.hpp"
#include "wf_route.hpp"

namespace mcpt {

using namespace dev;
using namespace trace;

hipError_t launch_wavefront_primary(const KernelParams& kp, const WfParams& wf, int grid, size_t lds,
                                    hipStream_t st);
hipError_t launch_wavefront_primary_lists(const KernelParams& kp, const WfParams& wf, int grid, size_t lds,
                                          hipStream_t st);
hipError_t launch_wavefront_primary_shade(const KernelParams& kp, const WfParams& wf, int grid, size_t lds,
                                          hipStream_t st);

namespace {

constexpr uint32_t kNoRay = 0xFFFFFFFFu;
__device__ __forceinline__ uint32_t ray_depth(uint32_t w) { return w == kNoRay ? w : (w & kDepthMask); }

__device__ __forceinline__ uint32_t unlisted_boxes(uint32_t direct_counts) {
    uint32_t m = 0;
#pragma unroll
    for (uint32_t b = 0; b < (uint32_t)kMaxMissBoxes; b++) m |= ((direct_counts >> (4u * b)) & 15u) ? 0u : 1u << b;
    return direct_counts ? m : 0u;
}

__device__ __forceinline__ bool terminal_ray_adds(bool qe, V3 o, V3 d, float best_init,
                                                  const uint32_t (&boxes)[kMaxCullBoxes][3], uint32_t n) {
    if (qe) return false;
    return emitter_reachable(o, d, v3(1.0f / d.x, 1.0f / d.y, 1.0f / d.z), best_init, boxes, n);
}

constexpr uint32_t kCarryMax = 1;

__device__ __forceinline__ float4 pack(V3 v, uint32_t w) { return make_float4(v.x, v.y, v.z, __uint_as_float(w)); }

__device__ __forceinline__ size_t qf(uint32_t slot, uint32_t k, uint32_t stride) {
    return (size_t)k * stride + slot;
}
constexpr uint32_t kQO = 0, kQD = 1, kQPS = 2, kQHIT = 3;
__device__ __forceinline__ V3 xyz(float4 v) { return v3(v.x, v.y, v.z); }

#ifndef MCPT_WF_NT
#define MCPT_WF_NT 3
#endif
typedef float f32x4 __attribute__((ext_vector_type(4)));
__device__ __forceinline__ float4 ldq(const float4* p) {
#if MCPT_WF_NT & 1
    const f32x4 v = __builtin_nontemporal_load(reinterpret_cast<const f32x4*>(p));
    return make_float4(v.x, v.y, v.z, v.w);
#else
    return *p;
#endif
}
__device__ __forceinline__ void stq(float4* p, float4 v) {
#if MCPT_WF_NT & 2
    const f32x4 x = {v.x, v.y, v.z, v.w};
    __builtin_nontemporal_store(x, reinterpret_cast<f32x4*>(p));
#else
    *p = v;
#endif
}

#ifndef MCPT_WF_XCD
#define MCPT_WF_XCD 1
#endif
__device__ __forceinline__ uint32_t seg_of(uint32_t k, uint32_t b, uint32_t nseg, bool xcd) {
    const uint32_t rot = (MCPT_WF_XCD && xcd && (nseg & 7u) == 0u)
                             ? (uint32_t)(((uint64_t)(b * 2654435761u) * (nseg >> 3)) >> 32) << 3
                             : (uint32_t)(((uint64_t)(b * 2654435761u) * nseg) >> 32);
    const uint32_t g = k + rot;
    return g >= nseg ? g - nseg : g;
}

__device__ __forceinline__ uint32_t slot_pid(const WfParams& wf, uint32_t g, uint32_t j) {
    const uint32_t gs = wf.group_shift, blk = j >> gs;
    const uint32_t rot = seg_of(0, blk, wf.nseg, wf.xcd_deal);
    const uint32_t k = g >= rot ? g - rot : g + wf.nseg - rot;
    return ((blk * wf.nseg + k) << gs) | (j & ((1u << gs) - 1u));
}

__device__ __forceinline__ uint32_t seg_queue0_len(const WfParams& wf, uint32_t g) {
    const uint32_t n = wf.nb * wf.ns;
    const uint32_t gs = wf.group_shift, gm = (1u << gs) - 1u;
    const uint32_t ngroups = (n + gm) >> gs;
    const uint32_t full = ngroups / wf.nseg, rem = ngroups - full * wf.nseg;
    const uint32_t k = (g + wf.nseg - seg_of(0, full, wf.nseg, wf.xcd_deal)) % wf.nseg;
    uint32_t len = (full + (k < rem ? 1u : 0u)) << gs;
    const uint32_t lb = (ngroups - 1u) / wf.nseg;
    if (seg_of(ngroups - 1u - lb * wf.nseg, lb, wf.nseg, wf.xcd_deal) == g) len -= (ngroups << gs) - n;
    return len;
}

__host__ __device__ __forceinline__ bool eye_origins0(const KernelParams& kp) {
    return MCPT_WF_IMPLICIT0 && kp.mode != kModeQE;
}
// ... 35 lines not shown
```

montecarlopathtracer_amd/csrc/wf_route.hpp:

```cpp
#pragma once

#include "render_launch.hpp"

#ifndef MCPT_WF_PACKET0
#define MCPT_WF_PACKET0 1
#endif
#ifndef MCPT_WF_GEN0
#define MCPT_WF_GEN0 1
#endif
#ifndef MCPT_WF_IMPLICIT0
#define MCPT_WF_IMPLICIT0 2
#endif
#ifndef MCPT_WF_GLOBAL_S
#define MCPT_WF_GLOBAL_S 6
#endif
#ifndef MCPT_WF_SHADE_LDS_BLOCK
#define MCPT_WF_SHADE_LDS_BLOCK 512
#endif
#ifndef MCPT_WF_GEO_LDS
#define MCPT_WF_GEO_LDS 1
#endif

namespace mcpt {

constexpr size_t kLdsPerCu = 160 * 1024;
constexpr size_t kShadeStaticLds = kDirectShadeLds + 64;

inline bool direct_lists_fit(uint32_t image_bytes, uint32_t node_boxes) {
    return !node_boxes && lds_bytes_counted_in_lds(image_bytes, 4) + kShadeStaticLds + kDirectLdsBytes <= kMaxLds;
}

struct WfFacts {
    const GpuScene* scene;
    uint32_t n_miss_boxes, direct_counts, n_cull_boxes;
    int cus;
    bool lean, sort, qe;
    bool listed;
    bool default_batch;
    bool tile_records;
    int tile, max_depth;
    uint32_t group_shift;
};

struct WfRoute {
    int cus;
    bool in_lds;
    uint32_t nseg;
    int variant;
    int queries;
    int terminal;
    uint32_t n_miss_boxes;
    uint32_t direct_counts;
    uint32_t n_cull_boxes;
    bool direct;
    bool shade_cull;
    bool carry;
    bool packet;
    bool generate;
    bool can_list;
    bool whole;
    bool primary_shade;
    int cull_bounce;
    uint32_t group_shift, xcd_deal;
    size_t packet_lds, extend_lds, direct_lds, primary_shade_lds, geo_lds;
};

inline WfRoute wf_route(const WfFacts& f) {
    const GpuScene& sc = *f.scene;
    WfRoute r{};
    r.cus = f.cus;
    r.in_lds = scene_in_lds(sc);
    r.nseg = uint32_t(f.cus) * (r.in_lds ? 1u : uint32_t(kWfGlobalSegsPerCu));
    r.variant = r.in_lds ? 4 : 5;
    r.queries = (f.qe ? 3 : 1) * f.max_depth + 1;
    r.terminal = r.queries - 1;
    r.n_miss_boxes = f.lean ? f.n_miss_boxes : 0u;
    r.direct = r.n_miss_boxes && f.direct_counts && direct_lists_fit(sc.image_bytes, sc.node_boxes);
    r.direct_counts = r.direct ? f.direct_counts : 0u;
    r.n_cull_boxes = f.n_cull_boxes;
    r.shade_cull = f.lean && r.in_lds && !f.sort && r.n_miss_boxes != 0;
    r.carry = r.shade_cull && r.direct;
    r.group_shift = r.in_lds ? 6u : f.group_shift;
    r.xcd_deal = r.in_lds ? 0u : 1u;
    r.packet = MCPT_WF_PACKET0 && MCPT_WF_IMPLICIT0 >= 2 && r.in_lds && !f.qe && !f.listed;
    r.generate = !(r.packet && MCPT_WF_GEN0);
    r.can_list = r.packet && MCPT_WF_GEN0 && f.lean && f.tile == 8 && sc.n_tris <= kListMaxTris && f.tile_records;
    r.whole = r.can_list && f.default_batch;
    r.primary_shade = r.can_list && r.shade_cull;
    r.cull_bounce = (f.lean && !r.shade_cull && r.terminal >= 1 && (f.qe || f.n_cull_boxes)) ? r.terminal : -1;
    r.packet_lds = r.in_lds ? lds_bytes_counted_in_lds(sc.image_bytes, 4) : 0;
    r.direct_lds = r.direct ? kDirectLdsBytes : 0;
    r.extend_lds = r.in_lds ? r.packet_lds + r.direct_lds : lds_bytes_global(MCPT_WF_GLOBAL_S, true);
    r.primary_shade_lds = r.in_lds ? r.packet_lds + r.direct_lds : 0;
    const size_t ext_cu = r.in_lds ? r.extend_lds : kWfGlobalSegsPerCu * r.extend_lds;
    const size_t geo = 64 * size_t(sc.n_geoms);
    r.geo_lds = (MCPT_WF_GEO_LDS && ext_cu + kShadeStaticLds + geo <= kLdsPerCu) ? geo : 0;
    return r;
}

inline int wf_shade_block(const WfRoute& r, int streams) {
    return r.in_lds ? (streams == 1 ? 1024 : MCPT_WF_SHADE_LDS_BLOCK) : 256;
}

struct WfSpan {
    uint32_t nsc, ncb, nb_max;
};
inline WfSpan wf_span(const KernelParams& kp, uint32_t capacity, uint32_t chunk, bool whole) {
    WfSpan s;
    s.nsc = (kp.spp - chunk * kp.chunk) < kp.chunk ? (kp.spp - chunk * kp.chunk) : kp.chunk;
    s.ncb = 1;
    if (s.nsc == kp.chunk && (uint64_t)kp.npix_local * kp.chunk <= capacity) {
        const uint32_t full = (kp.spp / kp.chunk) - chunk;
        const uint32_t fit = (uint32_t)(capacity / ((uint64_t)kp.npix_local * kp.chunk));
        s.ncb = fit < full ? fit : full;
    }
    s.nb_max = capacity / (s.ncb * s.nsc);
    if (whole && s.nb_max >= 64u && s.nb_max < kp.npix_local) s.nb_max &= ~63u;
    return s;
}
template <typename F>
void wf_for_each_batch(const KernelParams& kp, uint32_t capacity, bool whole, F&& fn) {
    for (uint32_t chunk = 0; chunk < kp.nchunks;) {
        const WfSpan s = wf_span(kp, capacity, chunk, whole);
        for (uint32_t v0 = 0; v0 < kp.npix_local; v0 += s.nb_max)
            if (!fn(s, chunk, v0)) return;
        chunk += s.ncb;
    }
}
inline WfParams wf_batch_params(const WfParams& of_stream, const WfRoute& r, const KernelParams& kp, const WfSpan& span,
                                uint32_t chunk0, uint32_t v0) {
    WfParams wf = of_stream;
    wf.chunk_index = chunk0;
    wf.s_begin = chunk0 * kp.chunk;
    wf.nsc = span.nsc;
    wf.ns = span.ncb * span.nsc;
    wf.v0 = v0;
    wf.nb = (kp.npix_local - v0) < span.nb_max ? (kp.npix_local - v0) : span.nb_max;
    const uint32_t n = wf.nb * wf.ns;
    wf.seg = ((((n + (1u << r.group_shift) - 1u) >> r.group_shift) + r.nseg - 1) / r.nseg) << r.group_shift;
    return wf;
}
inline bool whole_tiles(uint32_t v0, uint32_t nb) { return (v0 & 63u) == 0u && (nb & 63u) == 0u; }
inline bool any_whole_tile_batch(const KernelParams& kp, uint32_t capacity, bool whole) {
    for (uint32_t chunk = 0; chunk < kp.nchunks;) {
        const WfSpan s = wf_span(kp, capacity, chunk, whole);
        chunk += s.ncb;
        const uint32_t last_v0 = (kp.npix_local - 1u) / s.nb_max * s.nb_max;
        if ((s.nb_max & 63u) == 0u || whole_tiles(last_v0, kp.npix_local - last_v0)) return true;
    }
    return false;
}

}
```

montecarlopathtracer_amd/tracer.py:

```python
from __future__ import annotations

import ctypes as C
import os
from dataclasses import dataclass, field
from typing import Optional, Sequence

import numpy as np

from . import _capi
from ._capi import McptError, RenderParamsC, RenderStats, check, lib

IMG_WIDTH = 800
IMG_HEIGHT = 600
NUM_KERNELS = 100
NUM_SAMPLES_PER_KERNEL = 100
ILLUM = 10.0
DEFAULT_SEED = 0x4D435054


def _fptr(a):
    return a.ctypes.data_as(C.POINTER(C.c_float))


class ObjModel:
# ... 184 lines not shown
        if self.packed or self.shard_count > 1:
            return int(lib().mcpt_shard_pixel_count(C.byref(self.to_c())))
        return int(self.width) * int(self.height)

    def shard_pixels(self) -> np.ndarray:
        p = self.to_c()
        n = int(check(lib().mcpt_shard_pixel_count(C.byref(p))))
        xy = np.zeros((n, 2), np.int32)
        check(lib().mcpt_shard_pixels(C.byref(p), xy.ctypes.data_as(C.POINTER(C.c_int32))))
        return xy


class Scene:

    LAYOUTS = {"auto": _capi.LAYOUT_AUTO, "global": _capi.LAYOUT_GLOBAL}
    KD_BUILDS = {"reference": _capi.KD_BUILD_REFERENCE, "sah": _capi.KD_BUILD_SAH}

    def __init__(self, model: ObjModel, host_only: bool = False, kd_cache: Optional[str] = None,
                 layout: str = "auto", kd_build: str = "reference"):
        if layout not in self.LAYOUTS:
            raise ValueError(f"layout must be one of {sorted(self.LAYOUTS)}")
        if kd_build not in self.KD_BUILDS:
            raise ValueError(f"kd_build must be one of {sorted(self.KD_BUILDS)}")
        h = C.c_void_p()
        if kd_cache:
            os.makedirs(kd_cache, exist_ok=True)
        opt = _capi.SceneOptions(os.fsencode(kd_cache) if kd_cache else None, int(host_only), self.LAYOUTS[layout],
                                 self.KD_BUILDS[kd_build])
        hit = C.c_int32(0)
        check(lib().mcpt_scene_create_ex(model.handle, C.byref(opt), C.byref(h), C.byref(hit)))
        self.cache_hit = bool(hit.value)
        self._h = h
        self.host_only = host_only

    def close(self):
        h = getattr(self, "_h", None)
        if h is not None and _capi._lib is not None:
            _capi._lib.mcpt_scene_destroy(h)
        self._h = None

    __del__ = close

    @property
    def handle(self):
        if self._h is None:
            raise McptError(-1, "scene destroyed")
        return self._h

    def info(self) -> dict:
        i = _capi.SceneInfo()
        check(lib().mcpt_scene_get_info(self.handle, C.byref(i)))
        d = {n: int(getattr(i, n)) for n, _ in i._fields_}
        d["terminal_cull_boxes"] = int(lib().mcpt_scene_terminal_cull_boxes(self.handle))
        d["miss_cull_boxes"] = int(lib().mcpt_scene_miss_cull_boxes(self.handle, None))
        bt = np.zeros(8, np.uint32)
        k = int(lib().mcpt_scene_direct_lists(self.handle, None, bt.ctypes.data_as(C.POINTER(C.c_uint32)), None, None))
        d["direct_list_k"] = k
        d["direct_list_boxes"] = int(((bt >= 1) & (bt <= k)).sum()) if k else 0
        return d

    def miss_cull_boxes(self) -> np.ndarray:
        b = np.zeros((16, 6), np.float32)
        n = int(lib().mcpt_scene_miss_cull_boxes(self.handle, _fptr(b)))
        return b[:n]

    def direct_lists(self) -> dict:
        n = int(lib().mcpt_scene_miss_cull_boxes(self.handle, None))
        nt = self.info()["n_triangles"]
        tri_box = np.full(max(nt, 1), -1, np.int32)
        box_tris = np.zeros(8, np.uint32)
        lists = np.zeros(8 * 16, np.uint32)
        list_kd = np.full(8 * 16, -1, np.int32)
        k = int(lib().mcpt_scene_direct_lists(self.handle, tri_box.ctypes.data_as(C.POINTER(C.c_int32)),
                                              box_tris.ctypes.data_as(C.POINTER(C.c_uint32)),
                                              lists.ctypes.data_as(C.POINTER(C.c_uint32)),
                                              list_kd.ctypes.data_as(C.POINTER(C.c_int32))))
        box_tris = box_tris[:n] if k else box_tris[:0]
        counts = np.where(box_tris <= k, box_tris, 0).astype(np.uint32)
        return {"k": k, "tri_box": tri_box[:nt] if k else tri_box[:0], "box_tris": box_tris,
                "lists": lists[: 8 * k].reshape(8, k)[: len(box_tris)] if k else lists[:0].reshape(0, 0),
                "list_kd": list_kd[: 8 * k].reshape(8, k)[: len(box_tris)] if k else list_kd[:0].reshape(0, 0),
                "counts": counts}

    def _render_stats(self, st) -> dict:
        d = st.as_dict()
        d["direct_rays"] = int(lib().mcpt_scene_direct_rays(self.handle))
        d["extend_rays"] = int(lib().mcpt_scene_extend_rays(self.handle))
        d["clipped_rays"] = int(lib().mcpt_scene_clipped_rays(self.handle))
        d["primary_shaded"] = int(lib().mcpt_scene_primary_shaded(self.handle))
        return d

    def primary_tile_classes(self):
        out = (C.c_uint32 * 4)()
        check(lib().mcpt_scene_primary_tile_classes(self.handle, out))
        return {"empty": int(out[0]), "listed": int(out[1]), "walked": int(out[2]), "k": int(out[3])}

    def kd(self):
        i = self.info()
        nodes = np.zeros((i["n_nodes"], 12), np.uint32)
        leafs = np.zeros(max(i["n_leaf_refs"], 1), np.uint32)
        kdt = np.zeros(i["n_triangles"], np.int32)
        geoms = np.zeros((i["n_geometries"], 14), np.float32)
        check(lib().mcpt_scene_copy_kd(self.handle, nodes.ctypes.data_as(C.POINTER(C.c_uint32)),
                                       leafs.ctypes.data_as(C.POINTER(C.c_uint32)),
                                       kdt.ctypes.data_as(C.POINTER(C.c_int32)), _fptr(geoms)))
        return nodes, leafs[: i["n_leaf_refs"]], kdt, geoms

    def render(self, params: RenderParams, fb: Optional[np.ndarray] = None):
        n = params.output_pixels()
        if fb is None:
            fb = np.zeros((n, 3) if (params.packed or params.shard_count > 1) else (params.height, params.width, 3),
                          np.float32)
        if fb.dtype != np.float32 or not fb.flags.c_contiguous or fb.size != 3 * n:
            raise McptError(-1, "fb must be a C-contiguous float32 array with 3 floats per output pixel")
        st = RenderStats()
        check(lib().mcpt_render(self.handle, C.byref(params.to_c()), _fptr(fb), C.byref(st)))
        return fb, self._render_stats(st)

    def intersect(self, o: np.ndarray, d: np.ndarray, t_max: float = 3.402823466e38):
        o = np.ascontiguousarray(o, np.float32).reshape(-1, 3)
        d = np.ascontiguousarray(d, np.float32).reshape(-1, 3)
        if o.shape != d.shape:
            raise McptError(-1, "o and d must have the same shape")
        n = o.shape[0]
        tri = np.zeros(n, np.int32)
        hit = np.zeros((n, 3), np.float32)
        st = RenderStats()
        check(lib().mcpt_intersect(self.handle, n, _fptr(o), _fptr(d), C.c_float(t_max),
                                   tri.ctypes.data_as(C.POINTER(C.c_int32)), _fptr(hit), C.byref(st)))
        return tri, hit, st.as_dict()

    def trace_device(self, n: int, o_ptr: int, d_ptr: int, tri_ptr: int, hit_ptr: int = 0, t_max_ptr: int = 0,
                     stream_ptr: int = 0, **params):
        check(lib().mcpt_trace_device(self.handle, C.byref(trace_params(**params)), int(n), C.c_void_p(o_ptr),
                                      C.c_void_p(d_ptr), C.c_void_p(t_max_ptr), C.c_void_p(tri_ptr),
                                      C.c_void_p(hit_ptr), C.c_void_p(stream_ptr)))

    def occluded_device(self, n: int, o_ptr: int, d_ptr: int, occluded_ptr: int, t_max_ptr: int = 0,
                        stream_ptr: int = 0, **params):
        check(lib().mcpt_occluded_device(self.handle, C.byref(trace_params(**params)), int(n), C.c_void_p(o_ptr),
                                         C.c_void_p(d_ptr), C.c_void_p(t_max_ptr), C.c_void_p(occluded_ptr),
                                         C.c_void_p(stream_ptr)))

    def occluded(self, o: np.ndarray, d: np.ndarray, t_max=None, **params):
        o = np.ascontiguousarray(o, np.float32).reshape(-1, 3)
        d = np.ascontiguousarray(d, np.float32).reshape(-1, 3)
        if o.shape != d.shape:
            raise McptError(-1, "o and d must have the same shape")
        n = o.shape[0]
        tm = None
        if t_max is not None and np.ndim(t_max) == 0:
            params = {**params, "t_max": float(t_max)}
        elif t_max is not None:
            tm = np.ascontiguousarray(t_max, np.float32).reshape(-1)
            if tm.shape[0] != n:
                raise McptError(-1, "t_max must hold one value per ray")
        occ = np.zeros(n, np.uint8)
        st = RenderStats()
        check(lib().mcpt_occluded(self.handle, C.byref(trace_params(**params)), n, _fptr(o), _fptr(d),
                                  _fptr(tm) if tm is not None else None, occ.ctypes.data_as(C.POINTER(C.c_uint8)),
                                  C.byref(st)))
        return occ, st.as_dict()

    def trace_stats(self) -> dict:
        st = RenderStats()
        check(lib().mcpt_trace_stats_read(self.handle, C.byref(st)))
        return st.as_dict()

    def reserve_rays(self):
        check(lib().mcpt_scene_reserve_rays(self.handle))

    def radiance_device(self, n: int, o_ptr: int, d_ptr: int, out_ptr: int, stream_ids_ptr: int = 0,
# ... 288 lines not shown
```

Before: 26800 Mray/s.

## Add bounding-sphere clip for unlisted miss boxes in wavefront extend

Computes, on the host, a bounding sphere around the triangles assigned to each unlisted miss-cull box. The wavefront extend kernel then intersects the ray with that sphere to tighten the clip interval or skip the kd walk when the ray misses. It moves the extend kernel body into a new header and source with a SPHERE template variant, and adds a counter for skipped rays. The goal is to cut kd traversal work for rays that pass through a box without reaching its geometry, at the cost of extra per-ray sphere math and some register pressure.

```diff
diff --git a/include/mcpt.h b/include/mcpt.h
--- a/include/mcpt.h
+++ b/include/mcpt.h
@@ -190,6 +190,8 @@
 uint64_t mcpt_scene_extend_rays(const mcpt_scene* s);
 uint64_t mcpt_scene_clipped_rays(const mcpt_scene* s);
 uint64_t mcpt_scene_primary_shaded(const mcpt_scene* s);
+uint32_t mcpt_scene_clip_spheres(const mcpt_scene* s, float* spheres);
+uint64_t mcpt_scene_sphere_skips(const mcpt_scene* s);
 uint64_t mcpt_scene_primary_shade_lds(const mcpt_scene* s);
 int mcpt_scene_primary_tile_classes(mcpt_scene* s, uint32_t out[4]);
 int mcpt_scene_copy_kd(const mcpt_scene* s, uint32_t* nodes, uint32_t* leaf_ids,
diff --git a/montecarlopathtracer_amd/_build.py b/montecarlopathtracer_amd/_build.py
--- a/montecarlopathtracer_amd/_build.py
+++ b/montecarlopathtracer_amd/_build.py
@@ -12,18 +12,19 @@
 LIB = os.path.join(LIBDIR, os.environ.get("MCPT_LIB_NAME", "libmcpt.so"))
 SOURCES = ["host_model.cpp", "kd_cache.cpp", "capi.cpp", "scene_image.cpp", "plan.cpp", "render_host.cpp", "queries.cpp",
            "render.hip", "wavefront.hip", "wavefront_primary.hip", "wavefront_primary_shade.hip",
-           "aov.hip", "denoise.hip", "variance.hip", "denoise_var.hip", "adaptive.hip", "rayquery.hip"]
+           "wavefront_sphere.hip", "aov.hip", "denoise.hip", "variance.hip", "denoise_var.hip", "adaptive.hip", "rayquery.hip"]
 _WF_FLAGS = ["-mllvm", "-amdgpu-set-wave-priority=1", "-mllvm", "-two-entry-phi-node-folding-threshold=8",
              "-mllvm", "-unroll-threshold=2000"]
 SOURCE_FLAGS = {"wavefront_primary.hip": ["-mllvm", "-structurizecfg-skip-uniform-regions=1"] + _WF_FLAGS,
                 "wavefront_primary_shade.hip": _WF_FLAGS,
                 "wavefront.hip": _WF_FLAGS,
+                "wavefront_sphere.hip": _WF_FLAGS,
                 "rayquery.hip": _WF_FLAGS,
                 "render.hip": ["-mllvm", "-enable-gvn-hoist", "-mllvm", "-unroll-threshold=2000"]}
 SOURCE_SCHED = {"wavefront_primary_shade.hip": "iterative-minreg"}
 HEADERS = ["capi_internal.hpp", "staging.hpp", "host_model.hpp", "mcpt_device.hpp", "render_launch.hpp", "wf_route.hpp", "trace_device.hpp", "half_box.hpp",
            "aov_device.hpp", "aov_launch.hpp", "variance_launch.hpp", "adaptive_launch.hpp", "partial_sum.hpp", "rayquery_launch.hpp",
-           "wf_device.hpp", "wf_primary_body.hpp", "wf_primary_walk.hpp", "wf_primary_pairs.hpp", "wf_primary_shade_body.hpp", "wf_shade_item.hpp"]
+           "wf_device.hpp", "wf_extend_body.hpp", "wf_primary_body.hpp", "wf_primary_walk.hpp", "wf_primary_pairs.hpp", "wf_primary_shade_body.hpp", "wf_shade_item.hpp"]
 ARCH = os.environ.get("MCPT_OFFLOAD_ARCH", "gfx950")
 
 COMMON = ["-O3", "-std=c++17", "-fPIC", "-ffp-contract=off", "-fno-fast-math", "-fno-slp-vectorize", "-Wall",
diff --git a/montecarlopathtracer_amd/_capi.py b/montecarlopathtracer_amd/_capi.py
--- a/montecarlopathtracer_amd/_capi.py
+++ b/montecarlopathtracer_amd/_capi.py
@@ -163,6 +163,8 @@
     "mcpt_scene_extend_rays": (C.c_uint64, [_vp]),
     "mcpt_scene_clipped_rays": (C.c_uint64, [_vp]),
     "mcpt_scene_primary_shaded": (C.c_uint64, [_vp]),
+    "mcpt_scene_clip_spheres": (C.c_uint32, [_vp, C.POINTER(C.c_float)]),
+    "mcpt_scene_sphere_skips": (C.c_uint64, [_vp]),
     "mcpt_scene_primary_shade_lds": (C.c_uint64, [_vp]),
     "mcpt_scene_copy_kd": (C.c_int, [_vp, C.POINTER(C.c_uint32), C.POINTER(C.c_uint32), C.POINTER(C.c_int32),
                                      C.POINTER(C.c_float)]),
diff --git a/montecarlopathtracer_amd/csrc/capi_internal.hpp b/montecarlopathtracer_amd/csrc/capi_internal.hpp
--- a/montecarlopathtracer_amd/csrc/capi_internal.hpp
+++ b/montecarlopathtracer_amd/csrc/capi_internal.hpp
@@ -111,6 +111,10 @@
     uint64_t extend_rays = 0;
     uint64_t clipped_rays = 0;
     uint64_t primary_shaded = 0;
+    uint32_t clip_spheres = 0;
+    float clip_sphere[mcpt::kMaxMissBoxes][4] = {};
+    uint64_t sphere_skips = 0;
+    bool sphere_clipped = false;
     mcpt::host::DevBuf d_image, d_normals;
     mcpt::host::Workspace ws;
     std::vector<mcpt::host::Timing> pending, free_timing;
diff --git a/montecarlopathtracer_amd/csrc/host_model.cpp b/montecarlopathtracer_amd/csrc/host_model.cpp
--- a/montecarlopathtracer_amd/csrc/host_model.cpp
+++ b/montecarlopathtracer_amd/csrc/host_model.cpp
@@ -607,6 +607,53 @@
             if (in) tri_box[k] = b;
         }
     }
+}
+
+uint32_t clip_spheres(const HostScene& hs, const float (*boxes)[6], int n_boxes, const std::vector<int32_t>& tri_box,
+                      uint32_t want, double margin, double max_reach, float (*spheres)[4]) {
+    const size_t nt = hs.kd_verts.size() / 9;
+    double smin[3] = {INFINITY, INFINITY, INFINITY}, smax[3] = {-INFINITY, -INFINITY, -INFINITY};
+    for (size_t k = 0; k < nt; ++k)
+        for (int j = 0; j < 9; ++j) {
+            const double v = hs.kd_verts[9 * k + j];
+            smin[j % 3] = std::min(smin[j % 3], v);
+            smax[j % 3] = std::max(smax[j % 3], v);
+        }
+    double diag2 = 0.0;
+    for (int a = 0; a < 3; ++a) diag2 += (smax[a] - smin[a]) * (smax[a] - smin[a]);
+    uint32_t mask = 0;
+    for (int b = 0; b < n_boxes; ++b) {
+        for (int a = 0; a < 4; ++a) spheres[b][a] = 0.0f;
+        if (!((want >> b) & 1u) || tri_box.size() != nt) continue;
+        float c[3];
+        double half2 = 0.0;
+        for (int a = 0; a < 3; ++a) {
+            c[a] = (boxes[b][a] + boxes[b][3 + a]) * 0.5f;
+            const double h = std::max(double(boxes[b][3 + a]) - c[a], double(c[a]) - boxes[b][a]);
+            half2 += h * h;
+        }
+        double r2 = -1.0;
+        for (size_t k = 0; k < nt; ++k) {
+            if (tri_box[k] != b) continue;
+            for (int j = 0; j < 3; ++j) {
+                double d2 = 0.0;
+                for (int a = 0; a < 3; ++a) {
+                    const double d = double(hs.kd_verts[9 * k + 3 * j + a]) - c[a];
+                    d2 += d * d;
+                }
+                r2 = std::max(r2, d2);
+            }
+        }
+        if (!(r2 > 0.0) || !std::isfinite(r2) || !std::isfinite(half2)) continue;
+        const double r = std::sqrt(r2) * (1.0 + margin);
+        if (!(r * r < half2) || !(diag2 <= max_reach * max_reach * r * r)) continue;
+        float r2f = static_cast<float>(r * r);
+        if (double(r2f) < r * r) r2f = std::nextafter(r2f, INFINITY);
+        if (!std::isfinite(r2f) || !std::isfinite(c[0]) || !std::isfinite(c[1]) || !std::isfinite(c[2])) continue;
+        spheres[b][0] = c[0]; spheres[b][1] = c[1]; spheres[b][2] = c[2]; spheres[b][3] = r2f;
+        mask |= 1u << b;
+    }
+    return mask;
 }
 
 namespace {
diff --git a/montecarlopathtracer_amd/csrc/host_model.hpp b/montecarlopathtracer_amd/csrc/host_model.hpp
--- a/montecarlopathtracer_amd/csrc/host_model.hpp
+++ b/montecarlopathtracer_amd/csrc/host_model.hpp
@@ -69,6 +69,8 @@
 int terminal_cull_boxes(const HostScene& hs, float (*boxes)[6], int max_boxes);
 int miss_cull_boxes(const HostScene& hs, float (*boxes)[6], int max_boxes);
 void direct_list_assign(const HostScene& hs, const float (*boxes)[6], int n_boxes, std::vector<int32_t>& tri_box);
+uint32_t clip_spheres(const HostScene& hs, const float (*boxes)[6], int n_boxes, const std::vector<int32_t>& tri_box,
+                      uint32_t want, double margin, double max_reach, float (*spheres)[4]);
 bool kd_cache_load(const std::string& dir, const std::vector<float>& tri_verts, std::vector<KdNode>& nodes,
                    std::vector<uint32_t>& leaf_ids, int& depth, int kd_build = 0);
 bool kd_cache_store(const std::string& dir, const std::vector<float>& tri_verts, const std::vector<KdNode>& nodes,
diff --git a/montecarlopathtracer_amd/csrc/plan.cpp b/montecarlopathtracer_amd/csrc/plan.cpp
--- a/montecarlopathtracer_amd/csrc/plan.cpp
+++ b/montecarlopathtracer_amd/csrc/plan.cpp
@@ -157,7 +157,10 @@
 size_t launched_lanes(const mcpt_scene& s) { return static_cast<size_t>(mcpt::total_lanes_for(s.gpu, s.cus)); }
 
 mcpt::WfFacts scene_facts(const mcpt_scene& s) {
-    return mcpt::WfFacts{&s.gpu, s.n_miss_boxes, s.direct_counts, s.n_cull_boxes, s.cus};
+    mcpt::WfFacts f{&s.gpu, s.n_miss_boxes, s.direct_counts, s.n_cull_boxes, s.cus};
+    f.clip_spheres = s.clip_spheres;
+    f.clip_sphere = s.clip_sphere;
+    return f;
 }
 
 size_t spill_bytes(const mcpt_scene& s, int sets) { return size_t(sets) * kSpillEntries * launched_lanes(s) * 16; }
diff --git a/montecarlopathtracer_amd/csrc/render_host.cpp b/montecarlopathtracer_amd/csrc/render_host.cpp
--- a/montecarlopathtracer_amd/csrc/render_host.cpp
+++ b/montecarlopathtracer_amd/csrc/render_host.cpp
@@ -104,6 +104,7 @@
     HIP_TRY(hipMemsetAsync(tile_classes(s), 0, 16, st));
     const Timing t = acquire_timing(s, pl.capturing);
     if (pl.pipeline == MCPT_PIPELINE_WAVEFRONT) {
+        s.sphere_clipped = s.sphere_clipped || pl.route.clip.mask != 0;
         HIP_TRY(mcpt::launch_wavefront(pl.kp, pl.route, R.wf, wf_streams_on(s, pl.sets(), st), t.e[0], t.e[1], t.e[2],
                                        reinterpret_cast<float4*>(d_fb), &s.last_variant));
     } else {
@@ -135,11 +136,18 @@
     s.extend_rays = 0;
     s.clipped_rays = 0;
     s.primary_shaded = 0;
+    s.sphere_skips = 0;
     if (s.ws.small.p) {
         unsigned long long st[mcpt::kStatSlots];
         char* const block = static_cast<char*>(s.ws.small.p) + 64;
         HIP_TRY(hipMemcpy(st, block, sizeof st, hipMemcpyDeviceToHost));
         HIP_TRY(hipMemset(block, 0, sizeof st));
+        if (s.sphere_clipped) {
+            unsigned long long skips = 0;
+            HIP_TRY(hipMemcpy(&skips, block + 8 * mcpt::kStatSphereSkips, 8, hipMemcpyDeviceToHost));
+            HIP_TRY(hipMemset(block + 8 * mcpt::kStatSphereSkips, 0, 8));
+            s.sphere_skips = skips;
+        }
         HIP_TRY(hipStreamSynchronize(nullptr));
         if (st[8] | st[9] | st[10] | st[11])
             std::fprintf(stderr, "mcpt phase cycles (sum over waves): units %llu trav %llu shade %llu burst_iters %llu "
@@ -270,6 +278,7 @@
         s.extend_rays += R->extend_rays;
         s.clipped_rays += R->clipped_rays;
         s.primary_shaded += R->primary_shaded;
+        s.sphere_skips += R->sphere_skips;
         r.kernel_ms = std::max(r.kernel_ms, q.kernel_ms);
         r.reduce_ms = std::max(r.reduce_ms, q.reduce_ms);
     }
@@ -425,6 +434,7 @@
             k.pixel_list = aw.list;
             HIP_TRY(hipMemsetAsync(tile_classes(s), 0, 16, st));
             t = acquire_timing(s, false);
+            s.sphere_clipped = s.sphere_clipped || R.pl.route.clip.mask != 0;
             HIP_TRY(mcpt::launch_wavefront(k, R.pl.route, R.wf, wf_streams_on(s, R.pl.sets(), st), t.e[0], t.e[1],
                                            nullptr, nullptr, &s.last_variant));
         } else {
diff --git a/montecarlopathtracer_amd/csrc/render_launch.hpp b/montecarlopathtracer_amd/csrc/render_launch.hpp
--- a/montecarlopathtracer_amd/csrc/render_launch.hpp
+++ b/montecarlopathtracer_amd/csrc/render_launch.hpp
@@ -38,7 +38,11 @@
 static_assert(kMaxMissBoxes <= 8, "the clip walk's selector is one byte of box bits");
 constexpr int kStatClipped = 15;
 constexpr int kStatPrimaryShaded = 16;
+constexpr double kSphereMargin = 1.0 / 1024.0;
+constexpr double kSphereMaxReach = 256.0;
 constexpr int kStatSlots = 17;
+constexpr int kStatSphereSkips = kStatSlots + 3;
+static_assert(64 + 8 * (kStatSphereSkips + 1) <= 256, "the scene's small block (plan.cpp prepare_workspace)");
 
 struct GpuGeom {
     float Ka[3], Kd[3], Ks[3];
@@ -168,6 +172,10 @@
     uint32_t direct_list[kDirectTableWords];
     uint32_t shade_cull;
 };
+struct SphereClip {
+    uint32_t mask;
+    float sphere[kMaxMissBoxes][4];
+};
 
 inline size_t lds_bytes_in_lds(uint32_t image_bytes, int S) { return (size_t)image_bytes + (size_t)S * kLdsBlock * 16; }
 constexpr size_t kLdsCounterBytes = 32;
diff --git a/montecarlopathtracer_amd/csrc/scene_image.cpp b/montecarlopathtracer_amd/csrc/scene_image.cpp
--- a/montecarlopathtracer_amd/csrc/scene_image.cpp
+++ b/montecarlopathtracer_amd/csrc/scene_image.cpp
@@ -234,6 +234,11 @@
         if (s.box_tris[b] >= 1 && s.box_tris[b] <= mcpt::kDirectK) s.direct_counts |= s.box_tris[b] << (4u * b);
         else std::memset(&s.direct_list[size_t(b) * mcpt::kDirectK], 0, 4 * mcpt::kDirectK);
     }
+    uint32_t unlisted = 0;
+    for (uint32_t b = 0; b < s.n_miss_boxes; ++b)
+        if (s.box_tris[b] > mcpt::kDirectK) unlisted |= 1u << b;
+    s.clip_spheres = mcpt::clip_spheres(hs, s.miss_box, static_cast<int>(s.n_miss_boxes), s.tri_box, unlisted,
+                                        mcpt::kSphereMargin, mcpt::kSphereMaxReach, s.clip_sphere);
     s.cull_gain = 0.0f;
     for (const mcpt::Geometry& ge : hs.geoms)
         for (float k : {ge.Kd.x, ge.Kd.y, ge.Kd.z, ge.Ks.x, ge.Ks.y, ge.Ks.z})
@@ -288,6 +293,8 @@
                 std::memcpy(R->miss_box, s->miss_box, sizeof s->miss_box);
                 R->direct_counts = s->direct_counts;
                 std::memcpy(R->direct_list, s->direct_list, sizeof s->direct_list);
+                R->clip_spheres = s->clip_spheres;
+                std::memcpy(R->clip_sphere, s->clip_sphere, sizeof s->clip_sphere);
                 upload(*R, devs[i], s->image, nrm);
                 HIP_TRY(hipStreamCreateWithFlags(&R->stream, hipStreamNonBlocking));
                 HIP_TRY(hipEventCreateWithFlags(&R->done, hipEventDisableTiming));
@@ -509,6 +516,12 @@
 uint64_t mcpt_scene_extend_rays(const mcpt_scene* s) { return s ? s->extend_rays : 0; }
 uint64_t mcpt_scene_clipped_rays(const mcpt_scene* s) { return s ? s->clipped_rays : 0; }
 uint64_t mcpt_scene_primary_shaded(const mcpt_scene* s) { return s ? s->primary_shaded : 0; }
+uint64_t mcpt_scene_sphere_skips(const mcpt_scene* s) { return s ? s->sphere_skips : 0; }
+uint32_t mcpt_scene_clip_spheres(const mcpt_scene* s, float* spheres) {
+    if (!s) return 0;
+    if (spheres) std::memcpy(spheres, s->clip_sphere, sizeof s->clip_sphere);
+    return s->clip_spheres;
+}
 uint64_t mcpt_scene_primary_shade_lds(const mcpt_scene* s) {
     if (!s) return 0;
     mcpt::WfFacts f = scene_facts(*s);
diff --git a/montecarlopathtracer_amd/csrc/trace_device.hpp b/montecarlopathtracer_amd/csrc/trace_device.hpp
--- a/montecarlopathtracer_amd/csrc/trace_device.hpp
+++ b/montecarlopathtracer_amd/csrc/trace_device.hpp
@@ -258,6 +258,19 @@
     lo = max_qnan(max3_qnan(0.0f, nx ? bx : ax, ny ? by : ay), nz ? bz : az);
     hi = min_qnan(min3_qnan(best_init, nx ? ax : bx, ny ? ay : by), nz ? az : bz);
 }
+__device__ __forceinline__ void sphere_interval(V3 o, V3 d, const float (&s)[4], float& lo, float& hi) {
+    const float mx = s[0] - o.x, my = s[1] - o.y, mz = s[2] - o.z;
+    const float a = (d.x * d.x + d.y * d.y) + d.z * d.z;
+    const float b = (mx * d.x + my * d.y) + mz * d.z;
+    const float ia = 1.0f / a;
+    const float tc = b * ia;
+    const float px = mx - tc * d.x, py = my - tc * d.y, pz = mz - tc * d.z;
+    const float q = s[3] - ((px * px + py * py) + pz * pz);
+    const float h = sqrt_rn(q * ia);
+    const bool miss = q < 0.0f;
+    lo = miss ? kFltMax : max_qnan(lo, tc - h);
+    hi = miss ? 0.0f : min_qnan(hi, tc + h);
+}
 __device__ __forceinline__ uint32_t scene_box_hits(V3 o, V3 d, V3 inv, float best_init,
                                                    const float (&boxes)[kMaxMissBoxes][6], uint32_t n) {
     uint32_t acc = 0;
diff --git a/montecarlopathtracer_amd/csrc/wavefront.hip b/montecarlopathtracer_amd/csrc/wavefront.hip
--- a/montecarlopathtracer_amd/csrc/wavefront.hip
+++ b/montecarlopathtracer_amd/csrc/wavefront.hip
@@ -79,193 +79,9 @@
                                              : (LAY == kLayLds && !COUNT && MCPT_WF_LDS_WPE
                                                     ? MCPT_WF_LDS_WPE : 1))
 wf_extend(const KernelParams kp, const WfParams wf) {
-    constexpr bool IN_LDS = LAY != kLayGlobal;
-    extern __shared__ __attribute__((aligned(16))) unsigned char smem[];
-    const uint32_t g = blockIdx.x;
-    WfCounters* cn = wf.cnt + (size_t)wf.bounce * wf.nseg + g;
-    const uint32_t count = g < wf.nseg ? cn->queued : 0u;
-    if (count == 0) {
-        if (g < wf.nseg && threadIdx.x == 0) cn->hits = 0;
-        return;
-    }
-    const int tid = (int)threadIdx.x;
-    const GpuScene& sc = kp.scene;
-    unsigned char* const lds_image = smem + (size_t)S * BLOCK * 16;
-    uint32_t* const lslot = reinterpret_cast<uint32_t*>(lds_image + (IN_LDS ? sc.image_bytes : 0u));
-    if (tid == 0) *lslot = 0;
-    const SceneView sv = open_scene<IN_LDS, BLOCK>(lds_image, sc, tid);
-    constexpr bool CLIP = LAY == kLayLds && !COUNT;
-    uint32_t dtab = 0, dcnt = 0;
-    if constexpr (CLIP) {
-        asm volatile("s_mov_b32 %0, %1" : "=s"(dcnt) : "s"(wf.direct_counts));
-        asm volatile("s_mov_b32 %0, %1" : "=s"(dtab) : "s"((sc.image_bytes + (uint32_t)kLdsCounterBytes - sc.off_leafs) / 4u));
-        if (dcnt && tid < (int)(kDirectLdsBytes / 4))
-            (lslot + kLdsCounterBytes / 4)[tid] = tid < (int)kDirectTableWords ? wf.direct_list[tid] : 0u;
-    }
-    uint32_t unl = 0, nclip = 0, csel = 0;
-    if constexpr (CLIP) asm volatile("s_mov_b32 %0, %1" : "=s"(unl) : "s"(unlisted_boxes(wf.direct_counts)));
-    __syncthreads();
-    uint4* st = reinterpret_cast<uint4*>(smem) + tid;
-    uint4* spill = kp.spill + (blockIdx.x * BLOCK + (uint32_t)tid);
-    const uint32_t spill_stride = kp.total_lanes;
-    const size_t seg0 = (size_t)g * wf.seg;
-    float4* qb = wf.q[wf.bounce & 1];
-    const uint32_t qs = wf.slot_stride;
-
-    Counters c = {0, 0, 0, 0, 0, 0, 0, 0};
-#ifdef MCPT_PHASE_TIMING
-    LaneUse lu = {0, 0, 0, 0, 0, 0};
-#endif
-    SlotCursor cur_chunk = {0, kChunk};
-    RayState r;
-    r.htri = -1;
-    int mode = kDead;
-    constexpr bool PF = LAY != kLayGlobal || MCPT_WF_GLOBAL_PREFETCH;
-    uint32_t slot = cur_chunk.take(true, lslot), depth = 0;
-    uint32_t nslot = PF ? cur_chunk.take(true, lslot) : 0u;
-    float4 no4 = make_float4(0, 0, 0, 0), nd4 = make_float4(0, 0, 0, 0);
-    auto start = [&](float4 o4, float4 d4) {
-        r.o = v3(opaque(o4.x), opaque(o4.y), opaque(o4.z));
-        r.d = v3(opaque(d4.x), opaque(d4.y), opaque(d4.z));
-        depth = __float_as_uint(d4.w);
-        const bool live = begin_ray(r, sc, kp.best_init);
-        if constexpr (CLIP) {
-            csel = depth == kNoRay ? 0u : depth >> kDirectShift;
-            const uint32_t um = csel & unl;
-            const V3 inv = v3(r.ix, r.iy, r.iz);
-            float clo = kFltMax, chi = 0.0f;
-#pragma unroll 1
-            for (uint32_t i = 0; i < wf.n_miss_boxes; i++) {
-                const bool mine = ((um >> i) & 1u) != 0u;
-                if (((unl >> i) & 1u) != 0u && __ballot(mine)) {
-                    float lo, hi;
-                    box_interval(r.o, r.d, inv, kp.best_init, wf.miss_box[i], lo, hi);
-                    clo = mine ? min_qnan(clo, lo) : clo;
-                    chi = mine ? max_qnan(chi, hi) : chi;
-                }
-            }
-            const bool sel = csel != 0u;
-            const float t0 = max_qnan(r.tmin, clo * kEpsLo);
-            const float t1 = min_qnan(r.tmax, (chi * kEpsHi) * kEpsHi);
-            const bool walk = !(t0 > t1);
-            const uint32_t lm = csel & ~unl;
-            const bool hasl = lm != 0u;
-            const uint32_t lb = (uint32_t)(__ffs((int)lm) - 1) & 7u;
-            const uint32_t lp = dtab + lb * kDirectK;
-            r.lpos = hasl ? lp : 0u;
-            r.lend = hasl ? lp + ((dcnt >> (4u * lb)) & 15u) : 0u;
-            r.tmin = sel ? t0 : r.tmin;
-            r.tmax = sel ? t1 : r.tmax;
-            if (hasl & walk) {
-                st4(slot_of<S>(st, BLOCK, 0), make_uint4(r.nw0, r.nw1, __float_as_uint(t0), __float_as_uint(t1)));
-                r.sp = BLOCK * 16;
-            }
-            mode = (depth != kNoRay && live && (!sel | hasl | walk)) ? kTrav : kReady;
-            return;
-        }
-        mode = (depth != kNoRay && live) ? kTrav : kReady;
-    };
-#ifdef MCPT_PHASE_TIMING
-    unsigned long long tm_setup = 0, tm_trav = 0, tm_hand = 0, tm_iters = 0, tm_hands = 0,
-                       tm_t0 = __builtin_amdgcn_s_memtime();
-#define WF_STAMP(acc) do { unsigned long long t1_ = __builtin_amdgcn_s_memtime(); acc += t1_ - tm_t0; tm_t0 = t1_; } while (0)
-#else
-#define WF_STAMP(acc) do {} while (0)
-#endif
-    int refill;
-    asm volatile("s_mov_b32 %0, %1" : "=s"(refill) : "s"(wf.refill_thresh));
-    const bool eye0 = MCPT_WF_IMPLICIT0 >= 2 && wf.bounce == 0 && eye_origins0(kp);
-    const float4 eye4 = make_float4(kp.eye[0], kp.eye[1], kp.eye[2], 0.0f);
-    auto ld_o = [&](uint32_t sl) { return eye0 ? eye4 : ldq(&qb[qf(seg0 + sl, kQO, qs)]); };
-    if (slot < count) start(ld_o(slot), ldq(&qb[qf(seg0 + slot, kQD, qs)]));
-    if constexpr (CLIP) nclip += (uint32_t)__popcll(__ballot(slot < count && csel != 0u));
-    if (PF && nslot < count) { no4 = ld_o(nslot); nd4 = ldq(&qb[qf(seg0 + nslot, kQD, qs)]); }
-    WF_STAMP(tm_setup);
-    for (;;) {
-        __builtin_amdgcn_s_setprio(MCPT_WF_EXT_PRIO);
-        for (;;) {
-#ifdef MCPT_PHASE_TIMING
-            tm_iters++;
-            {
-                const uint64_t tv = __ballot(mode == kTrav);
-                if ((threadIdx.x & 63u) == 0) { lu.burst_w += 1; lu.burst_l += (unsigned long long)__popcll(tv); }
-            }
-#endif
-            MCPT_MARK(5);
-            if (mode == kTrav) {
-                if (trav_iter<S, !IN_LDS, COUNT, LAY == kLayLds, IN_LDS ? kWfLdsCap : MCPT_WF_DESCENT_CAP_GLOBAL>(
-                        r, sv.tris, sv.nodes, sv.leafs, st, BLOCK, spill, spill_stride, c MCPT_LU_ARG, sv.pairs))
-                    mode = kReady;
-            }
-            MCPT_MARK(6);
-            const uint64_t trv = __ballot(mode == kTrav);
-            const uint64_t rdy = __ballot(mode == kReady);
-            if (!trv || (int)__popcll(rdy) >= refill) break;
-        }
-        WF_STAMP(tm_trav);
-#ifdef MCPT_PHASE_TIMING
-        tm_hands++;
-#endif
-        MCPT_MARK(7);
-        __builtin_amdgcn_s_setprio(MCPT_WF_EXT_PRIO + 1);
-        if constexpr (PF) {
-            no4 = make_float4(opaque(no4.x), opaque(no4.y), opaque(no4.z), opaque(no4.w));
-            nd4 = make_float4(opaque(nd4.x), opaque(nd4.y), opaque(nd4.z), opaque(nd4.w));
-        }
-        const bool fin = mode == kReady;
-        const uint32_t ns0 = PF ? 0u : cur_chunk.take(fin, lslot);
-        const uint32_t fslot = slot;
-        csel = 0u;
-        if (fin) {
-            const int32_t hid = r.htri;
-            if constexpr (PF) {
-                slot = nslot;
-                start(no4, nd4);
-            } else {
-                slot = ns0;
-                float4 o4 = make_float4(0, 0, 0, 0), d4 = make_float4(0, 0, 0, __uint_as_float(kNoRay));
-                if (slot < count) { o4 = ld_o(slot); d4 = ldq(&qb[qf(seg0 + slot, kQD, qs)]); }
-                start(o4, d4);
-            }
-            if (slot >= count) mode = kDead;
-            reinterpret_cast<int32_t*>(qb + qf(0, kQHIT, qs))[seg0 + fslot] = hid;
-        }
-        if constexpr (CLIP) nclip += (uint32_t)__popcll(__ballot(fin && mode != kDead && csel != 0u));
-        if constexpr (PF) {
-            const bool want = fin && mode != kDead;
-            const uint32_t ns = cur_chunk.take(want, lslot);
-            if (want) {
-                nslot = ns;
-                if (nslot < count) { no4 = ld_o(nslot); nd4 = ldq(&qb[qf(seg0 + nslot, kQD, qs)]); }
-            }
-        }
-        WF_STAMP(tm_hand);
-        MCPT_MARK(8);
-        if (!__ballot(mode != kDead)) break;
-    }
-#ifdef MCPT_PHASE_TIMING
-    if ((threadIdx.x & 63u) == 0) {
-        atomicAdd(kp.stats + 8, tm_setup);
-        atomicAdd(kp.stats + 9, tm_trav);
-        atomicAdd(kp.stats + 10, tm_hand);
-        atomicAdd(kp.stats + 11, tm_iters);
-        atomicAdd(kp.stats + 12, tm_hands);
-    }
-    {
-        unsigned long long* gl = reinterpret_cast<unsigned long long*>(&g_lane_use);
-        const unsigned long long v[6] = {lu.desc_w, lu.desc_l, lu.tri_w, lu.tri_l, lu.burst_w, lu.burst_l};
-        for (int i = 0; i < 6; i++) {
-            unsigned long long x = v[i];
-            for (int off = 32; off > 0; off >>= 1) x += __shfl_xor(x, off);
-            if ((threadIdx.x & 63u) == 0) atomicAdd(gl + i, x);
-        }
-    }
-#endif
-    flush_counters(c, kp.stats);
-    if (tid == 0 && wf.bounce > 0) atomicAdd(kp.stats + kStatExtend, (unsigned long long)count);
-    if constexpr (CLIP)
-        if ((tid & 63) == 0 && nclip) atomicAdd(kp.stats + kStatClipped, (unsigned long long)nclip);
-    if (tid == 0) cn->hits = count;
+    constexpr bool SPHERE = false;
+    constexpr SphereClip sphc = {};
+#include "wf_extend_body.hpp"
 }
 
 template <int BLOCK, bool GEO_LDS, bool SORTB>
@@ -599,10 +415,11 @@
     return hipGetLastError();
 }
 
-enum class Extend { kPrimaryShade, kPrimaryLists, kPacket, kLds, kGlobal };
+enum class Extend { kPrimaryShade, kPrimaryLists, kPacket, kLds, kSphereClip, kGlobal };
 Extend extend_form(const WfRoute& r, int bounce, bool lists) {
     if (bounce == 0 && lists) return r.primary_shade ? Extend::kPrimaryShade : Extend::kPrimaryLists;
     if (bounce == 0 && r.packet) return Extend::kPacket;
+    if (bounce > 0 && r.clip.mask) return Extend::kSphereClip;
     return r.in_lds ? Extend::kLds : Extend::kGlobal;
 }
 hipError_t launch_bounce(const WfBatch& b, bool* shaded) {
@@ -615,6 +432,7 @@
         case Extend::kPrimaryLists: return launch_wavefront_primary_lists(b.kp, wf, (int)r.nseg, r.packet_lds, b.st);
         case Extend::kPacket: return launch_wavefront_primary(b.kp, wf, (int)r.nseg, r.packet_lds, b.st);
         case Extend::kLds: return launch_extend<kLayLds, 4, kLdsBlock>(b.kp, wf, (int)r.nseg, r.extend_lds, b.st);
+        case Extend::kSphereClip: return launch_wavefront_sphere_clip(b.kp, wf, r.clip, (int)r.nseg, r.extend_lds, b.st);
         default: return launch_extend<kLayGlobal, MCPT_WF_GLOBAL_S, kGlobalBlock>(b.kp, wf, (int)r.nseg, r.extend_lds, b.st);
     }
 }
diff --git a/montecarlopathtracer_amd/csrc/wavefront_sphere.hip b/montecarlopathtracer_amd/csrc/wavefront_sphere.hip
--- /dev/null
+++ b/montecarlopathtracer_amd/csrc/wavefront_sphere.hip
@@ -0,0 +1,22 @@
+#include "wf_device.hpp"
+
+namespace mcpt {
+namespace {
+
+template <int S, int BLOCK>
+__global__ void __launch_bounds__(BLOCK, 1)
+wf_sphere_clip(const KernelParams kp, const WfParams wf, const SphereClip sphc) {
+    constexpr int LAY = kLayLds;
+    constexpr bool COUNT = false;
+    constexpr bool SPHERE = true;
+#include "wf_extend_body.hpp"
+}
+
+}
+
+hipError_t launch_wavefront_sphere_clip(const KernelParams& kp, const WfParams& wf, const SphereClip& clip, int grid,
+                                        size_t lds, hipStream_t st) {
+    return launch_dyn_lds(wf_sphere_clip<4, kLdsBlock>, dim3(grid), dim3(kLdsBlock), lds, st, kp, wf, clip);
+}
+
+}
diff --git a/montecarlopathtracer_amd/csrc/wf_device.hpp b/montecarlopathtracer_amd/csrc/wf_device.hpp
--- a/montecarlopathtracer_amd/csrc/wf_device.hpp
+++ b/montecarlopathtracer_amd/csrc/wf_device.hpp
@@ -20,6 +20,8 @@
                                           hipStream_t st);
 hipError_t launch_wavefront_primary_shade(const KernelParams& kp, const WfParams& wf, int grid, size_t lds,
                                           hipStream_t st);
+hipError_t launch_wavefront_sphere_clip(const KernelParams& kp, const WfParams& wf, const SphereClip& clip, int grid,
+                                        size_t lds, hipStream_t st);
 
 namespace {
 
diff --git a/montecarlopathtracer_amd/csrc/wf_extend_body.hpp b/montecarlopathtracer_amd/csrc/wf_extend_body.hpp
--- /dev/null
+++ b/montecarlopathtracer_amd/csrc/wf_extend_body.hpp
@@ -0,0 +1,209 @@
+    constexpr bool IN_LDS = LAY != kLayGlobal;
+    extern __shared__ __attribute__((aligned(16))) unsigned char smem[];
+    const uint32_t g = blockIdx.x;
+    WfCounters* cn = wf.cnt + (size_t)wf.bounce * wf.nseg + g;
+    const uint32_t count = g < wf.nseg ? cn->queued : 0u;
+    if (count == 0) {
+        if (g < wf.nseg && threadIdx.x == 0) cn->hits = 0;
+        return;
+    }
+    const int tid = (int)threadIdx.x;
+    const GpuScene& sc = kp.scene;
+    unsigned char* const lds_image = smem + (size_t)S * BLOCK * 16;
+    uint32_t* const lslot = reinterpret_cast<uint32_t*>(lds_image + (IN_LDS ? sc.image_bytes : 0u));
+    if (tid == 0) *lslot = 0;
+    const SceneView sv = open_scene<IN_LDS, BLOCK>(lds_image, sc, tid);
+    constexpr bool CLIP = LAY == kLayLds && !COUNT;
+    uint32_t dtab = 0, dcnt = 0;
+    if constexpr (CLIP) {
+        asm volatile("s_mov_b32 %0, %1" : "=s"(dcnt) : "s"(wf.direct_counts));
+        asm volatile("s_mov_b32 %0, %1" : "=s"(dtab) : "s"((sc.image_bytes + (uint32_t)kLdsCounterBytes - sc.off_leafs) / 4u));
+        if (dcnt && tid < (int)(kDirectLdsBytes / 4))
+            (lslot + kLdsCounterBytes / 4)[tid] = tid < (int)kDirectTableWords ? wf.direct_list[tid] : 0u;
+    }
+    uint32_t unl = 0, nclip = 0, csel = 0;
+    if constexpr (CLIP) asm volatile("s_mov_b32 %0, %1" : "=s"(unl) : "s"(unlisted_boxes(wf.direct_counts)));
+    uint32_t sph = 0, nskip = 0;
+    bool cskip = false;
+    if constexpr (SPHERE) asm volatile("s_mov_b32 %0, %1" : "=s"(sph) : "s"(sphc.mask));
+    __syncthreads();
+    uint4* st = reinterpret_cast<uint4*>(smem) + tid;
+    uint4* spill = kp.spill + (blockIdx.x * BLOCK + (uint32_t)tid);
+    const uint32_t spill_stride = kp.total_lanes;
+    const size_t seg0 = (size_t)g * wf.seg;
+    float4* qb = wf.q[wf.bounce & 1];
+    const uint32_t qs = wf.slot_stride;
+
+    Counters c = {0, 0, 0, 0, 0, 0, 0, 0};
+#ifdef MCPT_PHASE_TIMING
+    LaneUse lu = {0, 0, 0, 0, 0, 0};
+#endif
+    SlotCursor cur_chunk = {0, kChunk};
+    RayState r;
+    r.htri = -1;
+    int mode = kDead;
+    constexpr bool PF = LAY != kLayGlobal || MCPT_WF_GLOBAL_PREFETCH;
+    uint32_t slot = cur_chunk.take(true, lslot), depth = 0;
+    uint32_t nslot = PF ? cur_chunk.take(true, lslot) : 0u;
+    float4 no4 = make_float4(0, 0, 0, 0), nd4 = make_float4(0, 0, 0, 0);
+    auto start = [&](float4 o4, float4 d4) {
+        r.o = v3(opaque(o4.x), opaque(o4.y), opaque(o4.z));
+        r.d = v3(opaque(d4.x), opaque(d4.y), opaque(d4.z));
+        depth = __float_as_uint(d4.w);
+        const bool live = begin_ray(r, sc, kp.best_init);
+        if constexpr (CLIP) {
+            csel = depth == kNoRay ? 0u : depth >> kDirectShift;
+            const uint32_t um = csel & unl;
+            const V3 inv = v3(r.ix, r.iy, r.iz);
+            float clo = kFltMax, chi = 0.0f;
+            float clo0 = kFltMax, chi0 = 0.0f;
+#pragma unroll 1
+            for (uint32_t i = 0; i < wf.n_miss_boxes; i++) {
+                const bool mine = ((um >> i) & 1u) != 0u;
+                if (((unl >> i) & 1u) != 0u && __ballot(mine)) {
+                    float lo, hi;
+                    box_interval(r.o, r.d, inv, kp.best_init, wf.miss_box[i], lo, hi);
+                    if constexpr (SPHERE) {
+                        clo0 = mine ? min_qnan(clo0, lo) : clo0;
+                        chi0 = mine ? max_qnan(chi0, hi) : chi0;
+                        if (((sph >> i) & 1u) != 0u) {
+                            sphere_interval(r.o, r.d, sphc.sphere[i], lo, hi);
+                            const bool none = lo * kEpsLo > hi * kEpsHi;
+                            lo = none ? kFltMax : lo;
+                            hi = none ? 0.0f : hi;
+                        }
+                    }
+                    clo = mine ? min_qnan(clo, lo) : clo;
+                    chi = mine ? max_qnan(chi, hi) : chi;
+                }
+            }
+            const bool sel = csel != 0u;
+            const float t0 = max_qnan(r.tmin, clo * kEpsLo);
+            const float t1 = min_qnan(r.tmax, (chi * kEpsHi) * kEpsHi);
+            const bool walk = !(t0 > t1);
+            if constexpr (SPHERE)
+                cskip = sel && !walk &&
+                        !(max_qnan(r.tmin, clo0 * kEpsLo) > min_qnan(r.tmax, (chi0 * kEpsHi) * kEpsHi));
+            const uint32_t lm = csel & ~unl;
+            const bool hasl = lm != 0u;
+            const uint32_t lb = (uint32_t)(__ffs((int)lm) - 1) & 7u;
+            const uint32_t lp = dtab + lb * kDirectK;
+            r.lpos = hasl ? lp : 0u;
+            r.lend = hasl ? lp + ((dcnt >> (4u * lb)) & 15u) : 0u;
+            r.tmin = sel ? t0 : r.tmin;
+            r.tmax = sel ? t1 : r.tmax;
+            if (hasl & walk) {
+                st4(slot_of<S>(st, BLOCK, 0), make_uint4(r.nw0, r.nw1, __float_as_uint(t0), __float_as_uint(t1)));
+                r.sp = BLOCK * 16;
+            }
+            mode = (depth != kNoRay && live && (!sel | hasl | walk)) ? kTrav : kReady;
+            return;
+        }
+        mode = (depth != kNoRay && live) ? kTrav : kReady;
+    };
+#ifdef MCPT_PHASE_TIMING
+    unsigned long long tm_setup = 0, tm_trav = 0, tm_hand = 0, tm_iters = 0, tm_hands = 0,
+                       tm_t0 = __builtin_amdgcn_s_memtime();
+#define WF_STAMP(acc) do { unsigned long long t1_ = __builtin_amdgcn_s_memtime(); acc += t1_ - tm_t0; tm_t0 = t1_; } while (0)
+#else
+#define WF_STAMP(acc) do {} while (0)
+#endif
+    int refill;
+    asm volatile("s_mov_b32 %0, %1" : "=s"(refill) : "s"(wf.refill_thresh));
+    const bool eye0 = MCPT_WF_IMPLICIT0 >= 2 && wf.bounce == 0 && eye_origins0(kp);
+    const float4 eye4 = make_float4(kp.eye[0], kp.eye[1], kp.eye[2], 0.0f);
+    auto ld_o = [&](uint32_t sl) { return eye0 ? eye4 : ldq(&qb[qf(seg0 + sl, kQO, qs)]); };
+    if (slot < count) start(ld_o(slot), ldq(&qb[qf(seg0 + slot, kQD, qs)]));
+    if constexpr (CLIP) nclip += (uint32_t)__popcll(__ballot(slot < count && csel != 0u));
+    if constexpr (SPHERE) nskip += (uint32_t)__popcll(__ballot(slot < count && cskip));
+    if (PF && nslot < count) { no4 = ld_o(nslot); nd4 = ldq(&qb[qf(seg0 + nslot, kQD, qs)]); }
+    WF_STAMP(tm_setup);
+    for (;;) {
+        __builtin_amdgcn_s_setprio(MCPT_WF_EXT_PRIO);
+        for (;;) {
+#ifdef MCPT_PHASE_TIMING
+            tm_iters++;
+            {
+                const uint64_t tv = __ballot(mode == kTrav);
+                if ((threadIdx.x & 63u) == 0) { lu.burst_w += 1; lu.burst_l += (unsigned long long)__popcll(tv); }
+            }
+#endif
+            MCPT_MARK(5);
+            if (mode == kTrav) {
+                if (trav_iter<S, !IN_LDS, COUNT, LAY == kLayLds, IN_LDS ? kWfLdsCap : MCPT_WF_DESCENT_CAP_GLOBAL>(
+                        r, sv.tris, sv.nodes, sv.leafs, st, BLOCK, spill, spill_stride, c MCPT_LU_ARG, sv.pairs))
+                    mode = kReady;
+            }
+            MCPT_MARK(6);
+            const uint64_t trv = __ballot(mode == kTrav);
+            const uint64_t rdy = __ballot(mode == kReady);
+            if (!trv || (int)__popcll(rdy) >= refill) break;
+        }
+        WF_STAMP(tm_trav);
+#ifdef MCPT_PHASE_TIMING
+        tm_hands++;
+#endif
+        MCPT_MARK(7);
+        __builtin_amdgcn_s_setprio(MCPT_WF_EXT_PRIO + 1);
+        if constexpr (PF) {
+            no4 = make_float4(opaque(no4.x), opaque(no4.y), opaque(no4.z), opaque(no4.w));
+            nd4 = make_float4(opaque(nd4.x), opaque(nd4.y), opaque(nd4.z), opaque(nd4.w));
+        }
+        const bool fin = mode == kReady;
+        const uint32_t ns0 = PF ? 0u : cur_chunk.take(fin, lslot);
+        const uint32_t fslot = slot;
+        csel = 0u;
+        cskip = false;
+        if (fin) {
+            const int32_t hid = r.htri;
+            if constexpr (PF) {
+                slot = nslot;
+                start(no4, nd4);
+            } else {
+                slot = ns0;
+                float4 o4 = make_float4(0, 0, 0, 0), d4 = make_float4(0, 0, 0, __uint_as_float(kNoRay));
+                if (slot < count) { o4 = ld_o(slot); d4 = ldq(&qb[qf(seg0 + slot, kQD, qs)]); }
+                start(o4, d4);
+            }
+            if (slot >= count) mode = kDead;
+            reinterpret_cast<int32_t*>(qb + qf(0, kQHIT, qs))[seg0 + fslot] = hid;
+        }
+        if constexpr (CLIP) nclip += (uint32_t)__popcll(__ballot(fin && mode != kDead && csel != 0u));
+        if constexpr (SPHERE) nskip += (uint32_t)__popcll(__ballot(fin && mode != kDead && cskip));
+        if constexpr (PF) {
+            const bool want = fin && mode != kDead;
+            const uint32_t ns = cur_chunk.take(want, lslot);
+            if (want) {
+                nslot = ns;
+                if (nslot < count) { no4 = ld_o(nslot); nd4 = ldq(&qb[qf(seg0 + nslot, kQD, qs)]); }
+            }
+        }
+        WF_STAMP(tm_hand);
+        MCPT_MARK(8);
+        if (!__ballot(mode != kDead)) break;
+    }
+#ifdef MCPT_PHASE_TIMING
+    if ((threadIdx.x & 63u) == 0) {
+        atomicAdd(kp.stats + 8, tm_setup);
+        atomicAdd(kp.stats + 9, tm_trav);
+        atomicAdd(kp.stats + 10, tm_hand);
+        atomicAdd(kp.stats + 11, tm_iters);
+        atomicAdd(kp.stats + 12, tm_hands);
+    }
+    {
+        unsigned long long* gl = reinterpret_cast<unsigned long long*>(&g_lane_use);
+        const unsigned long long v[6] = {lu.desc_w, lu.desc_l, lu.tri_w, lu.tri_l, lu.burst_w, lu.burst_l};
+        for (int i = 0; i < 6; i++) {
+            unsigned long long x = v[i];
+            for (int off = 32; off > 0; off >>= 1) x += __shfl_xor(x, off);
+            if ((threadIdx.x & 63u) == 0) atomicAdd(gl + i, x);
+        }
+    }
+#endif
+    flush_counters(c, kp.stats);
+    if (tid == 0 && wf.bounce > 0) atomicAdd(kp.stats + kStatExtend, (unsigned long long)count);
+    if constexpr (CLIP)
+        if ((tid & 63) == 0 && nclip) atomicAdd(kp.stats + kStatClipped, (unsigned long long)nclip);
+    if constexpr (SPHERE)
+        if ((tid & 63) == 0 && nskip) atomicAdd(kp.stats + kStatSphereSkips, (unsigned long long)nskip);
+    if (tid == 0) cn->hits = count;
diff --git a/montecarlopathtracer_amd/csrc/wf_route.hpp b/montecarlopathtracer_amd/csrc/wf_route.hpp
--- a/montecarlopathtracer_amd/csrc/wf_route.hpp
+++ b/montecarlopathtracer_amd/csrc/wf_route.hpp
@@ -40,6 +40,8 @@
     bool tile_records;
     int tile, max_depth;
     uint32_t group_shift;
+    uint32_t clip_spheres;
+    const float (*clip_sphere)[4];
 };
 
 struct WfRoute {
@@ -63,6 +65,7 @@
     int cull_bounce;
     uint32_t group_shift, xcd_deal;
     size_t packet_lds, extend_lds, direct_lds, primary_shade_lds, geo_lds;
+    SphereClip clip;
 };
 
 inline WfRoute wf_route(const WfFacts& f) {
@@ -80,6 +83,11 @@
     r.n_cull_boxes = f.n_cull_boxes;
     r.shade_cull = f.lean && r.in_lds && !f.sort && r.n_miss_boxes != 0;
     r.carry = r.shade_cull && r.direct;
+    if (r.direct && f.lean && r.in_lds && !f.sort && !f.qe && f.clip_sphere) {
+        r.clip.mask = f.clip_spheres;
+        for (int b = 0; b < kMaxMissBoxes; b++)
+            for (int a = 0; a < 4; a++) r.clip.sphere[b][a] = f.clip_sphere[b][a];
+    }
     r.group_shift = r.in_lds ? 6u : f.group_shift;
     r.xcd_deal = r.in_lds ? 0u : 1u;
     r.packet = MCPT_WF_PACKET0 && MCPT_WF_IMPLICIT0 >= 2 && r.in_lds && !f.qe && !f.listed;
diff --git a/montecarlopathtracer_amd/tracer.py b/montecarlopathtracer_amd/tracer.py
--- a/montecarlopathtracer_amd/tracer.py
+++ b/montecarlopathtracer_amd/tracer.py
@@ -290,12 +290,17 @@
                 "list_kd": list_kd[: 8 * k].reshape(8, k)[: len(box_tris)] if k else list_kd[:0].reshape(0, 0),
                 "counts": counts}
 
+    def clip_spheres(self) -> dict:
+        sp = np.zeros((8, 4), np.float32)
+        return {"mask": int(lib().mcpt_scene_clip_spheres(self.handle, _fptr(sp))), "spheres": sp}
+
     def _render_stats(self, st) -> dict:
         d = st.as_dict()
         d["direct_rays"] = int(lib().mcpt_scene_direct_rays(self.handle))
         d["extend_rays"] = int(lib().mcpt_scene_extend_rays(self.handle))
         d["clipped_rays"] = int(lib().mcpt_scene_clipped_rays(self.handle))
         d["primary_shaded"] = int(lib().mcpt_scene_primary_shaded(self.handle))
+        d["sphere_skips"] = int(lib().mcpt_scene_sphere_skips(self.handle))
         return d
 
     def primary_tile_classes(self):
```

Measured after the change: 29640 Mray/s, median of 6. 1.11x the previous value.
